# pyannote/pyannote-video

Measured on AMD Instinct MI355X. Metric: frames/sec end-to-end detect->embed->cluster, 1080p@25fps, higher is better.
Workload: dtype f32 (detector scores, embedder) / f64 (tracker, clustering) / u8 frames; an f16 screening pass with a proven error bound decides which windows the detector's exact f32 chain is evaluated for -- results identical to dense f32 scoring (`dense_scoring`)

## Files before the change

### include/pvface.h

```cpp
#ifndef PVFACE_H
#define PVFACE_H
#include <stdint.h>
#include <stddef.h>

#ifdef __cplusplus
extern "C" {
#endif

typedef uint64_t pvf_handle;
typedef struct { int32_t left, top, right, bottom; } pvf_rect_i32;

const char* pvf_last_error(void);
int32_t pvf_version(void);
int32_t pvf_device_count(int32_t* n);
int32_t pvf_ctx_create(int32_t device, pvf_handle* ctx);
int32_t pvf_ctx_create_prio(int32_t device, int32_t priority_class, pvf_handle* ctx);
int32_t pvf_ctx_destroy(pvf_handle ctx);
int32_t pvf_sync(pvf_handle ctx);

int32_t pvf_load_detector(pvf_handle ctx, const char* path);
int32_t pvf_load_shape_predictor(pvf_handle ctx, const char* path);
int32_t pvf_load_embedder(pvf_handle ctx, const char* path);
int32_t pvf_model_tensor(const char* path, int32_t kind, const char* name, void* out, int64_t cap_bytes, int64_t* nbytes);
int32_t pvf_set_tracker_tables(pvf_handle ctx, const double* mask64, const double* mask_scale, const double* tw64,
                               const double* tw32, double alpha_pow_m16, double ln_alpha);

int32_t pvf_frame_upload(pvf_handle ctx, const uint8_t* rgb, int32_t h, int32_t w, int64_t row_stride_bytes, pvf_handle* frame);
int32_t pvf_frame_wrap_device(pvf_handle ctx, const void* dev_rgb, int32_t h, int32_t w, pvf_handle* frame);
int32_t pvf_frame_release(pvf_handle ctx, pvf_handle frame);
int32_t pvf_frame_release_many(pvf_handle ctx, const pvf_handle* frames, int32_t n);
int32_t pvf_frame_pool_trim(pvf_handle ctx, int64_t keep_bytes, int64_t* pooled_bytes);
int32_t pvf_mem_info(pvf_handle ctx, int64_t* free_bytes, int64_t* total_bytes);
int32_t pvf_frame_device_ptr(pvf_handle ctx, pvf_handle frame, const void** dev_rgb);

int32_t pvf_ingest_create(pvf_handle ctx, int32_t h, int32_t w, int32_t depth, pvf_handle* ring);
int32_t pvf_ingest_destroy(pvf_handle ctx, pvf_handle ring);
int32_t pvf_ingest_acquire(pvf_handle ctx, pvf_handle ring, int32_t* slot, uint8_t** host_rgb);
int32_t pvf_ingest_submit(pvf_handle ctx, pvf_handle ring, int32_t slot, pvf_handle* frame);
int32_t pvf_ingest_wait(pvf_handle ctx, pvf_handle ring);
#define PVF_YUV_BT709 1
#define PVF_YUV_FULL_RANGE 2
int32_t pvf_ingest_create_yuv(pvf_handle ctx, int32_t h, int32_t w, int32_t depth, int32_t layout, int32_t flags, pvf_handle* ring);
int32_t pvf_frame_from_yuv(pvf_handle ctx, const uint8_t* y, int64_t y_pitch, const uint8_t* u, const uint8_t* v, int64_t c_pitch,
                           int32_t c_step, int32_t h, int32_t w, int32_t layout, int32_t flags, pvf_handle* frame);
int32_t pvf_frame_resize(pvf_handle ctx, pvf_handle frame, int32_t out_w, int32_t out_h, pvf_handle* out);

#define PVF_PRIM_RECT 0
#define PVF_PRIM_LINE 1
#define PVF_PRIM_TEXT 2
#define PVF_RENDER_MAX_PRIMS 4096
#define PVF_RENDER_MAX_RUN 64
#define PVF_RENDER_MAX_TEXT (1 << 20)
#define PVF_RENDER_MAX_SCALE 64
#define PVF_RENDER_MAX_BATCH 1024
typedef struct { int32_t type, a, b, c, d; uint32_t colour; int32_t scale, reserved; } pvf_prim;
int32_t pvf_render_batch(pvf_handle ctx, const pvf_handle* frames, int32_t n, int32_t out_w, int32_t out_h, int32_t flags,
                         const int32_t* start, const pvf_prim* prims, const uint8_t* text, int64_t text_bytes,
                         uint8_t* out, int32_t out_on_device);
int32_t pvf_egress_create(pvf_handle ctx, int32_t out_w, int32_t out_h, int32_t depth, int32_t flags, pvf_handle* ring);
int32_t pvf_egress_destroy(pvf_handle ctx, pvf_handle ring);
int32_t pvf_egress_submit(pvf_handle ctx, pvf_handle ring, pvf_handle frame, const pvf_prim* prims, int32_t n_prims,
                          const uint8_t* text, int64_t text_bytes, int32_t* slot);
int32_t pvf_egress_wait(pvf_handle ctx, pvf_handle ring, int32_t slot, const uint8_t** host_planes);
int32_t pvf_egress_release(pvf_handle ctx, pvf_handle ring, int32_t slot);
int32_t pvf_debug_render_rgb(pvf_handle ctx, pvf_handle frame, int32_t out_w, int32_t out_h, const pvf_prim* prims, int32_t n_prims,
                             const uint8_t* text, int64_t text_bytes, uint8_t* rgb);

int32_t pvf_detect(pvf_handle ctx, pvf_handle frame, int32_t upsample, double adjust_threshold,
                   pvf_rect_i32* out, float* scores, int32_t cap, int32_t* n);
int32_t pvf_detect_batch(pvf_handle ctx, const pvf_handle* frames, int32_t n_frames, int32_t upsample,
                         double adjust_threshold, pvf_rect_i32* out, float* scores, int32_t* counts,
                         int32_t cap_per_frame);
int32_t pvf_detect_many(pvf_handle ctx, const pvf_handle* frames, int32_t n_frames, int32_t batch, int32_t upsample,
                        double adjust_threshold, pvf_rect_i32* out, float* scores, int32_t* counts, int32_t cap);

int32_t pvf_detector_screening(pvf_handle ctx, int32_t on, int32_t list_cap);
int32_t pvf_detector_screening_stats(pvf_handle ctx, int64_t* batches, int64_t* listed, int64_t* retries, double* bounds, double* pipe_err);

int32_t pvf_embedder_split(pvf_handle ctx, int32_t on);
int32_t pvf_embedder_split_stats(pvf_handle ctx, int64_t* faces, int64_t* reruns, double* pipe_err);

int32_t pvf_tracker_create(pvf_handle ctx, pvf_handle* trk);
int32_t pvf_tracker_create_many(pvf_handle ctx, int32_t n, pvf_handle* trks);
int32_t pvf_tracker_destroy_many(pvf_handle ctx, const pvf_handle* trks, int32_t n);
int32_t pvf_tracker_clone_many(pvf_handle ctx, const pvf_handle* src, int32_t n, pvf_handle* dst);
int32_t pvf_tracker_destroy(pvf_handle ctx, pvf_handle trk);
int32_t pvf_tracker_start(pvf_handle ctx, pvf_handle trk, pvf_handle frame, const double box[4]);
int32_t pvf_tracker_update(pvf_handle ctx, pvf_handle trk, pvf_handle frame, double* psr);
int32_t pvf_tracker_position(pvf_handle ctx, pvf_handle trk, double box[4]);
int32_t pvf_tracker_start_many(pvf_handle ctx, const pvf_handle* trks, const pvf_handle* frames,
                               const double* boxes , int32_t n);
int32_t pvf_tracker_update_many(pvf_handle ctx, const pvf_handle* trks, const pvf_handle* frames, int32_t n,
                                double* psr , double* boxes_out );
int32_t pvf_tracker_update_many_deferred(pvf_handle ctx, const pvf_handle* trks, const pvf_handle* frames, int32_t n,
                                         double* psr, double* boxes_out);
int32_t pvf_tracker_commit_many(pvf_handle ctx, const pvf_handle* trks, const pvf_handle* frames, int32_t n);

int32_t pvf_overlap_matrix(const double* a, int32_t na, const double* b, int32_t nb, double ratio, double* out);
int32_t pvf_associate(const double* trackers, int32_t n_trackers, const double* detections, int32_t n_detections,
                      double min_overlap_ratio, int32_t* det_of_tracker);
int32_t pvf_munkres(const double* cost, int32_t n, int32_t* row_to_col);

int32_t pvf_landmarks(pvf_handle ctx, const pvf_handle* frames, const pvf_rect_i32* boxes, int32_t n,
                      int32_t* pts );
int32_t pvf_embed(pvf_handle ctx, const pvf_handle* frames, const int32_t* pts , int32_t n,
                  float* out );
int32_t pvf_landmarks_embed(pvf_handle ctx, const pvf_handle* frames, const pvf_rect_i32* boxes, int32_t n,
                            int32_t* pts , float* out );
int32_t pvf_embed_chips(pvf_handle ctx, const uint8_t* chips, int32_t n, float* out );
int32_t pvf_face_chips(pvf_handle ctx, const pvf_handle* frames, const int32_t* pts, int32_t n, uint8_t* chips );

int32_t pvf_pair_mean_dist(pvf_handle ctx, const double* X, int32_t N, int32_t dim, const int32_t* row_start,
                           int32_t T, double* D);
int32_t pvf_pair_mean_dist_metric(pvf_handle ctx, const double* X, int32_t N, int32_t dim, const int32_t* row_start,
                                  int32_t T, int32_t metric, double* D);
int32_t pvf_lane_create(int32_t n_frames, const int32_t* det_counts , const double* det_boxes ,
                        int32_t direction, double min_confidence, double min_overlap_ratio, int32_t deferring, pvf_handle* lane);
int32_t pvf_lane_destroy(pvf_handle lane);
int32_t pvf_lane_feed_plan(pvf_handle lane, int32_t p0, int32_t n_p, const uint8_t* has_update, const uint64_t* handles, const double* psr,
                           const double* pos);
int32_t pvf_lane_advance(pvf_handle lane, const double* reply_psr, const double* reply_pos, int32_t n_reply, int32_t* request,
                         uint64_t* req_handles, int32_t* req_frames, int32_t cap, int32_t* n_req, int32_t* plan_from);
int32_t pvf_lane_take_dead(pvf_handle lane, uint64_t* out, int32_t cap, int32_t* n);
int32_t pvf_lane_edges(pvf_handle lane, int32_t* n_edges, int32_t* u_frame_kind, double* u_box, int32_t* v_frame_kind, double* v_box,
                       double* conf, int32_t cap);
int32_t pvf_shot_tracks(pvf_handle lane_forward, pvf_handle lane_backward, const double* times, int32_t n_frames, double max_gap,
                        int32_t* rows, int32_t cap, int32_t* n_rows, int32_t* track_start, int32_t track_cap, int32_t* n_tracks);
int32_t pvf_track_rows(const int32_t* boxes, int64_t n, int32_t det_width, int32_t det_height, int32_t width, int32_t height,
                       double* file_box, int32_t* pixel_box);
int32_t pvf_round_decimals(const double* in, int64_t n, int32_t decimals, double* out);

int32_t pvf_pair_mean_dist_rows(pvf_handle ctx, const double* X, int32_t N, int32_t dim, const int32_t* row_start, int32_t T,
                                int32_t track0, int32_t track1, double* D);
int32_t pvf_pair_upper_rows(pvf_handle ctx, const double* X, int32_t N, int32_t dim, const int32_t* row_start, int32_t T,
                            int32_t track0, int32_t track1, double* D);
int32_t pvf_cluster_dist(pvf_handle ctx, const double* D, const int32_t* row_start, int32_t T, double threshold,
                         int32_t* labels, double* merge_log, int32_t* n_merges);
int32_t pvf_cluster_upper(pvf_handle ctx, const double* U, int32_t on_device, const int32_t* row_start, int32_t T, double threshold,
                          int32_t* labels, double* merge_log, int32_t* n_merges);
int32_t pvf_cluster_tracks(pvf_handle ctx, const double* X, int32_t N, int32_t dim, const int32_t* row_start,
                           int32_t T, double threshold, int32_t* labels, double* merge_log, int32_t* n_merges);
int32_t pvf_cluster_tracks_f32(pvf_handle ctx, const float* emb, int64_t row_stride_bytes, int32_t n_src, int32_t emb_on_device,
                               const int32_t* order, int32_t N, int32_t decimals, const int32_t* row_start, int32_t T, int32_t metric,
                               double threshold, int32_t* labels, double* merge_log, int32_t* n_merges);
int32_t pvf_pair_upper_rows_f32(pvf_handle ctx, const float* emb, int64_t row_stride_bytes, int32_t n_src, int32_t emb_on_device,
                                const int32_t* order, int32_t N, int32_t decimals, const int32_t* row_start, int32_t T,
                                int32_t track0, int32_t track1, double* rows_out, int32_t out_on_device);

int32_t pvf_format_rows(const double* t, const int64_t* identifier, const double* values, int64_t n_rows, int32_t n_cols,
                        int32_t decimals, char* out, int64_t cap, int64_t* written);

int32_t pvf_round_rows(const float* x, int64_t n, int32_t decimals, double* out);

int32_t pvf_parse_rows(const char* text, int64_t len, double* out, int64_t cap, int64_t* n_rows, int32_t* n_cols);

int32_t pvf_prof_enable(pvf_handle ctx, int32_t on);
int32_t pvf_prof_reset(pvf_handle ctx);
int32_t pvf_prof_get(pvf_handle ctx, const char* family, double* total_ms, int64_t* launches);

int32_t pvf_debug_pyramid_level(pvf_handle ctx, pvf_handle frame, int32_t upsample, int32_t level,
                                uint8_t* out, int32_t* h, int32_t* w);
int32_t pvf_debug_pyramid_batch(pvf_handle ctx, const pvf_handle* frames, int32_t n, int32_t upsample);
int32_t pvf_debug_level_features(pvf_handle ctx, pvf_handle frame, int32_t upsample, int32_t level,
                                 float* out, int32_t* fh, int32_t* fw);
int32_t pvf_debug_level_plan(pvf_handle ctx, pvf_handle frame, int32_t upsample, int32_t level, int32_t* out8);
int32_t pvf_debug_fhog(pvf_handle ctx, const uint8_t* img, int32_t h, int32_t w, int32_t cell, int32_t pad_r,
                       int32_t pad_c, float* out, int32_t* fh, int32_t* fw);
int32_t pvf_debug_detect_raw(pvf_handle ctx, pvf_handle frame, int32_t upsample, double adjust, float* scores,
                             int32_t* meta , int32_t cap, int32_t* n);
int32_t pvf_debug_detect_raw_many(pvf_handle ctx, const pvf_handle* frames, int32_t n_frames, int32_t batch, int32_t upsample,
                                  double adjust, int32_t* counts, int32_t* rows, int64_t cap, int64_t* total);
int32_t pvf_debug_extract_chip(pvf_handle ctx, pvf_handle frame, const double rect[4], double cs, double sn,
                               int32_t rows, int32_t cols, uint8_t* out);
int32_t pvf_debug_tracker_state(pvf_handle ctx, pvf_handle trk, double* F, double* A, double* B);
int32_t pvf_debug_tracker_scale_state(pvf_handle ctx, pvf_handle trk, double* As, double* Bs);
int32_t pvf_debug_embed_stage(pvf_handle ctx, const uint8_t* chips, int32_t n, int32_t split, int32_t stage, float* out, int32_t dims[3],
                              int32_t* flags);
int32_t pvf_debug_conv(pvf_handle ctx, const int32_t geom[18], const float* in, const float* w, const float* bias, const float* gamma,
                       const float* beta, const float* skip, int32_t split, int32_t force_generic, float* out, int32_t* flags);
int32_t pvf_debug_embed_head(pvf_handle ctx, const float* x, int32_t n, int32_t hw, float* out);

int32_t pvf_shot_dfd(pvf_handle ctx, const pvf_handle* frames, int32_t n, int32_t width, int32_t height, const float* tables,
                     double* dfd, uint8_t* gray_out, float* flow_out);

int32_t pvf_orb_extract(pvf_handle ctx, const pvf_handle* frames, int32_t n, int32_t width, int32_t height, int32_t cap,
                        int32_t* counts, float* keypoints, uint8_t* descriptors);
int32_t pvf_orb_match_counts(pvf_handle ctx, const uint8_t* descriptors, const int32_t* rows, int32_t n_sets, int32_t cap,
                             const int32_t* pairs, int64_t n_pairs, int32_t* counts);

#ifdef __cplusplus
}
#endif
#endif
```

### pyannote-video_amd/csrc/api.hip

```cpp
#include "pvf_internal.h"
#include <algorithm>
#include <cmath>
#include <cstdlib>
#include <string>
#include <thread>

#define API_BEGIN try {
#define API_END                                                        \
    return 0;                                                          \
    }                                                                  \
    catch (const std::exception& e) { pvf_set_error(e.what()); return -1; } \
    catch (...) { pvf_set_error("unknown error"); return -2; }

#define ENTER(c, h)                                                \
    Ctx* c = pvf_ctx(h);                                           \
    std::lock_guard<std::recursive_mutex> _api_lock(c->api_mu);    \
    HIP_CHECK(hipSetDevice(c->device))
#define ENTER_DET(c, h)                                            \
    Ctx* c = pvf_ctx(h);                                           \
    std::lock_guard<std::recursive_mutex> _det_lock(c->det_mu);    \
    HIP_CHECK(hipSetDevice(c->device))
#define ENTER_BOTH(c, h)                                           \
    Ctx* c = pvf_ctx(h);                                           \
    std::lock_guard<std::recursive_mutex> _det_lock(c->det_mu);    \
// ... 47 lines not shown
extern "C" int32_t pvf_embedder_split(pvf_handle h, int32_t on)
{
    API_BEGIN
    ENTER(c, h);
    c->emb_split = on != 0;
    API_END
}

extern "C" int32_t pvf_embedder_split_stats(pvf_handle h, int64_t* faces, int64_t* reruns, double* pipe_err)
{
    API_BEGIN
    ENTER(c, h);
    if (faces) *faces = c->emb_split_faces;
    if (reruns) *reruns = c->emb_reruns;
    if (pipe_err) *pipe_err = c->emb_pipe_err;
    API_END
}

extern "C" int32_t pvf_detect_batch(pvf_handle h, const pvf_handle* frames, int32_t n_frames, int32_t upsample, double adjust,
                                    pvf_rect_i32* out, float* scores, int32_t* counts, int32_t cap)
{
    API_BEGIN
    ENTER_DET(c, h);
    PVF_REQUIRE(n_frames > 0 && frames && out && counts && cap > 0, "pvf_detect_batch: bad arguments");
    PVF_REQUIRE(upsample >= 0 && upsample <= 2, "pvf_detect_batch: upsample must be 0..2");
    std::vector<Frame> fr(n_frames);
    for (int i = 0; i < n_frames; ++i) fr[i] = c->frame(frames[i]);
    std::vector<std::vector<RawDet>> raw;
    with_candidate_room(c, [&]() { det_run_batch(c, fr, upsample, adjust, raw); });
    std::vector<RawDet> kept;
    for (int i = 0; i < n_frames; ++i) {
        det_nms(c->det, raw[i], kept);
        const int n = std::min<int>((int)kept.size(), cap);
        counts[i] = n;
        for (int k = 0; k < n; ++k) {
            out[(size_t)i * cap + k] = pvf_rect_i32{kept[k].l, kept[k].t, kept[k].rr, kept[k].b};
            if (scores) scores[(size_t)i * cap + k] = kept[k].score;
        }
    }
    API_END
}

extern "C" int32_t pvf_detect_many(pvf_handle h, const pvf_handle* frames, int32_t n_frames, int32_t batch, int32_t upsample, double adjust,
                                   pvf_rect_i32* out, float* scores, int32_t* counts, int32_t cap)
{
    API_BEGIN
    ENTER_DET(c, h);
    PVF_REQUIRE(n_frames > 0 && batch > 0 && frames && out && counts && cap > 0, "pvf_detect_many: bad arguments");
    PVF_REQUIRE(upsample >= 0 && upsample <= 2, "pvf_detect_many: upsample must be 0..2");
    std::vector<Frame> fr(n_frames);
    for (int i = 0; i < n_frames; ++i) fr[i] = c->frame(frames[i]);
    std::vector<std::vector<RawDet>> kept_all;
    with_candidate_room(c, [&]() { det_run_many(c, fr, batch, upsample, adjust, kept_all, true); });
    for (int i = 0; i < n_frames; ++i) {
        const std::vector<RawDet>& kept = kept_all[i];
        const int n = std::min<int>((int)kept.size(), cap);
        counts[i] = n;
        for (int k = 0; k < n; ++k) {
            out[(size_t)i * cap + k] = pvf_rect_i32{kept[k].l, kept[k].t, kept[k].rr, kept[k].b};
            if (scores) scores[(size_t)i * cap + k] = kept[k].score;
        }
    }
    API_END
}

extern "C" int32_t pvf_detect(pvf_handle h, pvf_handle frame, int32_t upsample, double adjust, pvf_rect_i32* out, float* scores,
                              int32_t cap, int32_t* n)
{
    int32_t cnt = 0;
    const int32_t rc = pvf_detect_batch(h, &frame, 1, upsample, adjust, out, scores, &cnt, cap);
    if (rc == 0 && n) *n = cnt;
    return rc;
}

extern "C" int32_t pvf_debug_detect_raw(pvf_handle h, pvf_handle frame, int32_t upsample, double adjust, float* scores, int32_t* meta,
                                        int32_t cap, int32_t* n)
{
    API_BEGIN
    ENTER_DET(c, h);
    std::vector<Frame> fr{c->frame(frame)};
    std::vector<std::vector<RawDet>> raw;
    with_candidate_room(c, [&]() { det_run_batch(c, fr, upsample, adjust, raw); });
    const int k = std::min<int>((int)raw[0].size(), cap);
    *n = (int)raw[0].size();
    for (int i = 0; i < k; ++i) {
        const RawDet& d = raw[0][i];
        scores[i] = d.score;
        int32_t* m = meta + (size_t)i * 8;
        m[0] = d.filter; m[1] = d.level; m[2] = d.r; m[3] = d.c; m[4] = d.l; m[5] = d.t; m[6] = d.rr; m[7] = d.b;
    }
    API_END
}

extern "C" int32_t pvf_debug_detect_raw_many(pvf_handle h, const pvf_handle* frames, int32_t n_frames, int32_t batch, int32_t upsample, double adjust,
                                             int32_t* counts, int32_t* rows, int64_t cap, int64_t* total)
{
    API_BEGIN
    ENTER_DET(c, h);
    PVF_REQUIRE(n_frames > 0 && batch > 0 && frames && counts && total && (rows || cap == 0), "pvf_debug_detect_raw_many: bad arguments");
    PVF_REQUIRE(upsample >= 0 && upsample <= 2, "pvf_debug_detect_raw_many: upsample must be 0..2");
    std::vector<Frame> fr(n_frames);
    for (int i = 0; i < n_frames; ++i) fr[i] = c->frame(frames[i]);
    std::vector<std::vector<RawDet>> raw;
    with_candidate_room(c, [&]() { det_run_many(c, fr, batch, upsample, adjust, raw, false); });
    int64_t k = 0;
    for (int i = 0; i < n_frames; ++i) {
        counts[i] = (int32_t)raw[i].size();
        for (const RawDet& d : raw[i]) {
            if (k < cap) {
                int32_t* m = rows + (size_t)k * 5;
                m[0] = d.level; m[1] = d.filter; m[2] = d.r; m[3] = d.c;
                memcpy(&m[4], &d.score, 4);
            }
            ++k;
        }
    }
    *total = k;
    API_END
}

extern "C" int32_t pvf_debug_pyramid_level(pvf_handle h, pvf_handle frame, int32_t upsample, int32_t level, uint8_t* out, int32_t* oh,
                                           int32_t* ow)
{
    API_BEGIN
    ENTER_DET(c, h);
    std::vector<uint8_t> buf;
    int hh = 0, ww = 0;
    det_pyramid_level(c, c->frame(frame), upsample, level, out ? &buf : nullptr, &hh, &ww);
    *oh = hh; *ow = ww;
    if (out) memcpy(out, buf.data(), buf.size());
    API_END
}

extern "C" int32_t pvf_debug_pyramid_batch(pvf_handle h, const pvf_handle* frames, int32_t n, int32_t upsample)
{
    API_BEGIN
    ENTER_DET(c, h);
    PVF_REQUIRE(frames && n > 0, "pvf_debug_pyramid_batch: bad arguments");
    std::vector<Frame> fr;
    for (int i = 0; i < n; ++i) fr.push_back(c->frame(frames[i]));
    det_pyramid_batch(c, fr, upsample);
    API_END
}

extern "C" int32_t pvf_debug_level_features(pvf_handle h, pvf_handle frame, int32_t upsample, int32_t level, float* out, int32_t* fh, int32_t* fw)
{
    API_BEGIN
    ENTER_DET(c, h);
    std::vector<float> buf;
    int a = 0, b = 0;
    det_level_features(c, c->frame(frame), upsample, level, out ? &buf : nullptr, &a, &b);
    *fh = a; *fw = b;
    if (out) memcpy(out, buf.data(), buf.size() * sizeof(float));
    API_END
}

extern "C" int32_t pvf_debug_level_plan(pvf_handle h, pvf_handle frame, int32_t upsample, int32_t level, int32_t* out8)
{
    API_BEGIN
    ENTER_DET(c, h);
    PVF_REQUIRE(out8 != nullptr, "pvf_debug_level_plan: out8 is NULL");
    det_level_plan(c, c->frame(frame), upsample, level, out8);
    API_END
}

extern "C" int32_t pvf_debug_fhog(pvf_handle h, const uint8_t* img, int32_t ih, int32_t iw, int32_t cell, int32_t pad_r, int32_t pad_c,
                                  float* out, int32_t* fh, int32_t* fw)
{
    API_BEGIN
    ENTER_BOTH(c, h);
    int a = 0, b = 0;
    if (!out) { fhog_dims(ih, iw, cell, pad_r, pad_c, &a, &b); *fh = a; *fw = b; return 0; }
    std::vector<float> buf;
    fhog_debug(c, img, ih, iw, cell, pad_r, pad_c, buf, &a, &b);
    *fh = a; *fw = b;
    memcpy(out, buf.data(), buf.size() * sizeof(float));
    API_END
}

static pvf_handle tracker_new(Ctx* c)
{
    std::unique_ptr<Tracker> t(new Tracker());
    const uint64_t id = c->next_id++;
    c->trackers[id] = std::move(t);
    return id;
}

extern "C" int32_t pvf_tracker_create(pvf_handle h, pvf_handle* trk)
{
    API_BEGIN
    ENTER(c, h);
    *trk = tracker_new(c);
    API_END
}

extern "C" int32_t pvf_tracker_create_many(pvf_handle h, int32_t n, pvf_handle* trks)
{
    API_BEGIN
    ENTER(c, h);
    PVF_REQUIRE(n >= 0, "negative count");
    for (int i = 0; i < n; ++i) trks[i] = tracker_new(c);
    API_END
}

extern "C" int32_t pvf_tracker_clone_many(pvf_handle h, const pvf_handle* src, int32_t n, pvf_handle* dst)
{
    API_BEGIN
    ENTER(c, h);
    PVF_REQUIRE(n >= 0, "negative count");
    std::vector<Tracker*> s(n), d(n);
    for (int i = 0; i < n; ++i) s[i] = &c->tracker(src[i]);
    for (int i = 0; i < n; ++i) { dst[i] = tracker_new(c); d[i] = &c->tracker(dst[i]); }
    dsst_clone_many(c, s, d);
    API_END
}

static const size_t TRACKER_POOL_KEEP = 4096;
static void pool_tracker_state(Ctx* c, Tracker& t)
{
    double* d_state = t.d_state;
    t.d_state = nullptr;
    if (t.share) {
        int* sh = t.share;
        t.share = nullptr;
        if (--*sh > 0) return;
        delete sh;
    }
    if (!d_state) return;
    if (c->tracker_pool.size() < TRACKER_POOL_KEEP) { c->tracker_pool.push_back(d_state); return; }
    HIP_CHECK(hipStreamSynchronize(c->stream));
    HIP_CHECK(hipFree(d_state));
}

extern "C" int32_t pvf_tracker_destroy_many(pvf_handle h, const pvf_handle* trks, int32_t n)
{
    API_BEGIN
    ENTER(c, h);
    for (int i = 0; i < n; ++i) {
        auto it = c->trackers.find(trks[i]);
        PVF_REQUIRE(it != c->trackers.end(), "unknown tracker handle");
        pool_tracker_state(c, *it->second);
        c->trackers.erase(it);
    }
    API_END
}

extern "C" int32_t pvf_tracker_destroy(pvf_handle h, pvf_handle trk)
{
    API_BEGIN
    ENTER(c, h);
    auto it = c->trackers.find(trk);
    PVF_REQUIRE(it != c->trackers.end(), "unknown tracker handle");
    pool_tracker_state(c, *it->second);
    c->trackers.erase(it);
    API_END
}
extern "C" int32_t pvf_tracker_start_many(pvf_handle h, const pvf_handle* trks, const pvf_handle* frames, const double* boxes, int32_t n)
{
    API_BEGIN
    ENTER(c, h);
    std::vector<Tracker*> t(n);
    std::vector<Frame> f(n);
    PVF_REQUIRE(n >= 0 && (n == 0 || (trks && frames && boxes)), "tracker.start_track: bad arguments");
    for (int i = 0; i < n; ++i) {
        const double* b = boxes + 4 * (size_t)i;
        PVF_REQUIRE(std::isfinite(b[0]) && std::isfinite(b[1]) && std::isfinite(b[2]) && std::isfinite(b[3]),
                    "tracker.start_track: box with a non-finite coordinate");
        PVF_REQUIRE(b[2] - b[0] != 0.0 && b[3] - b[1] != 0.0, "tracker.start_track: box of zero width or height");
    }
    for (int i = 0; i < n; ++i) { t[i] = &c->tracker(trks[i]); f[i] = c->frame(frames[i]); }
    dsst_start_many(c, t, f, boxes);
    API_END
}
extern "C" int32_t pvf_tracker_update_many(pvf_handle h, const pvf_handle* trks, const pvf_handle* frames, int32_t n, double* psr,
                                           double* boxes_out)
{
    API_BEGIN
    ENTER(c, h);
    std::vector<Tracker*> t(n);
    std::vector<Frame> f(n);
    for (int i = 0; i < n; ++i) { t[i] = &c->tracker(trks[i]); f[i] = c->frame(frames[i]); }
    dsst_update_many(c, t, f, psr, boxes_out);
    API_END
}
extern "C" int32_t pvf_tracker_start(pvf_handle h, pvf_handle trk, pvf_handle frame, const double box[4])
{
    return pvf_tracker_start_many(h, &trk, &frame, box, 1);
}
extern "C" int32_t pvf_tracker_update_many_deferred(pvf_handle h, const pvf_handle* trks, const pvf_handle* frames, int32_t n, double* psr,
                                                    double* boxes_out)
{
    API_BEGIN
    ENTER(c, h);
    std::vector<Tracker*> t(n);
    std::vector<Frame> f(n);
    for (int i = 0; i < n; ++i) { t[i] = &c->tracker(trks[i]); f[i] = c->frame(frames[i]); }
    dsst_update_many(c, t, f, psr, boxes_out, 1);
    API_END
}

extern "C" int32_t pvf_tracker_commit_many(pvf_handle h, const pvf_handle* trks, const pvf_handle* frames, int32_t n)
{
    API_BEGIN
    ENTER(c, h);
    std::vector<Tracker*> t(n);
    std::vector<Frame> f(n);
// ... 689 lines not shown
```

### pyannote-video_amd/csrc/detect.hip

```cpp
#include "detect_ml.h"
#include <algorithm>
#include <thread>
#include <cmath>
#include <cstdlib>

#define RESIZE_MAXS 22
struct RowTab { int32_t top, bottom; double tb, tb1, pad; };
struct ColTab { int32_t left, pad; double lr, lr1, pad2; };

template <int RS, int NSTRIP>
__global__ void __launch_bounds__(256) resize_rows_k(const uint8_t* const* __restrict__ in_ptrs, const uint8_t* __restrict__ in_base,
                                                     size_t in_stride, int in_rb, int ih, int iw, uint8_t* __restrict__ out,
                                                     size_t out_stride, int out_rb, int oh, int ow,
                                                     const RowTab* __restrict__ rows, const ColTab* __restrict__ cols)
{
    constexpr int MAXS = (RS == 16) ? RESIZE_MAXS : (RS * 5) / 4 + 3;
    __shared__ uint32_t s_rows[4][MAXS][64];
    __shared__ uint32_t s_out[4][64];
    const int lane = threadIdx.x & 63;
    const int wave = __builtin_amdgcn_readfirstlane(threadIdx.x >> 6);
    const int c0 = blockIdx.x * 256 + wave * 64;
    const int b = blockIdx.z;
    if (c0 >= ow) return;
    const int c = min(c0 + lane, ow - 1);
// ... 164 lines not shown
}

static void pyramid_up_dims(int ih, int iw, int* oh, int* ow)
{
    const double right = ((iw - 1) + 1.25) * 2.0;
    const double bottom = ((ih - 1) + 0.75) * 2.0;
    *ow = (int)std::floor(right + 0.5) + 1;
    *oh = (int)std::floor(bottom + 0.5) + 1;
}


static inline long iround(double v) { return (long)std::floor(v + 0.5); }
static void rect_down6(long r[4]) { const double ratio = (6 - 1.0) / 6; for (int i = 0; i < 4; ++i) r[i] = iround((r[i] - 0.3) * ratio + 0.3); }
static void rect_up6(long r[4]) { const double ratio = 6 / (6 - 1.0); for (int i = 0; i < 4; ++i) r[i] = iround((r[i] - 0.3) * ratio + 0.3); }
static void rect_down2i(long r[4])
{
    r[0] = iround(r[0] / 2.0 - 1.25); r[1] = iround(r[1] / 2.0 - 0.75);
    r[2] = iround(r[2] / 2.0 - 1.25); r[3] = iround(r[3] / 2.0 - 0.75);
}
static int detector_levels(int h, int w, const DetectorModel& m)
{
    long r[4] = {0, 0, w - 1, h - 1};
    int levels = 0;
    do { rect_down6(r); ++levels; } while ((r[2] - r[0] + 1) >= m.min_w && (r[3] - r[1] + 1) >= m.min_h && levels < m.max_levels);
    return levels;
}
static void fhog_to_image(long px, long py, int cell, int pad_r, int pad_c, long* ox, long* oy)
{
    long x = (px + 1 - (pad_c - 1) / 2) * cell + 1;
    long y = (py + 1 - (pad_r - 1) / 2) * cell + 1;
    x += (x >= 0) ? cell / 2 : -(cell / 2);
    y += (y >= 0) ? cell / 2 : -(cell / 2);
    *ox = x; *oy = y;
}

struct LevelDims { int h, w; };
static std::vector<LevelDims> level_schedule(int h, int w, int upsample, const DetectorModel& m, std::vector<LevelDims>* ups)
{
    int ch = h, cw = w;
    for (int u = 0; u < upsample; ++u) {
        int nh, nw;
        pyramid_up_dims(ch, cw, &nh, &nw);
        ch = nh; cw = nw;
        if (ups) ups->push_back({ch, cw});
    }
    const int levels = detector_levels(ch, cw, m);
    std::vector<LevelDims> out;
    out.push_back({ch, cw});
    for (int l = 1; l < levels; ++l) { ch = (5 * ch) / 6; cw = (5 * cw) / 6; out.push_back({ch, cw}); }
    return out;
}

static void upload_frame_ptrs(Ctx* c, const std::vector<Frame>& frames, const uint8_t*** d_ptrs)
{
    DevBuf& d = c->s_fptr[c->det_slot & 1];
    HostBuf& h = c->h_fptr[c->det_slot & 1];
    d.ensure(frames.size() * sizeof(void*));
    h.ensure(frames.size() * sizeof(void*));
    const uint8_t** hp = h.as<const uint8_t*>();
    for (size_t i = 0; i < frames.size(); ++i) hp[i] = frames[i].d;
    HIP_CHECK(hipMemcpyAsync(d.p, hp, frames.size() * sizeof(void*), hipMemcpyHostToDevice, c->det_stream));
    *d_ptrs = d.as<const uint8_t*>();
}


__device__ __forceinline__ int ml_block(const MlStarts& st) { return (int)blockIdx.x; }
static inline int ml_grid(int total) { return total; }

__device__ __forceinline__ int ml_level(const MlStarts& st, int g)
{
    int l = 0;
    while (l + 1 < st.nl && g >= st.b0[l + 1]) ++l;
    return l;
}

#define FUSED_OUT 61
__device__ __forceinline__ uint32_t from_next_lane(uint32_t v) { return (uint32_t)__builtin_amdgcn_update_dpp(0, (int)v, 0x130, 0xf, 0xf, true); }
__device__ __forceinline__ uint32_t from_prev_lane(uint32_t v) { return (uint32_t)__builtin_amdgcn_update_dpp(0, (int)v, 0x138, 0xf, 0xf, true); }

#define FS_PAIRS 4
#define FS_COLS 65
#define FS_SLOT_DW (8 * FS_COLS * 2)
#define FS_BINS_DW (2 * 18 * 64)
#define FS_FLAG_DW (4 * 64)
#define FS_LDS_BYTES (FS_PAIRS * (FS_BINS_DW + 2 * FS_SLOT_DW + FS_FLAG_DW) * 4)
static_assert(FS_COLS * 8 == 520, "the ring's column pitch is written into the instruction strings below");
typedef __attribute__((address_space(3))) uint32_t* lds_u32;
__device__ __forceinline__ uint32_t lds_addr(const void* p) { return (uint32_t)(uintptr_t)(lds_u32)p; }

__device__ __forceinline__ void ring_write(uint32_t data_at, uint32_t flag_at, const u32x2* v, uint32_t row1)
{
    asm volatile("ds_write_b64 %0, %2\n\tds_write_b64 %0, %3 offset:520\n\tds_write_b64 %0, %4 offset:1040\n\tds_write_b64 %0, %5 offset:1560\n\t"
                 "ds_write_b64 %0, %6 offset:2080\n\tds_write_b64 %0, %7 offset:2600\n\tds_write_b64 %0, %8 offset:3120\n\t"
                 "ds_write_b64 %0, %9 offset:3640\n\tds_write_b32 %1, %10"
                 :: "v"(data_at), "v"(flag_at), "v"(v[0]), "v"(v[1]), "v"(v[2]), "v"(v[3]), "v"(v[4]), "v"(v[5]), "v"(v[6]), "v"(v[7]), "v"(row1) : "memory");
}
__device__ __forceinline__ uint32_t ring_read(uint32_t data_at, uint32_t flag_at, u32x2* own, u32x2* nb)
{
    uint32_t ready;
    asm volatile("ds_read_b32 %0, %18\n\t"
                 "ds_read_b64 %1, %17\n\tds_read_b64 %9, %17 offset:8\n\tds_read_b64 %2, %17 offset:520\n\tds_read_b64 %10, %17 offset:528\n\t"
                 "ds_read_b64 %3, %17 offset:1040\n\tds_read_b64 %11, %17 offset:1048\n\tds_read_b64 %4, %17 offset:1560\n\tds_read_b64 %12, %17 offset:1568\n\t"
                 "ds_read_b64 %5, %17 offset:2080\n\tds_read_b64 %13, %17 offset:2088\n\tds_read_b64 %6, %17 offset:2600\n\tds_read_b64 %14, %17 offset:2608\n\t"
                 "ds_read_b64 %7, %17 offset:3120\n\tds_read_b64 %15, %17 offset:3128\n\tds_read_b64 %8, %17 offset:3640\n\tds_read_b64 %16, %17 offset:3648\n\t"
                 "s_waitcnt lgkmcnt(0)"
                 : "=&v"(ready), "=&v"(own[0]), "=&v"(own[1]), "=&v"(own[2]), "=&v"(own[3]), "=&v"(own[4]), "=&v"(own[5]), "=&v"(own[6]), "=&v"(own[7]),
                   "=&v"(nb[0]), "=&v"(nb[1]), "=&v"(nb[2]), "=&v"(nb[3]), "=&v"(nb[4]), "=&v"(nb[5]), "=&v"(nb[6]), "=&v"(nb[7])
                 : "v"(data_at), "v"(flag_at) : "memory");
    return ready;
}
__device__ __forceinline__ void flag_write(uint32_t flag_at, uint32_t v)
{
    asm volatile("ds_write_b32 %0, %1" :: "v"(flag_at), "v"(v) : "memory");
}

template <int A, int B> __device__ __forceinline__ uint32_t sub_into_upper(uint32_t acc, uint32_t x, uint32_t y);
#define PVF_SUBW1(A, B)                                                                                                                  \
    template <> __device__ __forceinline__ uint32_t sub_into_upper<A, B>(uint32_t acc, uint32_t x, uint32_t y)                           \
    {                                                                                                                                    \
        asm("v_sub_u32_sdwa %0, %1, %2 dst_sel:WORD_1 dst_unused:UNUSED_PRESERVE src0_sel:BYTE_" #A " src1_sel:BYTE_" #B "\n\ts_nop 0"   \
            : "+v"(acc) : "v"(x), "v"(y));                                                                                               \
        return acc;                                                                                                                      \
    }
PVF_SUBW1(0, 0) PVF_SUBW1(1, 1) PVF_SUBW1(2, 2) PVF_SUBW1(3, 3)
#undef PVF_SUBW1
typedef short s16x2 __attribute__((ext_vector_type(2)));

template <int P>
__device__ __forceinline__ u32x2 split_grad_px(const uint32_t* up, const uint32_t* ce, const uint32_t* dn, const __amdgpu_buffer_rsrc_t& lut_rs,
                                               bool valid)
{
    uint32_t pk[3];
    int cv[3];
#define PVF_CH(K)                                                                                                                         \
    {                                                                                                                                     \
        constexpr int IU = 4 + 3 * P + K, IL = 1 + 3 * P + K, IR = 7 + 3 * P + K;                                                         \
        const uint32_t cx = ((ce[IR >> 2] >> (8 * (IR & 3))) & 0xffu) - ((ce[IL >> 2] >> (8 * (IL & 3))) & 0xffu);                          \
        pk[K] = sub_into_upper<(IU & 3), (IU & 3)>(cx, dn[IU >> 2], up[IU >> 2]);                                                          \
        const s16x2 v = __builtin_bit_cast(s16x2, pk[K]);                                                                                 \
        cv[K] = __builtin_amdgcn_sdot2(v, v, 0, false);                                                                                   \
    }
    PVF_CH(0) PVF_CH(1) PVF_CH(2)
#undef PVF_CH
    const int bv = max(cv[0], max(cv[1], cv[2]));
    const uint32_t pb = (cv[0] == bv) ? pk[0] : ((cv[1] == bv) ? pk[1] : pk[2]);
    const uint32_t off = (pb & 7u) | ((pb >> 13) & 0xff8u) | ((pb << 9) & 0x3f000u);
    u32x2 r;
    r.y = (uint32_t)__builtin_amdgcn_raw_buffer_load_b8(lut_rs, off, 0, 0);
    const float m = sqrt_exact_small((float)bv);
    r.x = valid ? __float_as_uint(m) : 0u;
    return r;
}

__global__ void __launch_bounds__(512) __attribute__((amdgpu_waves_per_eu(4, 4)))
fhog_split_ml_k(MlStarts st, const LvDesc* __restrict__ lv, int B, const uint8_t* __restrict__ img_base, float* __restrict__ feat_base,
                const uint8_t* __restrict__ lutw, int oy, int ox)
{
    constexpr int RSRC_FLAGS = 0x00020000;
    extern __shared__ __attribute__((aligned(16))) uint32_t fs_lds[];
    const int lane = threadIdx.x & 63;
    const int wave = __builtin_amdgcn_readfirstlane(threadIdx.x >> 6);
    const int pair = wave & 3, role = wave >> 2;
    for (int i = threadIdx.x; i < FS_PAIRS * (2 * FS_SLOT_DW + FS_FLAG_DW); i += 512) fs_lds[FS_PAIRS * FS_BINS_DW + i] = 0u;
    __syncthreads();
    const int g = ml_block(st);
    if (g >= st.b0[st.nl]) return;
    const int l = ml_level(st, g);
    const LvDesc d = lv[l];
    const int task = (g - st.b0[l]) * FS_PAIRS + pair;
    if (task >= d.fused_tasks) return;
    const int sx = task % d.strips;
    const int t2 = task / d.strips;
    const int cy = t2 % d.chunks;
    const int b = t2 / d.chunks;
    const int y0 = cy * d.chunk_rows;
    const int R = min(d.chunk_rows, d.hog_nr - y0);
    const int g_first = y0 + 1, g_last = y0 + R + 3;
    const int y_begin = 8 * g_first - 12;
    const uint32_t ring_at = lds_addr(fs_lds + FS_PAIRS * FS_BINS_DW + pair * 2 * FS_SLOT_DW) + 8u * lane;
    uint32_t* const flags = fs_lds + FS_PAIRS * (FS_BINS_DW + 2 * FS_SLOT_DW) + pair * FS_FLAG_DW + lane;
    const uint32_t flag_at = lds_addr(flags);

    if (role == 0) {
        const int hx = FUSED_OUT * sx + 1 + lane;
        const int x_first = 8 * hx - 12;
        const uint8_t* im = img_base + d.img_off + (size_t)b * d.img_stride;
        const int rb = d.rb;
        unsigned xmask = 0;
#pragma unroll
        for (int p = 0; p < 8; ++p) if (x_first + p >= 1 && x_first + p < d.visible_nc) xmask |= 1u << p;
        const bool strip_inside = __builtin_amdgcn_ballot_w64(xmask != 0xffu) == 0;
        const int voff = 3 * x_first - 4, voff2 = voff + 16;
        const __amdgpu_buffer_rsrc_t lut_rs = __builtin_amdgcn_make_buffer_rsrc((void*)lutw, 0, 1 << 18, RSRC_FLAGS);
        uint32_t rw[4][8];
        auto load_row = [&](int yi, uint32_t* dst) {
            const int bytes = (yi >= 0 && yi < d.h) ? rb : 0;
            const int yc = min(max(yi, 0), d.h - 1);
            const __amdgpu_buffer_rsrc_t rs = __builtin_amdgcn_make_buffer_rsrc((void*)(im + (size_t)yc * rb), 0, bytes, RSRC_FLAGS);
            const u32x4 a = __builtin_amdgcn_raw_buffer_load_b128(rs, voff, 0, 0);
            const u32x4 c = __builtin_amdgcn_raw_buffer_load_b128(rs, voff2, 0, 0);
            dst[0] = a.x; dst[1] = a.y; dst[2] = a.z; dst[3] = a.w; dst[4] = c.x; dst[5] = c.y; dst[6] = c.z; dst[7] = c.w;
        };
#pragma unroll
        for (int q = 0; q < 4; ++q) load_row(y_begin - 1 + q, rw[q]);
        const int nrows = 8 * (g_last - g_first + 1);
        for (int k0 = 0; k0 < nrows; k0 += 4) {
#pragma unroll
            for (int i = 0; i < 4; ++i) {
                const int k = k0 + i, y = y_begin + k;
                const uint32_t* up = rw[i & 3];
                const uint32_t* ce = rw[(i + 1) & 3];
                const uint32_t* dn = rw[(i + 2) & 3];
                const int freed = (int)__hip_atomic_load(flags + 128 + 64 * (i & 1), __ATOMIC_RELAXED, __HIP_MEMORY_SCOPE_WORKGROUP);
                const bool ok = (y >= 1 && y < d.visible_nr);
                u32x2 mb[8];
                if (strip_inside && ok) {
                    mb[0] = split_grad_px<0>(up, ce, dn, lut_rs, true); mb[1] = split_grad_px<1>(up, ce, dn, lut_rs, true);
                    mb[2] = split_grad_px<2>(up, ce, dn, lut_rs, true); mb[3] = split_grad_px<3>(up, ce, dn, lut_rs, true);
                    mb[4] = split_grad_px<4>(up, ce, dn, lut_rs, true); mb[5] = split_grad_px<5>(up, ce, dn, lut_rs, true);
                    mb[6] = split_grad_px<6>(up, ce, dn, lut_rs, true); mb[7] = split_grad_px<7>(up, ce, dn, lut_rs, true);
                } else {
                    mb[0] = split_grad_px<0>(up, ce, dn, lut_rs, ok && (xmask & 1u));
                    mb[1] = split_grad_px<1>(up, ce, dn, lut_rs, ok && (xmask & 2u));
                    mb[2] = split_grad_px<2>(up, ce, dn, lut_rs, ok && (xmask & 4u));
                    mb[3] = split_grad_px<3>(up, ce, dn, lut_rs, ok && (xmask & 8u));
                    mb[4] = split_grad_px<4>(up, ce, dn, lut_rs, ok && (xmask & 16u));
                    mb[5] = split_grad_px<5>(up, ce, dn, lut_rs, ok && (xmask & 32u));
                    mb[6] = split_grad_px<6>(up, ce, dn, lut_rs, ok && (xmask & 64u));
                    mb[7] = split_grad_px<7>(up, ce, dn, lut_rs, ok && (xmask & 128u));
                }
                load_row(y + 3, rw[i & 3]);
                int fr = freed;
                while (fr < k - 1) {
                    __builtin_amdgcn_s_sleep(1);
                    fr = (int)__hip_atomic_load(flags + 128 + 64 * (i & 1), __ATOMIC_RELAXED, __HIP_MEMORY_SCOPE_WORKGROUP);
                }
                ring_write(ring_at + (i & 1) * 4 * FS_SLOT_DW, flag_at + 256 * (i & 1), mb, (uint32_t)(k + 1));
            }
        }
        return;
    }

    float* accE = reinterpret_cast<float*>(fs_lds) + pair * FS_BINS_DW + lane;
    float* accO = accE + 18 * 64;
#pragma unroll
    for (int k = 0; k < 18; ++k) { accE[64 * k] = 0.0f; accO[64 * k] = 0.0f; }
    float hprev[18];
    float e0 = 0.f, e1 = 0.f, e2 = 0.f;
#pragma unroll
    for (int k = 0; k < 18; ++k) hprev[k] = 0.f;
    int krow = 0;
    auto band = [&](int gb, float* accU, float* accL) {
#pragma unroll
        for (int i = 0; i < 8; ++i) {
            u32x2 own[8], nb[8];
            for (;;) {
                const int ready = (int)ring_read(ring_at + (i & 1) * 4 * FS_SLOT_DW, flag_at + 256 * (i & 1), own, nb);
                if (__builtin_amdgcn_readfirstlane(ready) > krow) break;
                __builtin_amdgcn_s_sleep(1);
            }
            ++krow;
            flag_write(flag_at + 512 + 256 * (i & 1), (uint32_t)krow);
            const float fy = ((float)i + 0.5f) / 8.0f;
#pragma unroll
            for (int j = 0; j < 16; ++j) {
                const int p = j & 7;
                const u32x2 v = (j < 8) ? own[p] : nb[p];
                const float mv = __uint_as_float(v.x);
                const int bv = (int)(v.y << 8);
                const float fx = ((float)p + 0.5f) / 8.0f;
                const float wx = (j < 8) ? fx : 1.0f - fx;
                float* const pl = reinterpret_cast<float*>(reinterpret_cast<char*>(accL) + bv);
                float* const pu = reinterpret_cast<float*>(reinterpret_cast<char*>(accU) + bv);
                const float vl = *pl, vu = *pu;
                *pl = vl + ((1.0f - fy) * wx) * mv;
                *pu = vu + (fy * wx) * mv;
            }
        }
        const int c = gb - 1;
        float e = 0.0f;
#pragma unroll
        for (int o = 0; o < 9; ++o) { const float s2 = accL[64 * o] + accL[64 * (o + 9)]; e = e + s2 * s2; }
        e2 = e1; e1 = e0; e0 = e;
        if (c >= y0 + 3) {
            float n[9];
            n[1] = e2; n[4] = e1; n[7] = e0;
            n[0] = __uint_as_float(from_prev_lane(__float_as_uint(e2))); n[2] = __uint_as_float(from_next_lane(__float_as_uint(e2)));
            n[3] = __uint_as_float(from_prev_lane(__float_as_uint(e1))); n[5] = __uint_as_float(from_next_lane(__float_as_uint(e1)));
            n[6] = __uint_as_float(from_prev_lane(__float_as_uint(e0))); n[8] = __uint_as_float(from_next_lane(__float_as_uint(e0)));
            const int x = FUSED_OUT * sx + lane - 1, yh = c - 3;
            if (lane >= 1 && lane <= FUSED_OUT && x < d.hog_nc) {
                float4* dst = reinterpret_cast<float4*>(feat_base + d.feat_off + (size_t)b * d.feat_stride + feat_at(yh + oy, 0, x + ox, d.fwp));
                const size_t step = (size_t)d.fwp;
                const float eps = 0.0001f;
                const float z1[4] = {n[4], n[1], n[3], n[0]}, z2[4] = {n[5], n[2], n[4], n[1]}, z3[4] = {n[7], n[4], n[6], n[3]}, z4[4] = {n[8], n[5], n[7], n[4]};
                float nn[4], nv[4], t[4] = {0.f, 0.f, 0.f, 0.f};
#pragma unroll
                for (int k = 0; k < 4; ++k) {
                    nn[k] = 0.2f * sqrtf((((z1[k] + z2[k]) + z3[k]) + z4[k]) + eps);
                    nv[k] = 0.1f / nn[k];
                }
                float o[20];
#pragma unroll
                for (int g = 0; g < 18; g += 3) {
                    float hh[3][4];
#pragma unroll
                    for (int j = 0; j < 3; ++j) {
#pragma unroll
                        for (int k = 0; k < 4; ++k) hh[j][k] = fminf(hprev[g + j], nn[k]) * nv[k];
                        o[g + j] = (hh[j][0] + hh[j][1]) + (hh[j][2] + hh[j][3]);
                    }
#pragma unroll
                    for (int k = 0; k < 4; ++k) t[k] = t[k] + ((hh[0][k] + hh[1][k]) + hh[2][k]);
                    if (g == 3) { *dst = make_float4(o[0], o[1], o[2], o[3]); dst += step; __builtin_amdgcn_sched_barrier(0); }
                    if (g == 6) { *dst = make_float4(o[4], o[5], o[6], o[7]); dst += step; __builtin_amdgcn_sched_barrier(0); }
                    if (g == 9) { *dst = make_float4(o[8], o[9], o[10], o[11]); dst += step; __builtin_amdgcn_sched_barrier(0); }
                    if (g == 15) { *dst = make_float4(o[12], o[13], o[14], o[15]); dst += step; __builtin_amdgcn_sched_barrier(0); }
                }
                float ci[9];
#pragma unroll
                for (int g = 0; g < 9; ++g) {
                    const float s2 = hprev[g] + hprev[g + 9];
                    float hh[4];
#pragma unroll
                    for (int k = 0; k < 4; ++k) hh[k] = fminf(s2, nn[k]) * nv[k];
                    ci[g] = (hh[0] + hh[1]) + (hh[2] + hh[3]);
                    if (g == 1) { *dst = make_float4(o[16], o[17], ci[0], ci[1]); dst += step; __builtin_amdgcn_sched_barrier(0); }
                    if (g == 5) { *dst = make_float4(ci[2], ci[3], ci[4], ci[5]); dst += step; __builtin_amdgcn_sched_barrier(0); }
                }
                const float tscale = (float)(2 * 0.2357);
#pragma unroll
                for (int k = 0; k < 4; ++k) t[k] = t[k] * tscale;
                *dst = make_float4(ci[6], ci[7], ci[8], t[0]); dst += step;
                *dst = make_float4(t[1], t[2], t[3], 0.0f);
            }
        }
#pragma unroll
        for (int k = 0; k < 18; ++k) { hprev[k] = accL[64 * k]; accL[64 * k] = 0.0f; }
    };
    for (int gb = g_first; gb <= g_last; ++gb) {
        if (gb & 1) band(gb, accO, accE);
        else band(gb, accE, accO);
    }
}

__global__ void __launch_bounds__(256) feat_ring_zero_k(MlStarts st, const LvDesc* __restrict__ lv, int B, float* __restrict__ feat_base, int oy, int ox)
{
    const int g = ml_block(st);
    if (g >= st.b0[st.nl]) return;
    const int l = ml_level(st, g);
    const LvDesc d = lv[l];
    const int local = g - st.b0[l];
    const int xb = local % d.feat_bx;
    const int py = (local / d.feat_bx) % d.fh;
    const int b = local / (d.feat_bx * d.fh);
    const int px = xb * 256 + threadIdx.x;
    if (px >= d.fwp) return;
    const int x = px - ox, y = py - oy;
    if (x >= 0 && y >= 0 && x < d.hog_nc && y < d.hog_nr) return;
    float4* dst = reinterpret_cast<float4*>(feat_base + d.feat_off + (size_t)b * d.feat_stride + feat_at(py, 0, px, d.fwp));
#pragma unroll
    for (int k = 0; k < 8; ++k) dst[(size_t)k * d.fwp] = make_float4(0.f, 0.f, 0.f, 0.f);
}

__global__ void __launch_bounds__(128) __attribute__((amdgpu_waves_per_eu(2, 2)))
score_roll_k(MlStarts st, const LvDesc* __restrict__ lv, int B, const float* __restrict__ feat_base,
             const float4* __restrict__ Bg4, ScoreParams sp, int* __restrict__ counts, CandRec* __restrict__ cands)
{
    constexpr int FR = 10, FC = 10, NK = 12, PITCH = 31, MT = 2, WCOLS = MT * 48, SEG = WCOLS + 11, R = 5;
    constexpr int LAST_STEPS = 93 - 8 * (NK - 1);
    constexpr int NSTW = (SEG * 8 + 127) / 128;
    constexpr int SLAB = (SEG * PITCH + 3) / 4 * 4;
    constexpr int RSRC_FLAGS = 0x00020000;
    extern __shared__ __attribute__((aligned(16))) float s_seg[];
    const int lane = threadIdx.x & 63;
    const int wave = __builtin_amdgcn_readfirstlane(threadIdx.x >> 6);
    const int g = (int)blockIdx.x;
    if (g >= st.b0[st.nl]) return;
    const int l = ml_level(st, g);
    const LvDesc d = lv[l];
    const int local = g - st.b0[l];
    const int bx = local % d.score_bx;
    const int sg = (local / d.score_bx) % d.roll_nseg;
    const int b = __builtin_amdgcn_readfirstlane(local / (d.score_bx * d.roll_nseg));
    const int fw = d.fw;
    const int c_base = bx * WCOLS;
    const int c1 = fw - (FC - FC / 2 - 1);
    const int r_base = sg * d.roll_rows;
    const int out_rows = min(d.roll_rows, d.fh - (FR - 1) - r_base);
    const int fh = out_rows + FR - 1;
    const int fwp = d.fwp;
    const float* fb = feat_base + d.feat_off + (size_t)b * d.feat_stride + feat_at(r_base, 0, c_base, fwp);
    const int seg_cells = (fw - c_base < SEG) ? fw - c_base : SEG;
    const int i = lane & 15, kq = lane >> 4;
    const int lane16 = lane * 16;
    const bool two_tiles = (c_base + 48 + FC / 2 < c1);
    const __amdgpu_buffer_rsrc_t brs = __builtin_amdgcn_make_buffer_rsrc((void*)Bg4, 0, FR * NK * 2 * 64 * 16, RSRC_FLAGS);
    f32x4 acc[R][MT];
#pragma unroll
    for (int q = 0; q < R; ++q)
#pragma unroll
        for (int tt = 0; tt < MT; ++tt) acc[q][tt] = (f32x4){0.f, 0.f, 0.f, 0.f};
    constexpr int NH = 4;
    static_assert(NSTW <= 8 && SEG <= 128, "one cell per thread");
    u32x4 sv[NH];
    const int tid16 = (int)threadIdx.x * 16;
    auto load_part = [&](int fr, int half) {
        const int bytes = (fr < fh) ? seg_cells * 16 : 0;
#pragma unroll
        for (int u = 0; u < NH; ++u) {
            const __amdgpu_buffer_rsrc_t rs = __builtin_amdgcn_make_buffer_rsrc((void*)(fb + ((size_t)fr * 8 + half * NH + u) * fwp * 4), 0, bytes, RSRC_FLAGS);
            sv[u] = __builtin_amdgcn_raw_buffer_load_b128(rs, tid16, 0, 0);
        }
    };
    auto fill_part = [&](float* seg, int half) {
        if ((int)threadIdx.x < SEG) {
#pragma unroll
            for (int u = 0; u < NH; ++u) {
                const int q = half * NH + u;
                uint32_t* dd = reinterpret_cast<uint32_t*>(seg + (int)threadIdx.x * PITCH + 4 * q);
                dd[0] = sv[u].x; dd[1] = sv[u].y; dd[2] = sv[u].z;
                if (q != 7) dd[3] = sv[u].w;
            }
        }
    };
    auto emit = [&](int r_out, const f32x4 (&a)[MT]) {
        const int jc = lane & 15;
        if (jc < 15) {
            const int sft = jc / 5, f = jc % 5;
            const float th = sp.thresh[f];
            const int r = r_base + r_out + FR / 2;
#pragma unroll
            for (int tt = 0; tt < MT; ++tt)
#pragma unroll
                for (int reg = 0; reg < 4; ++reg) {
                    const int pos = 4 * (lane >> 4) + reg;
                    const int cc = c_base + tt * 48 + 3 * pos + sft + FC / 2;
                    const float v = a[tt][reg];
                    if (cc < c1 && v >= th && (tt == 0 || two_tiles)) {
                        const int idx = atomicAdd(&counts[b], 1);
                        if (idx < sp.cap) {
                            CandRec rec;
                            rec.score = v - th; rec.filter = f; rec.level = l; rec.r = r; rec.c = cc;
                            cands[(size_t)b * sp.cap + idx] = rec;
                        }
                    }
                }
        }
    };
    load_part(0, 0); fill_part(s_seg, 0);
    load_part(0, 1); fill_part(s_seg, 1);
    __syncthreads();
    for (int s = 0; s < fh; ++s) {
        const float* seg = s_seg + (s & 1) * SLAB;
        float* nxt = s_seg + ((s + 1) & 1) * SLAB;
        load_part(s + 1, 0);
        const int p = (s - wave) & 1;
        const int r0 = s - p;
        bool on[R];
        bool all_on = two_tiles, any_on = false;
#pragma unroll
        for (int q = 0; q < R; ++q) {
            const int r = r0 - 2 * q;
            on[q] = (r >= 0 && r < out_rows);
            all_on = all_on && on[q];
            any_on = any_on || on[q];
        }
        if (any_on) {
            const int bop = p * NK * 2048;
            const float* a0 = seg + (3 * i) * PITCH + kq;
            u32x4 bn[R][2];
            float an[8 * MT];
#pragma unroll
            for (int q = 0; q < R; ++q) {
                bn[q][0] = __builtin_amdgcn_raw_buffer_load_b128(brs, lane16, bop + 2 * q * NK * 2048, 0);
                bn[q][1] = __builtin_amdgcn_raw_buffer_load_b128(brs, lane16, bop + 2 * q * NK * 2048 + 1024, 0);
            }
#pragma unroll
            for (int pq = 0; pq < 8; ++pq)
#pragma unroll
                for (int tt = 0; tt < MT; ++tt) an[pq * MT + tt] = a0[(tt * 48) * PITCH + 4 * pq];
#pragma unroll
            for (int n = 0; n < NK; ++n) {
                float ac[8 * MT];
                float bc[R][8];
#pragma unroll
                for (int x = 0; x < 8 * MT; ++x) ac[x] = an[x];
#pragma unroll
                for (int q = 0; q < R; ++q)
#pragma unroll
                    for (int h = 0; h < 2; ++h) {
                        const uint32_t b0 = bn[q][h].x, b1 = bn[q][h].y, b2 = bn[q][h].z, b3 = bn[q][h].w;
                        bc[q][4 * h] = __uint_as_float(b0); bc[q][4 * h + 1] = __uint_as_float(b1);
                        bc[q][4 * h + 2] = __uint_as_float(b2); bc[q][4 * h + 3] = __uint_as_float(b3);
                    }
                if (n + 1 < NK) {
#pragma unroll
                    for (int q = 0; q < R; ++q) {
                        bn[q][0] = __builtin_amdgcn_raw_buffer_load_b128(brs, lane16, bop + (2 * q * NK + n + 1) * 2048, 0);
                        bn[q][1] = __builtin_amdgcn_raw_buffer_load_b128(brs, lane16, bop + (2 * q * NK + n + 1) * 2048 + 1024, 0);
                    }
#pragma unroll
                    for (int pq = 0; pq < 8; ++pq)
#pragma unroll
                        for (int tt = 0; tt < MT; ++tt) an[pq * MT + tt] = a0[(tt * 48) * PITCH + 32 * (n + 1) + 4 * pq];
                }
                if (n == NK / 2) { fill_part(nxt, 0); load_part(s + 1, 1); }
                __builtin_amdgcn_sched_barrier(0);
                const int steps = (n == NK - 1) ? LAST_STEPS : 8;
                if (all_on) {
#pragma unroll
                    for (int pq = 0; pq < steps; ++pq)
#pragma unroll
                        for (int q = 0; q < R; ++q)
#pragma unroll
// ... 88 lines not shown
            const int hog_nr = (int)((double)ld.h / 8.0 + 0.5) - 2, hog_nc = (int)((double)ld.w / 8.0 + 0.5) - 2;
            if (hog_nr > 0 && hog_nc > 0) tasks += (long long)((hog_nc + FUSED_OUT - 1) / FUSED_OUT) * std::max(2, (hog_nr + cand - 1) / cand) * B;
        }
        if (tasks >= 2LL * c->n_cu * 2 * 4) { chunk_big = cand; break; }
    }
    if (getenv("PVF_FHOG_CHUNK") && atoi(getenv("PVF_FHOG_CHUNK")) > 0) chunk_big = atoi(getenv("PVF_FHOG_CHUNK"));
    for (size_t l = 0; l < dims.size(); ++l) {
        LvDesc d;
        memset(&d, 0, sizeof d);
        d.h = dims[l].h; d.w = dims[l].w;
        d.cells_nr = (int)((double)d.h / 8.0 + 0.5); d.cells_nc = (int)((double)d.w / 8.0 + 0.5);
        d.visible_nr = std::min(d.cells_nr * 8, d.h) - 1; d.visible_nc = std::min(d.cells_nc * 8, d.w) - 1;
        d.hog_nr = d.cells_nr - 2; d.hog_nc = d.cells_nc - 2;
        const bool feat_ok = d.hog_nr > 0 && d.hog_nc > 0;
        d.fh = feat_ok ? d.hog_nr + m.frows - 1 : 0; d.fw = feat_ok ? d.hog_nc + m.fcols - 1 : 0;
        d.valid_score = (d.fh >= m.frows && d.fw >= m.fcols) ? 1 : 0;
        d.rb = (int)al((size_t)d.w * 3, 64);
        d.img_off = (long long)p.img_bytes; d.img_stride = (long long)d.h * d.rb;
        p.img_bytes += (size_t)d.img_stride * B;
        d.fwp = feat_ok ? d.fw + FEAT_PAD_COLS : 0;
        d.feat_off = (long long)p.feat_floats; d.feat_stride = (long long)d.fh * d.fwp * PVF_FHOG_STRIDE;
        p.feat_floats += (size_t)d.feat_stride * B;
        d.feat_bx = feat_ok ? (d.fwp + 255) / 256 : 0;
        const int out_c = d.fw - 9;
        d.score_bx = d.valid_score ? (out_c + 95) / 96 : 0;
        d.strips = feat_ok ? (d.hog_nc + FUSED_OUT - 1) / FUSED_OUT : 0;
        {
            const int nch = std::max(2, (d.hog_nr + chunk_big - 1) / chunk_big);
            d.chunk_rows = std::max((d.hog_nr + nch - 1) / nch, 1);
        }
        d.chunks = feat_ok ? (d.hog_nr + d.chunk_rows - 1) / d.chunk_rows : 0;
        d.fused_tasks = d.strips * d.chunks * B;
        p.feat.b0[l] = p.feat_blocks; p.feat_blocks += d.feat_bx * d.fh * B;
        p.fused.b0[l] = p.fused_blocks; p.fused_blocks += (d.fused_tasks + 3) / 4;
        p.lv.push_back(d);
    }
    const int nl = (int)dims.size();
    {
        long long total = 0;
        for (const LvDesc& d : p.lv) if (d.valid_score) total += (long long)d.score_bx * (d.fh - 9 + 9) * B;
        const int slots = 4 * 256;
        int roll_max = (int)std::max<long long>(64, total / slots / 2);
        if (getenv("PVF_SCORE_SEG")) roll_max = std::max(2, atoi(getenv("PVF_SCORE_SEG")));
        for (int l = 0; l < nl; ++l) {
            LvDesc& d = p.lv[l];
            const int out_r = d.fh - 9;
            d.roll_nseg = d.valid_score ? (out_r + roll_max - 1) / roll_max : 0;
            d.roll_rows = d.valid_score ? ((out_r + d.roll_nseg - 1) / d.roll_nseg + 1) / 2 * 2 : 0;
            if (d.valid_score) d.roll_nseg = (out_r + d.roll_rows - 1) / d.roll_rows;
            p.walk.b0[l] = p.walk_blocks; p.walk_blocks += d.score_bx * d.roll_nseg * B;
        }
    }
    p.feat.b0[nl] = p.feat_blocks; p.walk.b0[nl] = p.walk_blocks;
    p.fused.b0[nl] = p.fused_blocks;
    HIP_CHECK(hipMalloc((void**)&p.d_lv, sizeof(LvDesc) * nl));
    HIP_CHECK(hipMemcpy(p.d_lv, p.lv.data(), sizeof(LvDesc) * nl, hipMemcpyHostToDevice));
    {
        std::vector<RowTab> tab;
        int ch = h;
        for (size_t u = 0; u < p.ups.size(); ++u) { p.up_tab.push_back(tab.size()); fill_row_table(tab, ch, p.ups[u].h); ch = p.ups[u].h; }
        p.lv_tab.push_back(0);
        for (int l = 1; l < nl; ++l) { p.lv_tab.push_back(tab.size()); fill_row_table(tab, p.lv[l - 1].h, p.lv[l].h); }
        HIP_CHECK(hipMalloc((void**)&p.d_rowtab, sizeof(RowTab) * std::max<size_t>(tab.size(), 1)));
        if (!tab.empty()) HIP_CHECK(hipMemcpy(p.d_rowtab, tab.data(), sizeof(RowTab) * tab.size(), hipMemcpyHostToDevice));
        std::vector<ColTab> ctab;
        int cw2 = w;
        for (size_t u = 0; u < p.ups.size(); ++u) { p.up_ctab.push_back(ctab.size()); fill_col_table(ctab, cw2, p.ups[u].w); cw2 = p.ups[u].w; }
        p.lv_ctab.push_back(0);
        for (int l = 1; l < nl; ++l) { p.lv_ctab.push_back(ctab.size()); fill_col_table(ctab, p.lv[l - 1].w, p.lv[l].w); }
        HIP_CHECK(hipMalloc((void**)&p.d_coltab, sizeof(ColTab) * std::max<size_t>(ctab.size(), 1)));
        if (!ctab.empty()) HIP_CHECK(hipMemcpy(p.d_coltab, ctab.data(), sizeof(ColTab) * ctab.size(), hipMemcpyHostToDevice));
    }
    MlPlan* raw = pp.get();
    c->ml_plans->plans[key] = std::move(pp);
    return raw;
}

static MlPlan* ml_build_pyramid(Ctx* c, const std::vector<Frame>& frames, int upsample)
{
    const int B = (int)frames.size();
    const int h = frames[0].h, w = frames[0].w;
    for (auto& f : frames) PVF_REQUIRE(f.h == h && f.w == w, "batched frames must share one size");
    MlPlan* p = ml_plan(c, h, w, upsample, B);
    c->s_pyr.ensure(p->img_bytes + p->up_bytes + 256);
    uint8_t* base = c->s_pyr.as<uint8_t>();
    uint8_t* up_tmp = base + ((p->img_bytes + 63) / 64) * 64;
    const uint8_t** d_ptrs = nullptr;
    upload_frame_ptrs(c, frames, &d_ptrs);
    ProfScope ps(c, "pyramid", c->det_stream);
    auto al = [](size_t v, size_t a) { return (v + a - 1) / a * a; };
    const uint8_t* cur = nullptr;
    int ch = h, cw = w, crb = w * 3;
    size_t cstride = 0;
    for (size_t u = 0; u < p->ups.size(); ++u) {
        const bool last = (u + 1 == p->ups.size());
        uint8_t* dst = last ? base + p->lv[0].img_off : up_tmp;
        const int drb = (int)al((size_t)p->ups[u].w * 3, 64);
        const size_t dstride = (size_t)p->ups[u].h * drb;
        launch_resize_rows(c, cur ? nullptr : d_ptrs, cur, cstride, crb, ch, cw, dst, dstride, drb, p->ups[u].h, p->ups[u].w, B, p->d_rowtab + p->up_tab[u], p->d_coltab + p->up_ctab[u]);
        cur = dst; cstride = dstride; crb = drb; ch = p->ups[u].h; cw = p->ups[u].w;
    }
    if (!cur) {
        for (int b = 0; b < B; ++b)
            HIP_CHECK(hipMemcpy2DAsync(base + p->lv[0].img_off + (size_t)b * p->lv[0].img_stride, (size_t)p->lv[0].rb, frames[b].d, (size_t)w * 3,
                                       (size_t)w * 3, (size_t)h, hipMemcpyDeviceToDevice, c->det_stream));
    }
    for (size_t l = 1; l < p->lv.size(); ++l)
        launch_resize_rows(c, nullptr, base + p->lv[l - 1].img_off, (size_t)p->lv[l - 1].img_stride, p->lv[l - 1].rb, p->lv[l - 1].h, p->lv[l - 1].w,
                           base + p->lv[l].img_off, (size_t)p->lv[l].img_stride, p->lv[l].rb, p->lv[l].h, p->lv[l].w, B, p->d_rowtab + p->lv_tab[l], p->d_coltab + p->lv_ctab[l]);
    return p;
}

__global__ void dpp_probe_k(int* out)
{
    const int lane = threadIdx.x;
    out[lane] = (int)from_next_lane((uint32_t)(lane + 100));
    out[64 + lane] = (int)from_prev_lane((uint32_t)(lane + 100));
}
#define SQRT_PROBE_N (2 * 255 * 255 + 1)
__global__ void sqrt_probe_k(float* out)
{
    const int i = blockIdx.x * blockDim.x + threadIdx.x;
    if (i < SQRT_PROBE_N) out[i] = sqrt_exact_small((float)i);
}
static void check_dpp_direction(Ctx* c)
{
    MlPlanCache* pc = c->ml_plans;
    if (pc->dpp_probe < 0) {
        int* d = nullptr;
        HIP_CHECK(hipMalloc((void**)&d, 128 * sizeof(int) + SQRT_PROBE_N * sizeof(float)));
        float* ds = reinterpret_cast<float*>(d + 128);
        hipLaunchKernelGGL(dpp_probe_k, dim3(1), dim3(64), 0, c->det_stream, d);
        hipLaunchKernelGGL(sqrt_probe_k, dim3((SQRT_PROBE_N + 255) / 256), dim3(256), 0, c->det_stream, ds);
        int h[128];
        std::vector<float> hs(SQRT_PROBE_N);
        HIP_CHECK(hipMemcpyAsync(h, d, sizeof h, hipMemcpyDeviceToHost, c->det_stream));
        HIP_CHECK(hipMemcpyAsync(hs.data(), ds, SQRT_PROBE_N * sizeof(float), hipMemcpyDeviceToHost, c->det_stream));
        HIP_CHECK(hipStreamSynchronize(c->det_stream));
        (void)hipFree(d);
        bool ok = true;
        for (int i = 0; i < 64; ++i) {
            ok = ok && h[i] == (i < 63 ? i + 101 : 0);
            ok = ok && h[64 + i] == (i > 0 ? i + 99 : 0);
        }
        pc->dpp_probe = ok ? 1 : 0;
        bool sq = true;
        for (int i = 0; i < SQRT_PROBE_N; ++i) sq = sq && hs[i] == (float)std::sqrt((double)i);
        pc->sqrt_probe = sq ? 1 : 0;
    }
    PVF_REQUIRE(pc->dpp_probe == 1, "v_mov_b32_dpp wave_shl / wave_shr do not move data as the FHOG kernel expects on this device");
    PVF_REQUIRE(pc->sqrt_probe == 1, "v_sqrt_f32 is not within one step below the correctly rounded root on this device: the FHOG kernel's one-sided correction does not hold");
}

static MlPlan* ml_features(Ctx* c, const std::vector<Frame>& frames, int upsample)
{
    const DetectorModel& m = c->det;
    const int B = (int)frames.size();
    MlPlan* p = ml_build_pyramid(c, frames, upsample);
    const int oy = (m.frows - 1) / 2, ox = (m.fcols - 1) / 2;
    const void* feat_before = c->s_feat.p;
    c->s_feat.ensure(p->feat_floats * sizeof(float) + 64);
    if (p->fused_blocks == 0) return p;
    check_dpp_direction(c);
    ProfScope ps(c, "fhog", c->det_stream);
    if (c->s_feat.p != feat_before || c->feat_ring_owner != (const void*)p) {
        hipLaunchKernelGGL(feat_ring_zero_k, dim3(ml_grid(p->feat_blocks)), dim3(256), 0, c->det_stream, p->feat, p->d_lv, B, c->s_feat.as<float>(), oy, ox);
        c->feat_ring_owner = (const void*)p;
    }
    static std::atomic<uint64_t> attr_set{0};
    const uint64_t bit = 1ull << (c->device & 63);
    if (!(attr_set.load() & bit)) {
        HIP_CHECK(hipFuncSetAttribute(reinterpret_cast<const void*>(fhog_split_ml_k), hipFuncAttributeMaxDynamicSharedMemorySize, FS_LDS_BYTES));
        attr_set.fetch_or(bit);
    }
    hipLaunchKernelGGL(fhog_split_ml_k, dim3(ml_grid(p->fused_blocks)), dim3(512), FS_LDS_BYTES, c->det_stream, p->fused, p->d_lv, B,
                       c->s_pyr.as<uint8_t>(), c->s_feat.as<float>(), orientation_lut_wrapped(c), oy, ox);
    return p;
}

static void det_run_batch_ml(Ctx* c, const std::vector<Frame>& frames, int upsample, const ScoreParams& sp0, int* d_counts, CandRec* d_cands)
{
    const DetectorModel& m = c->det;
    const int B = (int)frames.size();
    MlPlan* p = ml_features(c, frames, upsample);
    if (p->walk_blocks == 0) return;
    if (c->det_screen && !c->det_screen_suspended) {
        if (!p->screen_built) { screen_plan_build(p->screen, p->lv, B); p->screen_built = true; }
        if (p->screen.usable) {
            ProfScope ps(c, "score_screened", c->det_stream);
            screen_launch(c, p->screen, p->d_lv, B, c->s_feat.as<float>(), sp0, d_counts, d_cands, d_counts + B);
            ++c->screen_batches;
            return;
        }
    }
    ProfScope ps(c, "score", c->det_stream);
    const size_t lds = (size_t)2 * (((2 * 48 + 11) * 31 + 3) / 4 * 4) * sizeof(float);
    const float4* b4 = reinterpret_cast<const float4*>(m.d_bmfma4);
    hipLaunchKernelGGL(score_roll_k, dim3(p->walk_blocks), dim3(128), lds, c->det_stream, p->walk, p->d_lv, B, c->s_feat.as<float>(), b4, sp0, d_counts, d_cands);
}

void det_pyramid_level(Ctx* c, const Frame& f, int upsample, int level, std::vector<uint8_t>* out, int* oh, int* ow)
{
    PVF_REQUIRE(c->det.loaded, "detector not loaded");
    std::vector<Frame> fr{f};
    MlPlan* p = ml_build_pyramid(c, fr, upsample);
    PVF_REQUIRE(level >= 0 && level < (int)p->lv.size(), "pyramid level out of range");
    *oh = p->lv[level].h; *ow = p->lv[level].w;
    if (out) {
        out->resize((size_t)(*oh) * (*ow) * 3);
        HIP_CHECK(hipMemcpy2DAsync(out->data(), (size_t)(*ow) * 3, c->s_pyr.as<uint8_t>() + p->lv[level].img_off, (size_t)p->lv[level].rb,
                                   (size_t)(*ow) * 3, (size_t)(*oh), hipMemcpyDeviceToHost, c->det_stream));
    }
    HIP_CHECK(hipStreamSynchronize(c->det_stream));
}

void det_pyramid_batch(Ctx* c, const std::vector<Frame>& frames, int upsample)
{
    PVF_REQUIRE(c->det.loaded, "detector not loaded");
    PVF_REQUIRE(!frames.empty(), "pyramid batch: no frames");
    (void)ml_build_pyramid(c, frames, upsample);
    HIP_CHECK(hipStreamSynchronize(c->det_stream));
}

void det_level_features(Ctx* c, const Frame& f, int upsample, int level, std::vector<float>* out, int* fh, int* fw)
{
    PVF_REQUIRE(c->det.loaded, "detector not loaded");
    std::vector<Frame> fr{f};
    MlPlan* p = ml_features(c, fr, upsample);
    PVF_REQUIRE(level >= 0 && level < (int)p->lv.size(), "pyramid level out of range");
    const LvDesc& d = p->lv[level];
    *fh = d.fh; *fw = d.fw;
    if (out) {
        out->resize((size_t)d.fh * d.fw * PVF_FHOG_STRIDE);
        std::vector<float> dev((size_t)d.feat_stride);
        if (!dev.empty())
            HIP_CHECK(hipMemcpyAsync(dev.data(), c->s_feat.as<float>() + d.feat_off, dev.size() * sizeof(float), hipMemcpyDeviceToHost, c->det_stream));
        HIP_CHECK(hipStreamSynchronize(c->det_stream));
        for (int y = 0; y < d.fh; ++y)
            for (int j = 0; j < 8; ++j)
                for (int x = 0; x < d.fw; ++x)
                    memcpy(out->data() + ((size_t)y * d.fw + x) * PVF_FHOG_STRIDE + 4 * j, dev.data() + feat_at(y, j, x, d.fwp), 4 * sizeof(float));
    }
    HIP_CHECK(hipStreamSynchronize(c->det_stream));
}

void det_level_plan(Ctx* c, const Frame& f, int upsample, int level, int32_t out[8])
{
    PVF_REQUIRE(c->det.loaded, "detector not loaded");
    MlPlan* p = ml_plan(c, f.h, f.w, upsample, 1);
    PVF_REQUIRE(level >= 0 && level < (int)p->lv.size(), "pyramid level out of range");
    const LvDesc& d = p->lv[level];
    const int32_t v[8] = {d.h, d.w, d.hog_nr, d.hog_nc, d.chunk_rows, d.chunks, d.roll_rows, d.roll_nseg};
    memcpy(out, v, sizeof v);
}

static bool raw_less(const RawDet& x, const RawDet& y)
{
    if (x.score != y.score) return x.score > y.score;
    if (x.filter != y.filter) return x.filter < y.filter;
    if (x.level != y.level) return x.level < y.level;
    if (x.r != y.r) return x.r < y.r;
    return x.c < y.c;
}

static void decode_candidates(const DetectorModel& m, int upsample, const CandRec* q, int n, std::vector<RawDet>& v);

static void screen_verdict(Ctx* c, const int* ctl)
{
    if (!c->det_screen || c->det_screen_suspended) return;
    c->screen_listed += std::min(ctl[SCR_FLAGGED], c->screen_list_cap);
    if (ctl[SCR_FLAGGED] > c->screen_list_cap || ctl[SCR_VIOLATION] != 0) {
        HIP_CHECK(hipStreamSynchronize(c->det_stream));
        throw ScreenRetry();
    }
}

void det_run_batch(Ctx* c, const std::vector<Frame>& frames, int upsample, double adjust, std::vector<std::vector<RawDet>>& raw_sorted)
{
    const DetectorModel& m = c->det;
    PVF_REQUIRE(m.loaded, "detector not loaded");
    PVF_REQUIRE(!frames.empty(), "no frames");
    const int B = (int)frames.size();
    const int cap = c->det_cand_cap;
    const size_t cnt_bytes = (((size_t)(B + SCR_CTL_INTS) * sizeof(int) + 63) / 64) * 64;
    c->s_cand.ensure((size_t)B * cap * sizeof(CandRec) + cnt_bytes + 64);
    int* d_counts = c->s_cand.as<int>();
    CandRec* d_cands = reinterpret_cast<CandRec*>(c->s_cand.as<uint8_t>() + cnt_bytes);
    HIP_CHECK(hipMemsetAsync(d_counts, 0, (size_t)(B + SCR_CTL_INTS) * sizeof(int), c->det_stream));
    ScoreParams sp;
    for (int f = 0; f < 8; ++f) sp.thresh[f] = f < m.n_filters ? (float)((double)m.thresh[f] + adjust) : 3.0e38f;
    sp.n_filters = m.n_filters; sp.cap = cap;
    det_run_batch_ml(c, frames, upsample, sp, d_counts, d_cands);
    HIP_CHECK(hipGetLastError());
    c->h_cand.ensure((size_t)B * cap * sizeof(CandRec) + cnt_bytes + 64);
    int* h_counts = c->h_cand.as<int>();
    CandRec* h_cands = reinterpret_cast<CandRec*>(c->h_cand.as<uint8_t>() + cnt_bytes);
    HIP_CHECK(hipMemcpyAsync(h_counts, d_counts, (size_t)(B + SCR_CTL_INTS) * sizeof(int), hipMemcpyDeviceToHost, c->det_stream));
    HIP_CHECK(hipStreamSynchronize(c->det_stream));
    screen_verdict(c, h_counts + B);
    raw_sorted.assign(B, {});
    for (int b = 0; b < B; ++b) {
        const int n = h_counts[b];
        if (n > cap) throw CandOverflow(n);
        if (n == 0) continue;
        HIP_CHECK(hipMemcpyAsync(h_cands + (size_t)b * cap, d_cands + (size_t)b * cap, (size_t)n * sizeof(CandRec), hipMemcpyDeviceToHost,
                                 c->det_stream));
    }
    HIP_CHECK(hipStreamSynchronize(c->det_stream));
    for (int b = 0; b < B; ++b) decode_candidates(m, upsample, h_cands + (size_t)b * cap, h_counts[b], raw_sorted[b]);
}

static const int DET_PREFETCH = 512;

static void decode_candidates(const DetectorModel& m, int upsample, const CandRec* q, int n, std::vector<RawDet>& v)
{
    const int bw = m.fcols - 2 * m.padding, bh = m.frows - 2 * m.padding;
    v.resize(n);
    for (int i = 0; i < n; ++i) {
        long rect[4];
        const long cl = q[i].c - bw / 2, ct = q[i].r - bh / 2;
        fhog_to_image(cl, ct, m.cell, m.frows, m.fcols, &rect[0], &rect[1]);
        fhog_to_image(cl + bw - 1, ct + bh - 1, m.cell, m.frows, m.fcols, &rect[2], &rect[3]);
        for (int k = 0; k < q[i].level; ++k) rect_up6(rect);
        for (int u = 0; u < upsample; ++u) rect_down2i(rect);
        v[i] = RawDet{q[i].score, q[i].filter, q[i].level, q[i].r, q[i].c, (int32_t)rect[0], (int32_t)rect[1], (int32_t)rect[2], (int32_t)rect[3]};
    }
    std::sort(v.begin(), v.end(), raw_less);
}

void det_run_many(Ctx* c, const std::vector<Frame>& frames, int batch, int upsample, double adjust,
                  std::vector<std::vector<RawDet>>& raw_sorted, bool nms)
{
    const DetectorModel& m = c->det;
    PVF_REQUIRE(m.loaded, "detector not loaded");
    PVF_REQUIRE(!frames.empty() && batch > 0, "no frames");
    const int N = (int)frames.size();
    raw_sorted.assign(N, {});
    {
        const int nb = (N + batch - 1) / batch;
        batch = (N + nb - 1) / nb;
    }
    const int cap = c->det_cand_cap, PF = DET_PREFETCH;
    ScoreParams sp;
    for (int f = 0; f < 8; ++f) sp.thresh[f] = f < m.n_filters ? (float)((double)m.thresh[f] + adjust) : 3.0e38f;
    sp.n_filters = m.n_filters; sp.cap = cap;
    const size_t cnt_bytes = (((size_t)(batch + SCR_CTL_INTS) * sizeof(int) + 63) / 64) * 64;
    for (int k = 0; k < 2; ++k) {
        c->s_cand2[k].ensure(cnt_bytes + (size_t)batch * cap * sizeof(CandRec));
        c->h_cand2[k].ensure(cnt_bytes + (size_t)batch * PF * sizeof(CandRec));
        if (!c->det_ev[k]) HIP_CHECK(hipEventCreateWithFlags(&c->det_ev[k], hipEventDisableTiming));
    }
    auto submit = [&](int o, int slot) {
        std::vector<Frame> fr(frames.begin() + o, frames.begin() + std::min(N, o + batch));
        const int B = (int)fr.size();
        int* d_counts = c->s_cand2[slot].as<int>();
        CandRec* d_cands = reinterpret_cast<CandRec*>(c->s_cand2[slot].as<uint8_t>() + cnt_bytes);
        HIP_CHECK(hipMemsetAsync(d_counts, 0, (size_t)(B + SCR_CTL_INTS) * sizeof(int), c->det_stream));
        c->det_slot = slot;
        det_run_batch_ml(c, fr, upsample, sp, d_counts, d_cands);
        HIP_CHECK(hipGetLastError());
        uint8_t* hb = c->h_cand2[slot].as<uint8_t>();
        HIP_CHECK(hipMemcpyAsync(hb, d_counts, (size_t)(B + SCR_CTL_INTS) * sizeof(int), hipMemcpyDeviceToHost, c->det_stream));
        HIP_CHECK(hipMemcpy2DAsync(hb + cnt_bytes, (size_t)PF * sizeof(CandRec), d_cands, (size_t)cap * sizeof(CandRec),
                                   (size_t)PF * sizeof(CandRec), (size_t)B, hipMemcpyDeviceToHost, c->det_stream));
        HIP_CHECK(hipEventRecord(c->det_ev[slot], c->det_stream));
    };
    auto collect = [&](int o, int slot) {
        const int B = std::min(N, o + batch) - o;
        HIP_CHECK(hipEventSynchronize(c->det_ev[slot]));
        const uint8_t* hb = c->h_cand2[slot].as<uint8_t>();
        const int* h_counts = reinterpret_cast<const int*>(hb);
        const CandRec* h_cands = reinterpret_cast<const CandRec*>(hb + cnt_bytes);
        const CandRec* d_cands = reinterpret_cast<const CandRec*>(c->s_cand2[slot].as<uint8_t>() + cnt_bytes);
        screen_verdict(c, h_counts + B);
        for (int b = 0; b < B; ++b)
            if (h_counts[b] > cap) {
                HIP_CHECK(hipStreamSynchronize(c->det_stream));
                throw CandOverflow(h_counts[b]);
            }
        std::vector<std::vector<CandRec>> big(B);
        bool any_big = false;
        for (int b = 0; b < B; ++b)
            if (h_counts[b] > PF) {
                big[b].resize(h_counts[b]);
                HIP_CHECK(hipMemcpyAsync(big[b].data(), d_cands + (size_t)b * cap, (size_t)h_counts[b] * sizeof(CandRec), hipMemcpyDeviceToHost, c->det_stream));
                any_big = true;
            }
        if (any_big) HIP_CHECK(hipStreamSynchronize(c->det_stream));
        auto frames_of = [&](int b0, int b1) {
            std::vector<RawDet> sorted_raw;
            for (int b = b0; b < b1; ++b) {
                const int n = h_counts[b];
                std::vector<RawDet>& dst = nms ? sorted_raw : raw_sorted[o + b];
                decode_candidates(m, upsample, n <= PF ? h_cands + (size_t)b * PF : big[b].data(), n, dst);
// ... 43 lines not shown
```

### pyannote-video_amd/csrc/detect_ml.h

```cpp
#pragma once
#include "pvf_internal.h"
#include "fhog_dev.h"

#define ML_MAX 32
struct LvDesc {
    int h, w, rb;
    int cells_nr, cells_nc, visible_nr, visible_nc;
    int fh, fw, hog_nr, hog_nc;
    int fwp;
    int feat_bx, score_bx;
    int valid_score;
    int roll_nseg, roll_rows;
    int strips, chunks, chunk_rows, fused_tasks;
    long long img_off, img_stride;
    long long feat_off, feat_stride;
};
struct MlStarts { int nl; int b0[ML_MAX + 1]; };

#define FEAT_PAD_COLS 52
__host__ __device__ __forceinline__ size_t feat_at(int row, int j, int col, int fwp) { return (((size_t)row * 8 + j) * fwp + col) * 4; }

struct ScoreParams { float thresh[8]; int n_filters; int level; int cap; };
struct CandRec { float score; int32_t filter, level, r, c; };

#define SCR_SG 4
#define SCR_GROUP_COLS 48
#define SCR_TAIL_CELLS 9
#define SCR_FILTER_COLS 10
static_assert((SCR_GROUP_COLS - 1) + SCR_TAIL_CELLS - (SCR_FILTER_COLS - 1) <= FEAT_PAD_COLS,
              "FEAT_PAD_COLS: the screening pass's tail read leaves a feature row's zero columns");
struct ScreenItem { int32_t lv, b, c_base, r_base, out_rows, ng; };
enum { SCR_CURSOR = 0, SCR_FLAGGED = 1, SCR_VIOLATION = 2, SCR_CTL_INTS = 4 };

struct ScreenPlan {
    ScreenItem* d_items = nullptr;
    int n_items = 0;
    bool usable = false;
    ~ScreenPlan() { if (d_items) (void)hipFree(d_items); }
    ScreenPlan() = default;
    ScreenPlan(const ScreenPlan&) = delete;
    ScreenPlan& operator=(const ScreenPlan&) = delete;
};
void screen_plan_build(ScreenPlan& sp, const std::vector<LvDesc>& lv, int B);
void screen_launch(Ctx* c, const ScreenPlan& sp, const LvDesc* d_lv, int B, const float* feat, const ScoreParams& thr, int* d_counts,
                   CandRec* d_cands, int* ctl);
void screen_prepare_model(DetectorModel& d, const float* w);
```

### pyannote-video_amd/csrc/pvf_internal.h

```cpp
#pragma once
#include <hip/hip_runtime.h>
#include <cstdint>
#include <cstdio>
#include <cstring>
#include <deque>
#include <map>
#include <atomic>
#include <memory>
#include <mutex>
#include <stdexcept>
#include <string>
#include <unordered_map>
#include <vector>
#include "../../include/pvface.h"

#define PVF_FHOG_STRIDE 32

struct PvfError : std::runtime_error { using std::runtime_error::runtime_error; };
struct CandOverflow : PvfError { int needed; explicit CandOverflow(int n) : PvfError("detector: candidate buffer overflow"), needed(n) {} };
struct ScreenRetry : PvfError { ScreenRetry() : PvfError("detector: screening pass gave up") {} };

#define HIP_CHECK(expr)                                                                              \
    do {                                                                                             \
        hipError_t _e = (expr);                                                                      \
// ... 56 lines not shown
        if (busy[cur]) { HIP_CHECK(hipEventSynchronize(ev[cur])); busy[cur] = false; }
        buf[cur].ensure(bytes);
        return buf[cur].p;
    }
    void sent(hipStream_t st)
    {
        if (!ev[cur]) HIP_CHECK(hipEventCreateWithFlags(&ev[cur], hipEventDisableTiming));
        HIP_CHECK(hipEventRecord(ev[cur], st));
        busy[cur] = true;
    }
    ~StageRing() { for (auto e : ev) if (e) (void)hipEventDestroy(e); }
};

struct Tensor {
    std::string name;
    int dtype = 0;
    std::vector<int64_t> dims;
    std::vector<uint8_t> data;
    size_t numel() const { size_t n = 1; for (auto d : dims) n *= (size_t)d; return n; }
    const float* f32() const { return reinterpret_cast<const float*>(data.data()); }
    const int32_t* i32() const { return reinterpret_cast<const int32_t*>(data.data()); }
    const double* f64() const { return reinterpret_cast<const double*>(data.data()); }
};
std::map<std::string, Tensor> pvf_read_container(const char* path);
std::map<std::string, Tensor> pvf_read_model(const char* path, int kind);

struct Frame {
    const uint8_t* d = nullptr;
    int h = 0, w = 0;
    bool owned = false;
    bool pooled = false;
    hipEvent_t ready = nullptr;
};

struct ProfFamily {
    std::vector<std::pair<hipEvent_t, hipEvent_t>> pending;
    double total_ms = 0;
    int64_t launches = 0;
};

struct DetectorModel {
    bool loaded = false;
    int n_filters = 0, frows = 0, fcols = 0, cell = 0, padding = 0, win_w = 0, win_h = 0, min_w = 0, min_h = 0, max_levels = 0;
    double nms_iou = 0, nms_covered = 0;
    std::vector<float> thresh;
    float* d_w = nullptr;
    float* d_bmfma4 = nullptr;
    uint16_t* d_bscreen = nullptr;
    double screen_scale = 1.0;
    double screen_bound[8] = {0, 0, 0, 0, 0, 0, 0, 0};
};

struct ShapeModel {
    bool loaded = false;
    int n_cascades = 0, n_trees = 0, n_parts = 0, n_pix = 0, depth = 0;
    float* d_initial = nullptr;
    int32_t* d_anchor = nullptr;
    float* d_deltas = nullptr;
    int32_t* d_idx1 = nullptr;
    int32_t* d_idx2 = nullptr;
    float* d_thresh = nullptr;
    float* d_leaves = nullptr;
};

struct ConvLayer {
    int cin, cout, k, stride, pad;
    float* d_w;
    float* d_bias;
    float* d_gamma;
    float* d_beta;
    float* d_frag = nullptr;
    int w_exp = 0;
    uint32_t* d_wsplit = nullptr;
};

struct EmbedModel {
    bool loaded = false;
    int chip_size = 150;
    double chip_padding = 0.25;
    std::vector<float> mean_shape;
    std::vector<ConvLayer> convs;
    float* d_fc = nullptr;
    float* d_blob = nullptr;
    float* d_stem = nullptr;
};

struct TrackerTables {
    bool set = false;
    double* d_mask64 = nullptr;
    double* d_mask_scale = nullptr;
    double* d_tw64 = nullptr;
    double* d_tw32 = nullptr;
    double alpha_pow_m16 = 0, ln_alpha = 0;
};

struct Tracker {
    double* d_state = nullptr;
    int* share = nullptr;
    double pos[4] = {0, 0, 0, 0};
    double prev_pos[4] = {0, 0, 0, 0};
    bool started = false;
    bool pending = false;
};
constexpr size_t TRK_A = 0;
constexpr size_t TRK_B = TRK_A + (size_t)32 * 64 * 64 * 2;
constexpr size_t TRK_AS = TRK_B + (size_t)64 * 64;
constexpr size_t TRK_BS = TRK_AS + (size_t)512 * 32 * 2;
constexpr size_t TRK_POS = TRK_BS + 32;
constexpr size_t TRK_DOUBLES = TRK_POS + 4;
constexpr size_t TRKF_PLANE = (size_t)64 * 64;
constexpr size_t TRKF_A = 5 * TRKF_PLANE * sizeof(float);
constexpr size_t TRKF_BYTES = TRKF_A + TRKF_PLANE;
#define TRKF_SLOT(q) ((((q) & 511) << 3) | ((q) >> 9))

struct ChipJob {
    const uint8_t* img; int h, w;
    int bx0, by0, sw, sh, levels;
    double m[4], b[2];
    int rows, cols;
    bool empty;
};
struct ChipDetails { double l, t, r, b, cs, sn; int rows, cols; };

struct Ctx {
    int device = 0;
    hipStream_t stream = nullptr;
    hipStream_t det_stream = nullptr;
    DetectorModel det;
    ShapeModel shape;
    EmbedModel emb;
    TrackerTables ttab;
    std::unordered_map<uint64_t, Frame> frames;
    std::unordered_map<uint64_t, std::unique_ptr<Tracker>> trackers;
    std::vector<double*> tracker_pool;
    std::atomic<uint64_t> next_id{1};
    std::recursive_mutex api_mu;
    std::recursive_mutex det_mu;
    std::mutex frames_mu;
    std::mutex prof_mu;
    bool prof_on = false;
    std::map<std::string, ProfFamily> prof;
    std::vector<hipEvent_t> event_pool;
    DevBuf s_grad, s_pyr, s_hist, s_norm, s_feat, s_cand, s_misc, s_chip, s_chip_pyr, s_act0, s_act1, s_act2, s_trk0, s_trk1, s_trk2, s_trkfeat, s_clu0, s_clu1;
    HostBuf h_cand, h_misc;
    StageRing stage;
    DevBuf s_cand2[2], s_fptr[2];
    HostBuf h_cand2[2], h_fptr[2];
    hipEvent_t det_ev[2] = {nullptr, nullptr};
    int det_slot = 0;
    int det_cand_cap = 8192;
    bool det_screen = true, det_screen_suspended = false, screen_attr_set = false;
    int screen_list_cap = 1 << 20;
    DevBuf s_screen;
    int64_t screen_batches = 0, screen_listed = 0, screen_retries = 0;
    double screen_pipe_err = -1;
    bool screen_pipe_flushes_subnormals = false;
    bool emb_split = true, emb_probe_done = false;
    DevBuf s_emb_flags, s_emb_redo;
    int64_t emb_split_faces = 0, emb_reruns = 0;
    double emb_pipe_err = -1;
    int n_cu = 256;
    struct PoolBuf { uint8_t* p; hipEvent_t free_after; hipEvent_t free_after_det; };
    std::map<size_t, std::deque<PoolBuf>> frame_pool;
    size_t frame_pool_bytes = 0;
    void* ingest_rings = nullptr;
    void* render_state = nullptr;
    struct MlPlanCache* ml_plans = nullptr;
    std::map<std::vector<int>, std::unique_ptr<DevBuf>> resize_tabs;
    const void* feat_ring_owner = nullptr;
    uint8_t* d_orient_lut = nullptr;
    uint8_t* d_wrap_lut = nullptr;
    DevBuf s_orb_set, s_orb_work;
    int orb_n = 0, orb_cap = 0;

    Frame frame(uint64_t id)
    {
        std::lock_guard<std::mutex> lk(frames_mu);
        auto it = frames.find(id);
        if (it == frames.end()) throw PvfError("unknown frame handle");
        Frame& f = it->second;
        if (f.ready) {
            HIP_CHECK(hipStreamWaitEvent(stream, f.ready, 0));
            HIP_CHECK(hipStreamWaitEvent(det_stream, f.ready, 0));
            (void)hipEventDestroy(f.ready);
            f.ready = nullptr;
        }
        return f;
    }
    uint8_t* take_frame_buffer(size_t bytes, hipStream_t writer)
    {
        PoolBuf b{nullptr, nullptr, nullptr};
        {
            std::lock_guard<std::mutex> lk(frames_mu);
            auto& v = frame_pool[bytes];
            if (!v.empty()) { b = v.front(); v.pop_front(); frame_pool_bytes -= bytes; }
        }
        if (!b.p) {
            HIP_CHECK(hipMalloc((void**)&b.p, bytes));
            return b.p;
        }
        for (hipEvent_t e : {b.free_after, b.free_after_det}) {
            if (!e) continue;
            if (writer) HIP_CHECK(hipStreamWaitEvent(writer, e, 0));
            else HIP_CHECK(hipEventSynchronize(e));
            (void)hipEventDestroy(e);
        }
        return b.p;
    }
    void pool_give(uint8_t* p, size_t bytes)
    {
        hipEvent_t e = nullptr, e2 = nullptr;
        HIP_CHECK(hipEventCreateWithFlags(&e, hipEventDisableTiming));
        HIP_CHECK(hipEventRecord(e, stream));
        HIP_CHECK(hipEventCreateWithFlags(&e2, hipEventDisableTiming));
        HIP_CHECK(hipEventRecord(e2, det_stream));
        frame_pool[bytes].push_back(PoolBuf{p, e, e2});
        frame_pool_bytes += bytes;
    }
    uint64_t add_frame(const Frame& f)
    {
        const uint64_t id = next_id++;
        std::lock_guard<std::mutex> lk(frames_mu);
        frames[id] = f;
        return id;
    }
    Tracker& tracker(uint64_t id)
    {
        auto it = trackers.find(id);
        if (it == trackers.end()) throw PvfError("unknown tracker handle");
        return *it->second;
    }
};

struct ProfScope {
    Ctx* c; ProfFamily* f = nullptr; hipEvent_t a = nullptr, b = nullptr; hipStream_t s = nullptr; bool ranged = false;
    ProfScope(Ctx* ctx, const char* family, hipStream_t on = nullptr);
    ~ProfScope();
};

Ctx* pvf_ctx(pvf_handle h);
void pvf_set_error(const char* msg);

struct RawDet { float score; int32_t filter, level, r, c, l, t, rr, b; };
void det_run_batch(Ctx* c, const std::vector<Frame>& frames, int upsample, double adjust,
                   std::vector<std::vector<RawDet>>& raw_sorted);
void det_run_many(Ctx* c, const std::vector<Frame>& frames, int batch, int upsample, double adjust,
                  std::vector<std::vector<RawDet>>& raw_sorted, bool nms = false);
void ml_plans_free(Ctx* c);
void ingest_free_all(Ctx* c);
struct ResizeTab { std::vector<int32_t> idx; std::vector<int16_t> coef; };
ResizeTab linear_table(int in, int out);
void render_free_all(Ctx* c);
void det_nms(const DetectorModel& m, const std::vector<RawDet>& sorted, std::vector<RawDet>& out);
void det_pyramid_level(Ctx* c, const Frame& f, int upsample, int level, std::vector<uint8_t>* out, int* h, int* w);
void det_level_features(Ctx* c, const Frame& f, int upsample, int level, std::vector<float>* out, int* fh, int* fw);
void det_level_plan(Ctx* c, const Frame& f, int upsample, int level, int32_t out[8]);
void det_pyramid_batch(Ctx* c, const std::vector<Frame>& frames, int upsample);
void fhog_debug(Ctx* c, const uint8_t* himg, int h, int w, int cell, int pad_r, int pad_c, std::vector<float>& out, int* fh, int* fw);
void fhog_device(Ctx* c, const uint8_t* d_img, int n, int h, int w, int cell, int pad_r, int pad_c, float* d_feat,
                 DevBuf& hist, DevBuf& norm, size_t img_stride_in = 0);
void fhog1_compact(Ctx* c, const uint8_t* d_chips, int n, uint8_t* d_rec);
void fhog_scale_chips(Ctx* c, const uint8_t* d_chips, int n, float* d_feat);
void fhog_dims(int ih, int iw, int cell, int pad_r, int pad_c, int* fh, int* fw);
ChipJob chip_plan(const Frame& f, const ChipDetails& d);
void chip_extract_batch(Ctx* c, const std::vector<ChipJob>& jobs, uint8_t* d_out );
void transform_batch(Ctx* c, const std::vector<ChipJob>& jobs, uint8_t* d_out);
void ert_run(Ctx* c, const std::vector<Frame>& frames, const pvf_rect_i32* boxes, int n, int32_t* pts);
void face_chip_details(const EmbedModel& m, const int32_t* pts68, ChipDetails* out);
void resnet_forward(Ctx* c, const uint8_t* d_chips, int n, float* h_out);
void conv_layer_upload(ConvLayer& L, const float* w, const float* bias, const float* gamma, const float* beta);
void conv_layer_free(ConvLayer& L);
#define EMB_STAGES 30
struct EmbedTap { int stage; float* h_out; int dims[3]; };
void resnet_debug_stage(Ctx* c, const uint8_t* d_chips, int n, bool split, EmbedTap* tap, int* h_flags);
void resnet_debug_conv(Ctx* c, const int32_t* geom, const float* in, const float* w, const float* bias, const float* gamma, const float* beta,
                       const float* skip, bool split, bool force_generic, float* out, int32_t* flags);
void resnet_debug_head(Ctx* c, const float* x, int n, int hw, float* out);
void dsst_start_many(Ctx* c, const std::vector<Tracker*>& t, const std::vector<Frame>& f, const double* boxes);
void dsst_clone_many(Ctx* c, const std::vector<Tracker*>& src, const std::vector<Tracker*>& dst);
double* tracker_state_alloc(Ctx* c);
void shot_dfd(Ctx* c, const std::vector<Frame>& frames, int ow, int oh, const float* tables22, double* dfd, uint8_t* gray_out, float* flow_out);
std::vector<int> orb_level_quota();
void orb_extract(Ctx* c, const std::vector<Frame>& frames, int ow, int oh, int cap, int32_t* counts, float* kp_out, uint8_t* desc_out);
void orb_match_counts(Ctx* c, const uint8_t* desc, const int32_t* nrows, int n_sets, int cap, const int32_t* pairs, int64_t n_pairs, int32_t* out);
void dsst_update_many(Ctx* c, const std::vector<Tracker*>& t, const std::vector<Frame>& f, double* psr, double* boxes_out, int mode = 0);
void overlap_matrix_host(const double* a, int na, const double* b, int nb, double ratio, double* out);
void munkres_host(const double* cost, int n, int32_t* row_to_col);
struct PairInput {
    const double* X = nullptr;
    const float* emb = nullptr; int64_t emb_stride = 0; int n_src = 0; const int32_t* order = nullptr; int decimals = -1; bool emb_on_device = false;
};
struct PairOutput { double* out = nullptr; bool on_device = false; bool compact = false; };
void pair_mean_dist_dev(Ctx* c, const PairInput& in, int N, int dim, const int32_t* row_start, int T, const PairOutput& out, double** d_D_keep,
                        int t0, int t1, int metric, bool mirror);
void mirror_upper_dev(Ctx* c, double* dD, int T);
int hac_dev(Ctx* c, double* d_D, const int32_t* row_start, int T, double threshold, int32_t* labels, double* merge_log);
```

### pyannote-video_amd/csrc/screen.hip

```cpp
#include "detect_ml.h"
#include <algorithm>
#include <cmath>
#include <cstring>

typedef _Float16 f16x8 __attribute__((ext_vector_type(8)));
typedef _Float16 f16x2 __attribute__((ext_vector_type(2)));

struct ScreenParams { float flag_at[8]; float lim_lo, lim_hi; int n_items, list_cap; };

#define SCR_B_BYTES (10 * 12 * 64 * 16)
#define SCR_M_STRIDE (12 * 64 * 16)

__device__ __forceinline__ uint32_t pk_f16(float a, float b)
{
    return __builtin_bit_cast(uint32_t, __builtin_amdgcn_cvt_pkrtz(a, b));
}

template <int NG>
__device__ __forceinline__ void screen_walk(const ScreenItem t, const LvDesc* __restrict__ lv, const float* __restrict__ feat_base,
                                            const uint8_t* s_b, const float th_lane, int* __restrict__ ctl, uint2* __restrict__ list,
                                            const int list_cap, u32x4& mx)
{
    constexpr int RSRC_FLAGS = 0x00020000;
    constexpr int FR = 10, FC = 10;
    static_assert(FC == SCR_FILTER_COLS, "detect_ml.h: SCR_FILTER_COLS is this kernel's filter width");
    const int lane = threadIdx.x & 63, i = lane & 15, kq = lane >> 4;
    const int fw = lv[t.lv].fw;
    const long long feat_off = lv[t.lv].feat_off, feat_stride = lv[t.lv].feat_stride;
    const int fwp = lv[t.lv].fwp;
    const float* fb = feat_base + feat_off + (size_t)t.b * feat_stride + feat_at(t.r_base, 0, t.c_base, fwp);
    const int row_bytes = (8 * fwp - t.c_base) * 16;
    const int fh_in = t.out_rows + FR - 1;
    const int c1 = fw - (FC - FC / 2 - 1);
    const int voff = i * 48 + kq * 2 * fwp * 16;
    const int voff2 = voff + fwp * 16;
    const int voff_t = i < 3 ? voff : 0x40000000, voff2_t = i < 3 ? voff2 : 0x40000000;
    f32x4 acc[10][NG];
#pragma unroll
    for (int q = 0; q < 10; ++q)
#pragma unroll
        for (int g = 0; g < NG; ++g) acc[q][g] = (f32x4){0.f, 0.f, 0.f, 0.f};
    const uint8_t* b_lo = s_b + lane * 16;
    const uint8_t* b_hi = s_b + lane * 16 + 5 * SCR_M_STRIDE;
    auto load_cls = [&](int row, int cls, u32x4 (&raw)[NG + 1][2]) {
        const __amdgpu_buffer_rsrc_t rs = __builtin_amdgcn_make_buffer_rsrc((void*)(fb + (size_t)row * 8 * fwp * 4), 0,
                                                                            row < fh_in ? row_bytes : 0, RSRC_FLAGS);
#pragma unroll
        for (int g = 0; g <= NG; ++g) {
            raw[g][0] = __builtin_amdgcn_raw_buffer_load_b128(rs, (g < NG ? voff : voff_t) + cls * 16 + g * 768, 0, 0);
            raw[g][1] = __builtin_amdgcn_raw_buffer_load_b128(rs, (g < NG ? voff2 : voff2_t) + cls * 16 + g * 768, 0, 0);
        }
    };
    auto cvt_frag = [&](const u32x4 (&r)[2]) -> u32x4 {
        u32x4 o;
        o.x = pk_f16(__uint_as_float(r[0].x), __uint_as_float(r[0].y)); o.y = pk_f16(__uint_as_float(r[0].z), __uint_as_float(r[0].w));
        o.z = pk_f16(__uint_as_float(r[1].x), __uint_as_float(r[1].y)); o.w = pk_f16(__uint_as_float(r[1].z), __uint_as_float(r[1].w));
#pragma unroll
        for (int k = 0; k < 4; ++k) mx[k] = __builtin_bit_cast(uint32_t, __builtin_elementwise_max(__builtin_bit_cast(f16x2, mx[k]), __builtin_bit_cast(f16x2, o[k])));
        return o;
    };
    auto shift_bases = [&](u32x4 (&a)[NG + 1]) {
#pragma unroll
        for (int g = 0; g <= NG; ++g) {
#pragma unroll
            for (int e = 0; e < 4; ++e) {
                int fill = 0;
                if (g < NG) fill = __builtin_amdgcn_update_dpp(0, (int)a[g + 1][e], 0x11F , 0xf, 0xf, true);
                a[g][e] = (uint32_t)__builtin_amdgcn_update_dpp(fill, (int)a[g][e], 0x101 , 0xf, 0xf, false);
            }
        }
    };
    auto emit = [&](const f32x4 (&a)[NG], int r_out) {
        float vm = a[0][0];
#pragma unroll
        for (int g = 0; g < NG; ++g)
#pragma unroll
            for (int e = 0; e < 4; ++e) vm = fmaxf(vm, a[g][e]);
        const bool hit = vm >= th_lane;
        if (r_out >= 0 && __builtin_amdgcn_ballot_w64(hit) != 0) {
            const int jc = lane & 15;
            const int sft = jc / 5, f = jc % 5;
            const int r = t.r_base + r_out + FR / 2;
#pragma unroll
            for (int g = 0; g < NG; ++g)
#pragma unroll
                for (int e = 0; e < 4; ++e) {
                    const int cc = t.c_base + 48 * g + 3 * (4 * kq + e) + sft + FC / 2;
                    if (a[g][e] >= th_lane && cc < c1) {
                        const int idx = atomicAdd(&ctl[SCR_FLAGGED], 1);
                        if (idx < list_cap) list[idx] = make_uint2((uint32_t)t.b, ((uint32_t)t.lv << 27) | ((uint32_t)f << 24) | ((uint32_t)r << 12) | (uint32_t)cc);
                    }
                }
        }
    };

    u32x4 A[3][NG + 1];
    {
        u32x4 raw[NG + 1][2];
#pragma unroll
        for (int cls = 0; cls < 3; ++cls) {
            load_cls(0, cls, raw);
#pragma unroll
            for (int g = 0; g <= NG; ++g) A[cls][g] = cvt_frag(raw[g]);
        }
    }
    auto b_frag = [&](int q, int j) -> u32x4 {
        return *reinterpret_cast<const u32x4*>((q < 5 ? b_lo + q * SCR_M_STRIDE : b_hi + (q - 5) * SCR_M_STRIDE) + j * 1024);
    };
    u32x4 bn[10];
#pragma unroll
    for (int q = 0; q < 10; ++q) bn[q] = b_frag(q, 0);
    for (int s = 0; s < fh_in; ++s) {
        u32x4 An[3][NG + 1];
        u32x4 raw[NG + 1][2];
        f32x4 done[NG];
#pragma unroll
        for (int j = 0; j < 12; ++j) {
            const int cls = j % 3;
            if (j > 0 && cls == 0) {
#pragma unroll
                for (int k = 0; k < 3; ++k) shift_bases(A[k]);
            }
            if (j % 4 == 0) load_cls(s + 1, j / 4, raw);
            u32x4 bc[10];
#pragma unroll
            for (int q = 0; q < 10; ++q) bc[q] = bn[q];
#pragma unroll
            for (int q = 0; q < 10; ++q) bn[q] = b_frag(q, (j + 1) % 12);
#pragma unroll
            for (int q = 9; q >= 0; --q) {
#pragma unroll
                for (int g = 0; g < NG; ++g) {
                    const f32x4 v = __builtin_amdgcn_mfma_f32_16x16x32_f16(__builtin_bit_cast(f16x8, A[cls][g]), __builtin_bit_cast(f16x8, bc[q]), acc[q][g], 0, 0, 0);
                    if (j < 11) acc[q][g] = v;
                    else if (q == 9) done[g] = v;
                    else acc[q + 1][g] = v;
                }
            }
            if (j % 4 == 3) {
#pragma unroll
                for (int g = 0; g <= NG; ++g) An[j / 4][g] = cvt_frag(raw[g]);
            }
            __builtin_amdgcn_sched_barrier(0);
        }
#pragma unroll
        for (int g = 0; g < NG; ++g) acc[0][g] = (f32x4){0.f, 0.f, 0.f, 0.f};
        emit(done, s - (FR - 1));
#pragma unroll
        for (int cls = 0; cls < 3; ++cls)
#pragma unroll
            for (int g = 0; g <= NG; ++g) A[cls][g] = An[cls][g];
    }
}

__global__ void __launch_bounds__(256) __attribute__((amdgpu_waves_per_eu(1, 1)))
score_screen_k(const ScreenItem* __restrict__ items, const LvDesc* __restrict__ lv, const float* __restrict__ feat_base,
               const u32x4* __restrict__ Bh, ScreenParams sp, int* __restrict__ ctl, uint2* __restrict__ list)
{
    extern __shared__ __attribute__((aligned(16))) uint8_t s_b[];
    for (int k = threadIdx.x; k < SCR_B_BYTES / 16; k += 256) reinterpret_cast<u32x4*>(s_b)[k] = Bh[k];
    __syncthreads();
    const int lane = threadIdx.x & 63;
    const int jc = lane & 15, f = jc % 5;
    float th_lane = sp.flag_at[0];
    th_lane = f == 1 ? sp.flag_at[1] : th_lane;
    th_lane = f == 2 ? sp.flag_at[2] : th_lane;
    th_lane = f == 3 ? sp.flag_at[3] : th_lane;
    th_lane = f == 4 ? sp.flag_at[4] : th_lane;
    th_lane = jc < 15 ? th_lane : 3.0e38f;
    u32x4 mx = {0u, 0u, 0u, 0u};
    for (;;) {
        int it = 0;
        if (lane == 0) it = atomicAdd(&ctl[SCR_CURSOR], 1);
        it = __builtin_amdgcn_readfirstlane(it);
        if (it >= sp.n_items) break;
        ScreenItem t;
        t.lv = __builtin_amdgcn_readfirstlane(items[it].lv); t.b = __builtin_amdgcn_readfirstlane(items[it].b);
        t.c_base = __builtin_amdgcn_readfirstlane(items[it].c_base); t.r_base = __builtin_amdgcn_readfirstlane(items[it].r_base);
        t.out_rows = __builtin_amdgcn_readfirstlane(items[it].out_rows); t.ng = __builtin_amdgcn_readfirstlane(items[it].ng);
        switch (t.ng) {
        case 1: screen_walk<1>(t, lv, feat_base, s_b, th_lane, ctl, list, sp.list_cap, mx); break;
        case 2: screen_walk<2>(t, lv, feat_base, s_b, th_lane, ctl, list, sp.list_cap, mx); break;
        case 3: screen_walk<3>(t, lv, feat_base, s_b, th_lane, ctl, list, sp.list_cap, mx); break;
        default: screen_walk<4>(t, lv, feat_base, s_b, th_lane, ctl, list, sp.list_cap, mx); break;
        }
    }
    auto lo16 = [](uint32_t v) { return (float)__builtin_bit_cast(f16x2, v)[0]; };
    auto hi16 = [](uint32_t v) { return (float)__builtin_bit_cast(f16x2, v)[1]; };
    const float m_lo = fmaxf(fmaxf(lo16(mx.x), hi16(mx.x)), lo16(mx.y));
    const float m_hi = fmaxf(fmaxf(hi16(mx.y), fmaxf(lo16(mx.z), hi16(mx.z))), fmaxf(lo16(mx.w), hi16(mx.w)));
    const float lim_hi = (lane >> 4) == 3 ? sp.lim_hi : sp.lim_lo;
    if (m_lo > sp.lim_lo || m_hi > lim_hi) atomicOr(&ctl[SCR_VIOLATION], 1);
}

__global__ void __launch_bounds__(256) score_list_k(const uint2* __restrict__ list, const int* __restrict__ ctl, int list_cap,
                                                    const LvDesc* __restrict__ lv, const float* __restrict__ feat_base,
                                                    const float* __restrict__ W, ScoreParams sp, int* __restrict__ counts, CandRec* __restrict__ cands)
{
    constexpr int FR = 10, FC = 10;
    const int n = min(ctl[SCR_FLAGGED], list_cap);
    for (int e = blockIdx.x * 256 + threadIdx.x; e < n; e += gridDim.x * 256) {
        const uint2 q = list[e];
        const int b = (int)q.x;
        const int l = (int)(q.y >> 27), f = (int)((q.y >> 24) & 7), r = (int)((q.y >> 12) & 4095), cc = (int)(q.y & 4095);
        const int fwp = lv[l].fwp;
        const float* fp = feat_base + lv[l].feat_off + (size_t)b * lv[l].feat_stride + feat_at(r - FR / 2, 0, cc - FC / 2, fwp);
        const float* wp = W + (size_t)f * FR * FC * PVF_FHOG_STRIDE;
        float acc = 0.0f;
        for (int m = 0; m < FR; ++m)
            for (int nn = 0; nn < FC; ++nn) {
                const f32x4* fv = reinterpret_cast<const f32x4*>(fp + feat_at(m, 0, nn, fwp));
                const f32x4* wv = reinterpret_cast<const f32x4*>(wp + ((size_t)m * FC + nn) * PVF_FHOG_STRIDE);
#pragma unroll
                for (int k = 0; k < 8; ++k) {
                    const f32x4 a = fv[(size_t)k * fwp], w = wv[k];
                    acc = fmaf(a[0], w[0], acc); acc = fmaf(a[1], w[1], acc); acc = fmaf(a[2], w[2], acc);
                    if (k < 7) acc = fmaf(a[3], w[3], acc);
                }
            }
        const float th = sp.thresh[f];
        if (acc >= th) {
            const int idx = atomicAdd(&counts[b], 1);
            if (idx < sp.cap) {
                CandRec rec;
                rec.score = acc - th; rec.filter = f; rec.level = l; rec.r = r; rec.c = cc;
                cands[(size_t)b * sp.cap + idx] = rec;
            }
        }
    }
}

__global__ void screen_probe_k(const u32x4* __restrict__ a, const u32x4* __restrict__ b, int steps, float* __restrict__ d, int* __restrict__ moved)
{
    const int lane = threadIdx.x;
    f32x4 acc = {0.f, 0.f, 0.f, 0.f};
    for (int s = 0; s < steps; ++s)
        acc = __builtin_amdgcn_mfma_f32_16x16x32_f16(__builtin_bit_cast(f16x8, a[s * 64 + lane]), __builtin_bit_cast(f16x8, b[s * 64 + lane]), acc, 0, 0, 0);
    for (int e = 0; e < 4; ++e) d[lane * 4 + e] = acc[e];
    const int fill = __builtin_amdgcn_update_dpp(0, lane + 1000, 0x11F, 0xf, 0xf, false);
    moved[lane] = __builtin_amdgcn_update_dpp(fill, lane + 100, 0x101, 0xf, 0xf, false);
}

static uint16_t f32_to_f16_rne(float v)
{
    uint32_t x;
    memcpy(&x, &v, 4);
    const uint32_t sign = (x >> 16) & 0x8000u;
    const int32_t e = (int32_t)((x >> 23) & 0xff) - 127 + 15;
    uint32_t man = x & 0x7fffffu;
    if (((x >> 23) & 0xff) == 0xff) return (uint16_t)(sign | 0x7c00u | (man ? 0x200u : 0));
    if (e >= 31) return (uint16_t)(sign | 0x7c00u);
    if (e <= 0) {
        if (e < -10) return (uint16_t)sign;
        man |= 0x800000u;
        const int shift = 14 - e;
        const uint32_t half = man >> shift, rem = man & ((1u << shift) - 1), mid = 1u << (shift - 1);
        uint32_t h = half;
        if (rem > mid || (rem == mid && (half & 1))) ++h;
        return (uint16_t)(sign | h);
    }
    uint32_t h = ((uint32_t)e << 10) | (man >> 13);
    const uint32_t rem = man & 0x1fffu;
    if (rem > 0x1000u || (rem == 0x1000u && (h & 1))) ++h;
    return (uint16_t)(sign | h);
}
static double f16_to_f64(uint16_t h)
{
    const int s = (h >> 15) & 1, e = (h >> 10) & 31, m = h & 1023;
    double v;
    if (e == 0) v = std::ldexp((double)m, -24);
    else if (e == 31) v = INFINITY;
    else v = std::ldexp((double)(m | 1024), e - 25);
    return s ? -v : v;
}

static const double SCR_FM_LO = 0.4004, SCR_FM_HI = 0.8492;
static const float SCR_LIM_LO = 0.400146484375f , SCR_LIM_HI = 0.8486328125f ;

void screen_prepare_model(DetectorModel& d, const float* w)
{
    PVF_REQUIRE(d.n_filters == 5 && d.frows == 10 && d.fcols == 10, "screening: 5 filters of 10 x 10 cells");
    double wmax = 0;
    for (size_t k = 0; k < (size_t)d.n_filters * 10 * 10 * 32; ++k) wmax = std::max(wmax, std::fabs((double)w[k]));
    PVF_REQUIRE(std::isfinite(wmax), "detector weights are not finite");
    int sh = 0;
    if (wmax > 0) { int ex; (void)std::frexp(wmax, &ex); sh = 7 - ex; }
    sh = std::max(-100, std::min(100, sh));
    const double SCR_SCALE = std::ldexp(1.0, sh);
    d.screen_scale = SCR_SCALE;
    std::vector<uint16_t> bh((size_t)10 * 12 * 64 * 8, 0);
    for (int m = 0; m < 10; ++m)
        for (int j = 0; j < 12; ++j)
            for (int l = 0; l < 64; ++l) {
                const int jc = l & 15, kq = l >> 4;
                if (jc >= 15) continue;
                const int sft = jc / 5, f = jc % 5, n = j - sft;
                if (n < 0 || n >= 10) continue;
                for (int e = 0; e < 8; ++e) {
                    const int p = 8 * kq + e;
                    if (p >= 31) continue;
                    bh[(((size_t)m * 12 + j) * 64 + l) * 8 + e] = f32_to_f16_rne((float)((double)w[(((size_t)f * 10 + m) * 10 + n) * 32 + p] * SCR_SCALE));
                }
            }
    if (d.d_bscreen) (void)hipFree(d.d_bscreen);
    HIP_CHECK(hipMalloc((void**)&d.d_bscreen, bh.size() * sizeof(uint16_t)));
    HIP_CHECK(hipMemcpy(d.d_bscreen, bh.data(), bh.size() * sizeof(uint16_t), hipMemcpyHostToDevice));
    const double u = std::ldexp(1.0, -24);
    for (int f = 0; f < d.n_filters; ++f) {
        double e_w = 0, e_f = 0, e_sub = 0, a_h = 0, a_w = 0;
// ... 7 lines not shown
                    e_f += std::fabs(wh) * std::max(fm * std::ldexp(1.0, -10), std::ldexp(1.0, -14));
                    a_h += fm * std::fabs(wh);
                    a_w += fm * std::fabs(wv);
                    if (wh != 0.0 && std::fabs(wh) * SCR_SCALE < std::ldexp(1.0, -14)) e_sub += fm * std::fabs(wh);
                }
        const double e_pipe = 3200.0 * std::ldexp(1.0, -22) * a_h * (1.0 + std::ldexp(1.0, -10));
        const double e_chain = 3100.0 * u / (1.0 - 3100.0 * u) * a_w;
        d.screen_bound[f] = 1.02 * (e_w + e_f + e_sub + e_pipe + e_chain) + 1e-6;
    }
}

void screen_plan_build(ScreenPlan& sp, const std::vector<LvDesc>& lv, int B)
{
    int seg = 16;
    for (int cand : {512, 160, 96, 64, 48, 32, 24}) {
        long long n = 0;
        for (const LvDesc& d : lv)
            if (d.valid_score) n += (long long)((d.fw - 9 + 48 * SCR_SG - 1) / (48 * SCR_SG)) * ((d.fh - 9 + cand - 1) / cand) * B;
        if (n >= 3 * 1024) { seg = cand; break; }
    }
    if (getenv("PVF_SCREEN_SEG") && atoi(getenv("PVF_SCREEN_SEG")) > 0) seg = std::max(2, atoi(getenv("PVF_SCREEN_SEG")));
    std::vector<ScreenItem> items;
    sp.usable = lv.size() <= 32;
    for (const LvDesc& d : lv) sp.usable = sp.usable && d.fh < 4096 && d.fw < 4096;
    if (!sp.usable) return;
    for (int l = 0; l < (int)lv.size(); ++l) {
        const LvDesc& d = lv[l];
        if (!d.valid_score) continue;
        const int out_c = d.fw - 9, out_r = d.fh - 9;
        const int nseg = (out_r + seg - 1) / seg, rows = (out_r + nseg - 1) / nseg;
        for (int c0 = 0; c0 < out_c; c0 += 48 * SCR_SG)
            for (int r0 = 0; r0 < out_r; r0 += rows)
                for (int b = 0; b < B; ++b)
                    items.push_back(ScreenItem{l, b, c0, r0, std::min(rows, out_r - r0), std::min(SCR_SG, (out_c - c0 + 47) / 48)});
    }
    for (const ScreenItem& it : items)
        PVF_REQUIRE(it.ng >= 1 && it.c_base + SCR_GROUP_COLS * it.ng + SCR_TAIL_CELLS - 1 < lv[it.lv].fwp,
                    "screening plan: a strip's tail read passes the FEAT_PAD_COLS zero columns of its feature row");
    std::stable_sort(items.begin(), items.end(), [](const ScreenItem& a, const ScreenItem& b) { return a.ng * (a.out_rows + 9) > b.ng * (b.out_rows + 9); });
    if (sp.d_items) (void)hipFree(sp.d_items);
    sp.d_items = nullptr;
    sp.n_items = (int)items.size();
    if (items.empty()) return;
    HIP_CHECK(hipMalloc((void**)&sp.d_items, items.size() * sizeof(ScreenItem)));
    HIP_CHECK(hipMemcpy(sp.d_items, items.data(), items.size() * sizeof(ScreenItem), hipMemcpyHostToDevice));
}

static void screen_probe(Ctx* c)
{
    const int steps = 100;
    const size_t nh = (size_t)steps * 64 * 8;
    std::vector<uint16_t> ha(nh), hb(nh);
    uint8_t* dev = nullptr;
    const size_t fb = nh * 2;
    HIP_CHECK(hipMalloc((void**)&dev, 2 * fb + 64 * 4 * sizeof(float) + 64 * sizeof(int)));
    float* d_d = reinterpret_cast<float*>(dev + 2 * fb);
    int* d_m = reinterpret_cast<int*>(dev + 2 * fb + 64 * 4 * sizeof(float));
    float hd[256];
    int hm[64];
    auto A = [&](int row, int K) -> uint16_t& { return ha[((size_t)(K >> 5) * 64 + ((K >> 3) & 3) * 16 + row) * 8 + (K & 7)]; };
    auto B = [&](int K, int col) -> uint16_t& { return hb[((size_t)(K >> 5) * 64 + ((K >> 3) & 3) * 16 + col) * 8 + (K & 7)]; };
    auto run = [&]() {
        HIP_CHECK(hipMemcpy(dev, ha.data(), fb, hipMemcpyHostToDevice));
        HIP_CHECK(hipMemcpy(dev + fb, hb.data(), fb, hipMemcpyHostToDevice));
        hipLaunchKernelGGL(screen_probe_k, dim3(1), dim3(64), 0, c->det_stream, reinterpret_cast<const u32x4*>(dev), reinterpret_cast<const u32x4*>(dev + fb),
                           steps, d_d, d_m);
        HIP_CHECK(hipMemcpyAsync(hd, d_d, sizeof hd, hipMemcpyDeviceToHost, c->det_stream));
        HIP_CHECK(hipMemcpyAsync(hm, d_m, sizeof hm, hipMemcpyDeviceToHost, c->det_stream));
        HIP_CHECK(hipStreamSynchronize(c->det_stream));
    };
    auto worst_rel = [&]() {
        double worst = 0;
        for (int l = 0; l < 64; ++l)
            for (int e = 0; e < 4; ++e) {
                const int col = l & 15, row = 4 * (l >> 4) + e;
                double sum = 0, mag = 0;
                for (int K = 0; K < 32 * steps; ++K) {
                    const double t = f16_to_f64(A(row, K)) * f16_to_f64(B(K, col));
                    sum += t; mag += std::fabs(t);
                }
                if (mag > 0) worst = std::max(worst, std::fabs((double)hd[l * 4 + e] - sum) / mag);
            }
        return worst;
    };
    uint32_t rs = 12345u;
    auto rnd = [&]() { rs = rs * 1664525u + 1013904223u; return (double)(rs >> 8) / 16777216.0; };
    double worst = 0;
    for (int s = 0; s < steps; ++s)
        for (int l = 0; l < 64; ++l)
            for (int e = 0; e < 8; ++e) {
                ha[((size_t)s * 64 + l) * 8 + e] = f32_to_f16_rne((float)(0.05 + 0.8 * rnd()));
                const double sgn = ((l & 15) < 8 || ((s + e) & 1)) ? 1.0 : -1.0;
                hb[((size_t)s * 64 + l) * 8 + e] = f32_to_f16_rne((float)(sgn * (1.0 + 25.0 * rnd())));
            }
    run();
    worst = std::max(worst, worst_rel());
    bool dpp_ok = true;
    for (int l = 0; l < 64; ++l) dpp_ok = dpp_ok && hm[l] == ((l & 15) < 15 ? l + 101 : l - 15 + 1000);
    for (int order = 0; order < 2; ++order) {
        std::vector<double> av(32 * steps), bv(32 * steps);
        for (int K = 0; K < 32 * steps; ++K) {
            av[K] = std::ldexp(1.0 + rnd(), -14 + (int)(rnd() * 21.999));
            bv[K] = std::ldexp(1.0 + rnd(), -14 + (int)(rnd() * 21.999));
        }
        std::vector<int> idx(32 * steps);
        for (int K = 0; K < 32 * steps; ++K) idx[K] = K;
        if (order == 1) std::sort(idx.begin(), idx.end(), [&](int x, int y) { return av[x] * bv[x] > av[y] * bv[y]; });
        for (int K = 0; K < 32 * steps; ++K)
            for (int r = 0; r < 16; ++r) {
                const int kk = idx[(K + 97 * r) % (32 * steps)], kr = idx[(32 * steps - 1 - K + 97 * r) % (32 * steps)];
                A(r, K) = f32_to_f16_rne((float)av[r < 8 ? kk : kr]);
                B(K, r) = f32_to_f16_rne((float)bv[r < 8 ? kk : kr]);
            }
        run();
        worst = std::max(worst, worst_rel());
    }
    {
        const DetectorModel& m = c->det;
        std::vector<float> w((size_t)5 * 10 * 10 * 32);
        HIP_CHECK(hipMemcpy(w.data(), m.d_w, w.size() * sizeof(float), hipMemcpyDeviceToHost));
        std::fill(ha.begin(), ha.end(), (uint16_t)0);
        std::fill(hb.begin(), hb.end(), (uint16_t)0);
        for (int K = 0; K < 3100; ++K) {
            const int cellp = K / 31, p = K % 31;
            const double fm = p < 27 ? (double)SCR_LIM_LO : (double)SCR_LIM_HI;
            for (int col = 0; col < 16; ++col)
                B(K, col) = f32_to_f16_rne((float)((double)w[((size_t)(col % 5) * 100 + cellp) * 32 + p] * m.screen_scale));
            for (int row = 0; row < 16; ++row) {
                double f;
                switch (row & 3) {
                case 0: f = fm; break;
                case 1: f = (K & 1) ? fm : 0.0; break;
                case 2: f = (K & 1) ? 0.0 : fm; break;
                default: f = fm * rnd(); break;
                }
                A(row, K) = f32_to_f16_rne((float)f);
            }
        }
        run();
        worst = std::max(worst, worst_rel());
    }
    {
        for (size_t i = 0; i < nh; ++i) { ha[i] = 0x3c00u ; hb[i] = 0x0010u ; }
        run();
        c->screen_pipe_flushes_subnormals = !(hd[0] > 0.0f);
        if (!c->screen_pipe_flushes_subnormals) worst = std::max(worst, worst_rel());
    }
    (void)hipFree(dev);
    c->screen_pipe_err = worst;
    PVF_REQUIRE(worst <= 3200.0 * std::ldexp(1.0, -22), "screening: v_mfma_f32_16x16x32_f16 does not accumulate as the error bound of the screening pass assumes on this device");
    PVF_REQUIRE(dpp_ok, "screening: v_mov_b32_dpp row_shl:1 / row_shr:15 do not move data as the screening kernel expects on this device");
}

void screen_launch(Ctx* c, const ScreenPlan& plan, const LvDesc* d_lv, int B, const float* feat, const ScoreParams& thr, int* d_counts,
                   CandRec* d_cands, int* ctl)
{
    const DetectorModel& m = c->det;
    if (plan.n_items == 0) return;
    if (!c->screen_attr_set) {
        screen_probe(c);
        HIP_CHECK(hipFuncSetAttribute(reinterpret_cast<const void*>(score_screen_k), hipFuncAttributeMaxDynamicSharedMemorySize, SCR_B_BYTES));
        c->screen_attr_set = true;
    }
    ScreenParams sp;
    for (int f = 0; f < 8; ++f) {
        if (f < m.n_filters) {
            const float at = (float)(((double)thr.thresh[f] - m.screen_bound[f]) * m.screen_scale);
            sp.flag_at[f] = std::nextafterf(at, -INFINITY);
        }
        else sp.flag_at[f] = 3.0e38f;
    }
    sp.lim_lo = SCR_LIM_LO; sp.lim_hi = SCR_LIM_HI;
    if (const char* e = getenv("PVF_SCREEN_LIMIT_SCALE")) {
        sp.lim_lo *= (float)atof(e); sp.lim_hi *= (float)atof(e);
    }
    sp.n_items = plan.n_items;
    sp.list_cap = c->screen_list_cap;
    c->s_screen.ensure((size_t)sp.list_cap * sizeof(uint2) + 64);
    uint2* list = c->s_screen.as<uint2>();
    const int grid = std::min(c->n_cu, (plan.n_items + 3) / 4);
    hipLaunchKernelGGL(score_screen_k, dim3(grid), dim3(256), SCR_B_BYTES, c->det_stream, plan.d_items, d_lv, feat,
                       reinterpret_cast<const u32x4*>(m.d_bscreen), sp, ctl, list);
    hipLaunchKernelGGL(score_list_k, dim3(256), dim3(256), 0, c->det_stream, list, ctl, sp.list_cap, d_lv, feat, m.d_w, thr, d_counts, d_cands);
}
```

### pyannote-video_amd/pyannote_video_amd/_lib.py

```python
import ctypes as C
import os
import numpy as np

_HERE = os.path.dirname(os.path.abspath(__file__))
LIB_PATH = os.environ.get("PVF_LIBRARY") or os.path.join(_HERE, "libpvface.so")

_lib = None


class PvfError(RuntimeError):
    pass


class OrbCapError(PvfError):

    def __init__(self, message, needed):
        PvfError.__init__(self, message)
        self.needed = int(needed)


class Rect(C.Structure):
    _fields_ = [("left", C.c_int32), ("top", C.c_int32), ("right", C.c_int32), ("bottom", C.c_int32)]


H = C.c_uint64
P = C.c_void_p
_SIGS = {
    "pvf_last_error": (C.c_char_p, []),
    "pvf_version": (C.c_int32, []),
    "pvf_device_count": (C.c_int32, [P]),
    "pvf_ctx_create": (C.c_int32, [C.c_int32, P]),
    "pvf_ctx_create_prio": (C.c_int32, [C.c_int32, C.c_int32, P]),
    "pvf_ctx_destroy": (C.c_int32, [H]),
    "pvf_sync": (C.c_int32, [H]),
    "pvf_load_detector": (C.c_int32, [H, C.c_char_p]),
    "pvf_load_shape_predictor": (C.c_int32, [H, C.c_char_p]),
    "pvf_load_embedder": (C.c_int32, [H, C.c_char_p]),
    "pvf_model_tensor": (C.c_int32, [C.c_char_p, C.c_int32, C.c_char_p, P, C.c_int64, P]),
    "pvf_set_tracker_tables": (C.c_int32, [H, P, P, P, P, C.c_double, C.c_double]),
    "pvf_frame_upload": (C.c_int32, [H, P, C.c_int32, C.c_int32, C.c_int64, P]),
    "pvf_frame_wrap_device": (C.c_int32, [H, P, C.c_int32, C.c_int32, P]),
    "pvf_frame_release": (C.c_int32, [H, H]),
    "pvf_frame_release_many": (C.c_int32, [H, P, C.c_int32]),
    "pvf_frame_pool_trim": (C.c_int32, [H, C.c_int64, P]),
    "pvf_mem_info": (C.c_int32, [H, P, P]),
    "pvf_frame_device_ptr": (C.c_int32, [H, H, P]),
    "pvf_ingest_create": (C.c_int32, [H, C.c_int32, C.c_int32, C.c_int32, P]),
    "pvf_ingest_destroy": (C.c_int32, [H, H]),
    "pvf_ingest_acquire": (C.c_int32, [H, H, P, P]),
    "pvf_ingest_submit": (C.c_int32, [H, H, C.c_int32, P]),
    "pvf_ingest_wait": (C.c_int32, [H, H]),
    "pvf_ingest_create_yuv": (C.c_int32, [H, C.c_int32, C.c_int32, C.c_int32, C.c_int32, C.c_int32, P]),
    "pvf_frame_from_yuv": (C.c_int32, [H, P, C.c_int64, P, P, C.c_int64, C.c_int32, C.c_int32, C.c_int32, C.c_int32, C.c_int32, P]),
    "pvf_frame_resize": (C.c_int32, [H, H, C.c_int32, C.c_int32, P]),
    "pvf_render_batch": (C.c_int32, [H, P, C.c_int32, C.c_int32, C.c_int32, C.c_int32, P, P, P, C.c_int64, P, C.c_int32]),
    "pvf_egress_create": (C.c_int32, [H, C.c_int32, C.c_int32, C.c_int32, C.c_int32, P]),
    "pvf_egress_destroy": (C.c_int32, [H, H]),
    "pvf_egress_submit": (C.c_int32, [H, H, H, P, C.c_int32, P, C.c_int64, P]),
    "pvf_egress_wait": (C.c_int32, [H, H, C.c_int32, P]),
    "pvf_egress_release": (C.c_int32, [H, H, C.c_int32]),
    "pvf_debug_render_rgb": (C.c_int32, [H, H, C.c_int32, C.c_int32, P, C.c_int32, P, C.c_int64, P]),
    "pvf_detect": (C.c_int32, [H, H, C.c_int32, C.c_double, P, P, C.c_int32, P]),
    "pvf_detect_batch": (C.c_int32, [H, P, C.c_int32, C.c_int32, C.c_double, P, P, P, C.c_int32]),
    "pvf_detect_many": (C.c_int32, [H, P, C.c_int32, C.c_int32, C.c_int32, C.c_double, P, P, P, C.c_int32]),
    "pvf_detector_screening": (C.c_int32, [H, C.c_int32, C.c_int32]),
    "pvf_detector_screening_stats": (C.c_int32, [H, P, P, P, P, P]),
    "pvf_embedder_split": (C.c_int32, [H, C.c_int32]),
    "pvf_embedder_split_stats": (C.c_int32, [H, P, P, P]),
    "pvf_tracker_create": (C.c_int32, [H, P]),
    "pvf_tracker_destroy": (C.c_int32, [H, H]),
    "pvf_tracker_create_many": (C.c_int32, [H, C.c_int32, P]),
    "pvf_tracker_destroy_many": (C.c_int32, [H, P, C.c_int32]),
    "pvf_tracker_clone_many": (C.c_int32, [H, P, C.c_int32, P]),
    "pvf_tracker_start": (C.c_int32, [H, H, H, P]),
    "pvf_tracker_update": (C.c_int32, [H, H, H, P]),
    "pvf_tracker_position": (C.c_int32, [H, H, P]),
    "pvf_tracker_start_many": (C.c_int32, [H, P, P, P, C.c_int32]),
    "pvf_tracker_update_many": (C.c_int32, [H, P, P, C.c_int32, P, P]),
    "pvf_tracker_update_many_deferred": (C.c_int32, [H, P, P, C.c_int32, P, P]),
    "pvf_tracker_commit_many": (C.c_int32, [H, P, P, C.c_int32]),
    "pvf_overlap_matrix": (C.c_int32, [P, C.c_int32, P, C.c_int32, C.c_double, P]),
    "pvf_munkres": (C.c_int32, [P, C.c_int32, P]),
    "pvf_associate": (C.c_int32, [P, C.c_int32, P, C.c_int32, C.c_double, P]),
    "pvf_landmarks": (C.c_int32, [H, P, P, C.c_int32, P]),
    "pvf_embed": (C.c_int32, [H, P, P, C.c_int32, P]),
    "pvf_landmarks_embed": (C.c_int32, [H, P, P, C.c_int32, P, P]),
    "pvf_embed_chips": (C.c_int32, [H, P, C.c_int32, P]),
    "pvf_face_chips": (C.c_int32, [H, P, P, C.c_int32, P]),
    "pvf_pair_mean_dist": (C.c_int32, [H, P, C.c_int32, C.c_int32, P, C.c_int32, P]),
    "pvf_pair_mean_dist_metric": (C.c_int32, [H, P, C.c_int32, C.c_int32, P, C.c_int32, C.c_int32, P]),
    "pvf_pair_mean_dist_rows": (C.c_int32, [H, P, C.c_int32, C.c_int32, P, C.c_int32, C.c_int32, C.c_int32, P]),
    "pvf_pair_upper_rows": (C.c_int32, [H, P, C.c_int32, C.c_int32, P, C.c_int32, C.c_int32, C.c_int32, P]),
    "pvf_lane_create": (C.c_int32, [C.c_int32, P, P, C.c_int32, C.c_double, C.c_double, C.c_int32, P]),
    "pvf_lane_destroy": (C.c_int32, [H]),
    "pvf_lane_feed_plan": (C.c_int32, [H, C.c_int32, C.c_int32, P, P, P, P]),
    "pvf_lane_advance": (C.c_int32, [H, P, P, C.c_int32, P, P, P, C.c_int32, P, P]),
    "pvf_lane_take_dead": (C.c_int32, [H, P, C.c_int32, P]),
    "pvf_lane_edges": (C.c_int32, [H, P, P, P, P, P, P, C.c_int32]),
    "pvf_shot_tracks": (C.c_int32, [H, H, P, C.c_int32, C.c_double, P, C.c_int32, P, P, C.c_int32, P]),
    "pvf_track_rows": (C.c_int32, [P, C.c_int64, C.c_int32, C.c_int32, C.c_int32, C.c_int32, P, P]),
    "pvf_round_decimals": (C.c_int32, [P, C.c_int64, C.c_int32, P]),
    "pvf_cluster_dist": (C.c_int32, [H, P, P, C.c_int32, C.c_double, P, P, P]),
    "pvf_cluster_tracks": (C.c_int32, [H, P, C.c_int32, C.c_int32, P, C.c_int32, C.c_double, P, P, P]),
    "pvf_cluster_upper": (C.c_int32, [H, P, C.c_int32, P, C.c_int32, C.c_double, P, P, P]),
    "pvf_cluster_tracks_f32": (C.c_int32, [H, P, C.c_int64, C.c_int32, C.c_int32, P, C.c_int32, C.c_int32, P, C.c_int32, C.c_int32, C.c_double, P, P, P]),
    "pvf_pair_upper_rows_f32": (C.c_int32, [H, P, C.c_int64, C.c_int32, C.c_int32, P, C.c_int32, C.c_int32, P, C.c_int32, C.c_int32, C.c_int32, P, C.c_int32]),
    "pvf_format_rows": (C.c_int32, [P, P, P, C.c_int64, C.c_int32, C.c_int32, P, C.c_int64, P]),
    "pvf_round_rows": (C.c_int32, [P, C.c_int64, C.c_int32, P]),
    "pvf_parse_rows": (C.c_int32, [C.c_char_p, C.c_int64, P, C.c_int64, P, P]),
    "pvf_prof_enable": (C.c_int32, [H, C.c_int32]),
    "pvf_prof_reset": (C.c_int32, [H]),
    "pvf_prof_get": (C.c_int32, [H, C.c_char_p, P, P]),
    "pvf_debug_pyramid_level": (C.c_int32, [H, H, C.c_int32, C.c_int32, P, P, P]),
    "pvf_debug_pyramid_batch": (C.c_int32, [H, P, C.c_int32, C.c_int32]),
    "pvf_debug_level_features": (C.c_int32, [H, H, C.c_int32, C.c_int32, P, P, P]),
    "pvf_debug_level_plan": (C.c_int32, [H, H, C.c_int32, C.c_int32, P]),
    "pvf_debug_fhog": (C.c_int32, [H, P, C.c_int32, C.c_int32, C.c_int32, C.c_int32, C.c_int32, P, P, P]),
    "pvf_debug_detect_raw": (C.c_int32, [H, H, C.c_int32, C.c_double, P, P, C.c_int32, P]),
    "pvf_debug_detect_raw_many": (C.c_int32, [H, P, C.c_int32, C.c_int32, C.c_int32, C.c_double, P, P, C.c_int64, P]),
    "pvf_debug_extract_chip": (C.c_int32, [H, H, P, C.c_double, C.c_double, C.c_int32, C.c_int32, P]),
    "pvf_debug_tracker_state": (C.c_int32, [H, H, P, P, P]),
    "pvf_debug_tracker_scale_state": (C.c_int32, [H, H, P, P]),
    "pvf_debug_embed_stage": (C.c_int32, [H, P, C.c_int32, C.c_int32, C.c_int32, P, P, P]),
    "pvf_debug_conv": (C.c_int32, [H, P, P, P, P, P, P, P, C.c_int32, C.c_int32, P, P]),
    "pvf_debug_embed_head": (C.c_int32, [H, P, C.c_int32, C.c_int32, P]),
    "pvf_shot_dfd": (C.c_int32, [H, P, C.c_int32, C.c_int32, C.c_int32, P, P, P, P]),
    "pvf_orb_extract": (C.c_int32, [H, P, C.c_int32, C.c_int32, C.c_int32, C.c_int32, P, P, P]),
    "pvf_orb_match_counts": (C.c_int32, [H, P, P, C.c_int32, C.c_int32, P, C.c_int64, P]),
}
EXPORTS = sorted(_SIGS)


def lib():
    global _lib
    if _lib is None:
        if not os.path.exists(LIB_PATH):
            raise PvfError("libpvface.so is not built (%s): run `python -c 'import __graft_entry__ as g; g.build()'`; "
                           "there is no CPU fallback" % LIB_PATH)
        l = C.CDLL(LIB_PATH)
        for name, (res, args) in _SIGS.items():
            fn = getattr(l, name)
            fn.restype = res
            fn.argtypes = args
        _lib = l
    return _lib


def check(rc):
    if rc != 0:
        raise PvfError(lib().pvf_last_error().decode("utf-8", "replace"))


def ptr(a):
    return a.ctypes.data_as(C.c_void_p) if a is not None else None


def handles(seq):
    return np.ascontiguousarray(np.asarray(seq, dtype=np.uint64))


def device_count():
    n = C.c_int32(0)
    check(lib().pvf_device_count(C.byref(n)))
    return n.value


def model_tensor(path, kind, name, dtype):
    n = C.c_int64(0)
    check(lib().pvf_model_tensor(str(path).encode(), int(kind), name.encode(), None, 0, C.byref(n)))
    out = np.zeros(n.value // np.dtype(dtype).itemsize, dtype)
    check(lib().pvf_model_tensor(str(path).encode(), int(kind), name.encode(), ptr(out), out.nbytes, C.byref(n)))
    return out


def overlap_matrix(a, b, ratio):
    a = np.ascontiguousarray(a, np.float64).reshape(-1, 4)
    b = np.ascontiguousarray(b, np.float64).reshape(-1, 4)
    out = np.zeros((len(a), len(b)), np.float64)
    check(lib().pvf_overlap_matrix(ptr(a), len(a), ptr(b), len(b), float(ratio), ptr(out)))
    return out


import threading as _threading
_assoc_tls = _threading.local()
_ASSOC_KEEP = 256


def associate(trackers, detections, ratio):
    na, nb = len(trackers), len(detections)
    key = (na, nb)
    cache = getattr(_assoc_tls, "buf", None)
    if cache is None:
        cache = _assoc_tls.buf = {}
    buf = cache.get(key)
    if buf is None:
        if len(cache) >= _ASSOC_KEEP:
            cache.clear()
        buf = cache[key] = ((C.c_double * (4 * na))(), (C.c_double * (4 * nb))(), (C.c_int32 * max(na, 1))())
    a, b, out = buf
    k = 0
    for box in trackers:
        a[k], a[k + 1], a[k + 2], a[k + 3] = box
        k += 4
    k = 0
    for box in detections:
        b[k], b[k + 1], b[k + 2], b[k + 3] = box
        k += 4
    check(lib().pvf_associate(a, na, b, nb, float(ratio), out))
    return [(t, d) for t, d in enumerate(out[:na]) if d >= 0]


def round_decimals(x, decimals):
    x = np.ascontiguousarray(x, np.float64)
    out = np.empty_like(x)
    if x.size:
        check(lib().pvf_round_decimals(ptr(x), x.size, int(decimals), ptr(out)))
    return out


def track_rows(boxes, det_width, det_height, width, height):
    b = np.ascontiguousarray(boxes, np.int32).reshape(-1, 4)
    fb = np.empty(b.shape, np.float64)
    pb = np.empty(b.shape, np.int32)
    if len(b):
        check(lib().pvf_track_rows(ptr(b), len(b), int(det_width), int(det_height), int(width), int(height), ptr(fb), ptr(pb)))
    return fb, pb


def format_rows(t, identifier, values, decimals=5):
    t = np.ascontiguousarray(t, np.float64)
    ident = np.ascontiguousarray(identifier, np.int64)
    v = np.ascontiguousarray(values, np.float64)
    v = v.reshape(len(t), -1) if len(t) else v.reshape(0, max(v.shape[-1], 1) if v.ndim else 1)
    cap = len(t) * (64 + 42 * v.shape[1])
    buf = np.empty(max(cap, 1), np.uint8)
    n = C.c_int64(0)
    check(lib().pvf_format_rows(ptr(t), ptr(ident), ptr(v), len(t), v.shape[1], int(decimals), ptr(buf), cap, C.byref(n)))
    return buf[:n.value].tobytes()


def round_rows(x, decimals=5):
    x = np.ascontiguousarray(x, np.float32)
    out = np.empty(x.shape, np.float64)
    check(lib().pvf_round_rows(ptr(x), x.size, int(decimals), ptr(out)))
    return out


def parse_rows(text):
    n = len(text)
    rows, cols = C.c_int64(0), C.c_int32(0)
    for cap in (n // 6 + 16, n // 2 + 1):
        out = np.empty(cap, np.float64)
        if lib().pvf_parse_rows(text, n, ptr(out), out.size, C.byref(rows), C.byref(cols)) == 0:
            return out[:rows.value * cols.value].reshape(rows.value, cols.value)
        if b"too small" not in lib().pvf_last_error():
            break
    raise PvfError(lib().pvf_last_error().decode("utf-8", "replace"))


def munkres(cost):
    cost = np.ascontiguousarray(cost, np.float64)
    n = cost.shape[0]
    assert cost.shape == (n, n)
    out = np.zeros(n, np.int32)
    check(lib().pvf_munkres(ptr(cost), n, ptr(out)))
    return [(i, int(out[i])) for i in range(n)]
```

### pyannote-video_amd/pyannote_video_amd/runtime.py

```python
import contextlib
import ctypes as C
import threading
import itertools
import operator
import numpy as np
from . import _lib
from ._lib import check, ptr, handles
from . import models as _models
from .y4m import YuvFrame, chroma_shape


class DeviceFrame(object):
    __slots__ = ("ctx", "handle", "height", "width", "keep", "transient", "__weakref__")

    def __init__(self, ctx, handle, height, width, keep=None, transient=False):
        self.ctx, self.handle, self.height, self.width, self.keep = ctx, handle, height, width, keep
        self.transient = transient

    @property
    def shape(self):
        return (self.height, self.width, 3)

    def release(self):
        if self.handle is not None and self.ctx._h is not None:
# ... 356 lines not shown
        _, p, text = _render.pack_primitives([prims])
        out = np.empty((int(height), int(width), 3), np.uint8)
        check(self._l.pvf_debug_render_rgb(self._h, self.stage(frame).handle, int(width), int(height), ptr(p), len(p), ptr(text), len(text),
                                           ptr(out)))
        return out

    def frame_from_yuv_device(self, y_ptr, y_pitch, u_ptr, v_ptr, c_pitch, height, width, layout="420", matrix="601", full_range=False,
                              c_step=1):
        h = C.c_uint64(0)
        check(self._l.pvf_frame_from_yuv(self._h, C.c_void_p(int(y_ptr)), int(y_pitch), C.c_void_p(int(u_ptr)), C.c_void_p(int(v_ptr)),
                                         int(c_pitch), int(c_step), int(height), int(width), _yuv_layout(layout),
                                         _yuv_flags(matrix, full_range), C.byref(h)))
        return DeviceFrame(self, h.value, int(height), int(width))

    def frame_from_yuv_torch(self, y, u, v=None, layout="420", matrix="601", full_range=False):
        for t in (y, u) + (() if v is None else (v,)):
            assert t.is_cuda and t.element_size() == 1 and t.stride(-1) == 1
        if v is None:
            assert u.dim() == 3 and u.shape[2] == 2 and (u.shape[1] == 1 or u.stride(1) == 2)
            return self.frame_from_yuv_device(y.data_ptr(), y.stride(0), u.data_ptr(), u.data_ptr() + 1, u.stride(0), y.shape[0], y.shape[1],
                                              layout, matrix, full_range, c_step=2)
        assert u.dim() == 2 and v.dim() == 2 and u.shape == v.shape and u.stride(0) == v.stride(0)
        return self.frame_from_yuv_device(y.data_ptr(), y.stride(0), u.data_ptr(), v.data_ptr(), u.stride(0), y.shape[0], y.shape[1],
                                          layout, matrix, full_range)

    def stage(self, rgb):
        if isinstance(rgb, DeviceFrame):
            return rgb
        key = (id(rgb), rgb.__array_interface__["data"][0] if hasattr(rgb, "__array_interface__") else 0)
        with self._stage_mu:
            f = self._staged.get(key)
            if f is None or f.keep is not rgb:
                f = self.upload(rgb)
                f.keep = rgb
                self._staged[key] = f
                self._staged_order.append(key)
                if not self._hold:
                    self._trim()
            return f

    def _trim(self):
        with self._stage_mu:
            while len(self._staged_order) > self.stage_capacity:
                old = self._staged_order.pop(0)
                g = self._staged.pop(old, None)
                if g is not None:
                    g.release()

    @contextlib.contextmanager
    def _staging(self):
        with self._stage_mu:
            self._hold += 1
        try:
            yield
        finally:
            with self._stage_mu:
                self._hold -= 1
                if not self._hold:
                    self._trim()

    def _handles(self, frames):
        if isinstance(frames, np.ndarray) and frames.dtype == np.uint64:
            return np.ascontiguousarray(frames)
        try:
            return np.fromiter(map(_handle_of, frames), dtype=np.uint64, count=len(frames))
        except AttributeError:
            return handles([self.stage(f).handle for f in frames])

    def frame_handles(self, frames):
        return self._handles(frames)

    def unstage_all(self):
        for f in self._staged.values():
            f.release()
        self._staged.clear()
        self._staged_order = []

    def detect_batch(self, frames, upsample=1, adjust_threshold=0.0, cap=256):
        n = len(frames)
        out = np.zeros((n, cap, 4), np.int32)
        scores = np.zeros((n, cap), np.float32)
        counts = np.zeros(n, np.int32)
        with self._staging():
            hs = self._handles(frames)
            check(self._l.pvf_detect_batch(self._h, ptr(hs), n, int(upsample), float(adjust_threshold), ptr(out), ptr(scores), ptr(counts), cap))
        if int(counts.max(initial=0)) >= cap:
            return self.detect_batch(frames, upsample, adjust_threshold, cap * 8)
        return _boxes_and_scores(out, scores, counts)

    def detect_many(self, frames, batch, upsample=1, adjust_threshold=0.0, cap=64, arrays=False):
        n = len(frames)
        out = np.zeros((n, cap, 4), np.int32)
        scores = np.zeros((n, cap), np.float32)
        counts = np.zeros(n, np.int32)
        with self._staging():
            hs = self._handles(frames)
            check(self._l.pvf_detect_many(self._h, ptr(hs), n, int(batch), int(upsample), float(adjust_threshold), ptr(out), ptr(scores), ptr(counts), cap))
        if int(counts.max(initial=0)) >= cap:
            return self.detect_many(frames, batch, upsample, adjust_threshold, cap * 8, arrays)
        if arrays:
            m = int(counts.max(initial=0))
            return out[:, :m], scores[:, :m], counts
        return _boxes_and_scores(out, scores, counts)

    def detect(self, frame, upsample=1, adjust_threshold=0.0):
        return self.detect_batch([frame], upsample, adjust_threshold)[0]

    def detect_raw(self, frame, upsample=1, adjust_threshold=0.0, cap=65536):
        f = self.stage(frame)
        scores = np.zeros(cap, np.float32)
        meta = np.zeros((cap, 8), np.int32)
        n = C.c_int32(0)
        check(self._l.pvf_debug_detect_raw(self._h, f.handle, int(upsample), float(adjust_threshold), ptr(scores), ptr(meta), cap, C.byref(n)))
        k = min(n.value, cap)
        return [(float(scores[i]), int(meta[i, 0]), int(meta[i, 1]), int(meta[i, 2]), int(meta[i, 3]),
                 tuple(int(v) for v in meta[i, 4:8])) for i in range(k)]

    def detect_raw_many(self, frames, batch, upsample=1, adjust_threshold=0.0, cap=1 << 16):
        n = len(frames)
        counts = np.zeros(n, np.int32)
        total = C.c_int64(0)
        with self._staging():
            hs = self._handles(frames)
            while True:
                rows = np.zeros((cap, 5), np.int32)
                check(self._l.pvf_debug_detect_raw_many(self._h, ptr(hs), n, int(batch), int(upsample), float(adjust_threshold), ptr(counts), ptr(rows), cap, C.byref(total)))
                if total.value <= cap:
                    break
                cap = int(total.value)
        off = np.concatenate([[0], np.cumsum(counts)])
        return [rows[off[i]:off[i + 1]] for i in range(n)]

    def pyramid_batch(self, frames, upsample=1):
        with self._staging():
            hs = self._handles(frames)
            check(self._l.pvf_debug_pyramid_batch(self._h, ptr(hs), len(frames), int(upsample)))

    def pyramid_level(self, frame, upsample, level):
        f = self.stage(frame)
        oh, ow = C.c_int32(0), C.c_int32(0)
        check(self._l.pvf_debug_pyramid_level(self._h, f.handle, upsample, level, None, C.byref(oh), C.byref(ow)))
        out = np.zeros((oh.value, ow.value, 3), np.uint8)
        check(self._l.pvf_debug_pyramid_level(self._h, f.handle, upsample, level, ptr(out), C.byref(oh), C.byref(ow)))
        return out

    def level_features(self, frame, upsample, level):
        f = self.stage(frame)
        fh, fw = C.c_int32(0), C.c_int32(0)
        check(self._l.pvf_debug_level_features(self._h, f.handle, upsample, level, None, C.byref(fh), C.byref(fw)))
        out = np.zeros((fh.value, fw.value, 32), np.float32)
        if out.size:
            check(self._l.pvf_debug_level_features(self._h, f.handle, upsample, level, ptr(out), C.byref(fh), C.byref(fw)))
        return out

    def level_plan(self, frame, upsample, level):
        f = self.stage(frame)
        out = np.zeros(8, np.int32)
        check(self._l.pvf_debug_level_plan(self._h, f.handle, int(upsample), int(level), ptr(out)))
        return dict(zip(("h", "w", "hog_nr", "hog_nc", "chunk_rows", "chunks", "roll_rows", "roll_nseg"), (int(v) for v in out)))

    def fhog(self, img, cell, pad_r, pad_c):
        img = np.ascontiguousarray(img, np.uint8)
        fh, fw = C.c_int32(0), C.c_int32(0)
        check(self._l.pvf_debug_fhog(self._h, ptr(img), img.shape[0], img.shape[1], cell, pad_r, pad_c, None, C.byref(fh), C.byref(fw)))
        out = np.zeros((fh.value, fw.value, 32), np.float32)
        check(self._l.pvf_debug_fhog(self._h, ptr(img), img.shape[0], img.shape[1], cell, pad_r, pad_c, ptr(out), C.byref(fh), C.byref(fw)))
        return out

    def tracker_create(self):
        self.ensure_tracker_tables()
        h = C.c_uint64(0)
        check(self._l.pvf_tracker_create(self._h, C.byref(h)))
        return h.value

    def tracker_create_many(self, n, as_array=False):
        self.ensure_tracker_tables()
        out = np.zeros(int(n), np.uint64)
        if n:
            check(self._l.pvf_tracker_create_many(self._h, int(n), ptr(out)))
        return out if as_array else out.tolist()

    def tracker_clone_many(self, trks, as_array=False):
        out = np.zeros(len(trks), np.uint64)
        if len(trks):
            check(self._l.pvf_tracker_clone_many(self._h, ptr(handles(trks)), len(trks), ptr(out)))
        return out if as_array else out.tolist()

    def tracker_destroy_many(self, trks):
        if self._h is not None and len(trks):
            check(self._l.pvf_tracker_destroy_many(self._h, ptr(handles(trks)), len(trks)))

    def tracker_destroy(self, trk):
        if self._h is not None:
            check(self._l.pvf_tracker_destroy(self._h, trk))

    def tracker_start_many(self, trks, frames, boxes):
        if not len(trks):
            return
        b = np.ascontiguousarray(boxes, np.float64).reshape(-1, 4)
        with self._staging():
            check(self._l.pvf_tracker_start_many(self._h, ptr(handles(trks)), ptr(self._handles(frames)), ptr(b), len(trks)))

    def tracker_update_many(self, trks, frames, defer=False):
        n = len(trks)
        if not n:
            return np.zeros(0), np.zeros((0, 4))
        psr = np.zeros(n, np.float64)
        boxes = np.zeros((n, 4), np.float64)
        fn = self._l.pvf_tracker_update_many_deferred if defer else self._l.pvf_tracker_update_many
        with self._staging():
            check(fn(self._h, ptr(handles(trks)), ptr(self._handles(frames)), n, ptr(psr), ptr(boxes)))
        return psr, boxes

    def tracker_commit_many(self, trks, frames):
        n = len(trks)
        if n:
            with self._staging():
                check(self._l.pvf_tracker_commit_many(self._h, ptr(handles(trks)), ptr(self._handles(frames)), n))

    def tracker_position(self, trk):
        b = np.zeros(4, np.float64)
        check(self._l.pvf_tracker_position(self._h, trk, ptr(b)))
        return tuple(b.tolist())

    def tracker_state(self, trk):
        F = np.zeros((32, 64, 64, 2), np.float64)
        A = np.zeros((32, 64, 64, 2), np.float64)
        B = np.zeros((64, 64), np.float64)
        check(self._l.pvf_debug_tracker_state(self._h, trk, ptr(F), ptr(A), ptr(B)))
        return F, A, B

    def tracker_scale_state(self, trk):
        As = np.zeros((512, 32, 2), np.float64)
        Bs = np.zeros(32, np.float64)
        check(self._l.pvf_debug_tracker_scale_state(self._h, trk, ptr(As), ptr(Bs)))
        return As, Bs

    def landmarks(self, frames, boxes):
        n = len(boxes)
        pts = np.zeros((n, 68, 2), np.int32)
        if n == 0:
            return pts
        r = _rects(boxes, n)
        with self._staging():
            check(self._l.pvf_landmarks(self._h, ptr(self._handles(frames)), ptr(r), n, ptr(pts)))
        return pts

    def embed(self, frames, pts):
        pts = np.ascontiguousarray(pts, np.int32).reshape(-1, 68, 2)
        n = len(pts)
        out = np.zeros((n, 128), np.float32)
        if n == 0:
            return out
        with self._staging():
            check(self._l.pvf_embed(self._h, ptr(self._handles(frames)), ptr(pts), n, ptr(out)))
        return out

    def landmarks_embed(self, frames, boxes):
        n = len(boxes)
        pts = np.zeros((n, 68, 2), np.int32)
        out = np.zeros((n, 128), np.float32)
        if n == 0:
            return pts, out
        r = _rects(boxes, n)
        with self._staging():
            check(self._l.pvf_landmarks_embed(self._h, ptr(self._handles(frames)), ptr(r), n, ptr(pts), ptr(out)))
        return pts, out

    def face_chips(self, frames, pts):
        pts = np.ascontiguousarray(pts, np.int32).reshape(-1, 68, 2)
        n = len(pts)
        out = np.zeros((n, 150, 150, 3), np.uint8)
        with self._staging():
            check(self._l.pvf_face_chips(self._h, ptr(self._handles(frames)), ptr(pts), n, ptr(out)))
        return out

    def embed_chips(self, chips):
        chips = np.ascontiguousarray(chips, np.uint8).reshape(-1, 150, 150, 3)
        out = np.zeros((len(chips), 128), np.float32)
        check(self._l.pvf_embed_chips(self._h, ptr(chips), len(chips), ptr(out)))
        return out

    def extract_chip(self, frame, rect, cs, sn, rows, cols):
        f = self.stage(frame)
        r = np.asarray(rect, np.float64)
        out = np.zeros((rows, cols, 3), np.uint8)
        check(self._l.pvf_debug_extract_chip(self._h, f.handle, ptr(r), float(cs), float(sn), rows, cols, ptr(out)))
        return out

    EMBED_STAGES = 30

    def embed_stage(self, chips, stage, split):
        chips = np.ascontiguousarray(chips, np.uint8).reshape(-1, 150, 150, 3)
        n = len(chips)
        dims = np.zeros(3, np.int32)
        check(self._l.pvf_debug_embed_stage(self._h, None, n, 1 if split else 0, int(stage), None, ptr(dims), None))
        out = np.zeros((n,) + tuple(int(d) for d in dims), np.float32)
        flags = np.zeros(n, np.int32)
        check(self._l.pvf_debug_embed_stage(self._h, ptr(chips), n, 1 if split else 0, int(stage), ptr(out), ptr(dims), ptr(flags)))
        return out, flags

    def debug_conv(self, x, w, bias, gamma, beta, stride=1, pad=1, skip=None, skip_mode=0, out_hw=None, split=False, force_generic=False):
        x = np.ascontiguousarray(x, np.float32)
        w = np.ascontiguousarray(w, np.float32)
        B, H, W, cin = x.shape
        cout, wc, k, k2 = w.shape
# ... 228 lines not shown
```

Measured before the change: 4661.

## Emit packed f16 FHOG features in the FHOG kernel for the screening pass

When screening is enabled, the FHOG kernel now writes a second feature buffer in packed f16, in a layout matching the screening kernel's fragments, alongside the f32 features. The screening kernel reads these f16 features directly, halving its feature loads and dropping the per-load f32-to-f16 conversion. The exact f32 rescoring still reads the f32 buffer. The cost is extra stores and a second ring buffer written by the FHOG kernel, plus a debug API for inspecting the f16 features.

New measurement: 4660. No clear change (-0.0%).

```diff
diff --git a/include/pvface.h b/include/pvface.h
--- a/include/pvface.h
+++ b/include/pvface.h
@@ -163,6 +163,8 @@
 int32_t pvf_debug_pyramid_batch(pvf_handle ctx, const pvf_handle* frames, int32_t n, int32_t upsample);
 int32_t pvf_debug_level_features(pvf_handle ctx, pvf_handle frame, int32_t upsample, int32_t level,
                                  float* out, int32_t* fh, int32_t* fw);
+int32_t pvf_debug_level_features_f16(pvf_handle ctx, pvf_handle frame, int32_t upsample, int32_t level,
+                                     uint16_t* out, int32_t* fh, int32_t* fw, int32_t pad_kq, uint16_t* pad_out, int32_t* fwp);
 int32_t pvf_debug_level_plan(pvf_handle ctx, pvf_handle frame, int32_t upsample, int32_t level, int32_t* out8);
 int32_t pvf_debug_fhog(pvf_handle ctx, const uint8_t* img, int32_t h, int32_t w, int32_t cell, int32_t pad_r,
                        int32_t pad_c, float* out, int32_t* fh, int32_t* fw);
diff --git a/pyannote-video_amd/csrc/api.hip b/pyannote-video_amd/csrc/api.hip
--- a/pyannote-video_amd/csrc/api.hip
+++ b/pyannote-video_amd/csrc/api.hip
@@ -223,6 +223,21 @@
     det_level_features(c, c->frame(frame), upsample, level, out ? &buf : nullptr, &a, &b);
     *fh = a; *fw = b;
     if (out) memcpy(out, buf.data(), buf.size() * sizeof(float));
+    API_END
+}
+
+extern "C" int32_t pvf_debug_level_features_f16(pvf_handle h, pvf_handle frame, int32_t upsample, int32_t level, uint16_t* out, int32_t* fh, int32_t* fw,
+                                                int32_t pad_kq, uint16_t* pad_out, int32_t* fwp)
+{
+    API_BEGIN
+    ENTER_DET(c, h);
+    PVF_REQUIRE(fh && fw && fwp, "pvf_debug_level_features_f16: fh, fw or fwp is NULL");
+    std::vector<uint16_t> buf, pad;
+    int a = 0, b = 0, p = 0;
+    det_level_features_f16(c, c->frame(frame), upsample, level, out ? &buf : nullptr, &a, &b, pad_kq, pad_out ? &pad : nullptr, &p);
+    *fh = a; *fw = b; *fwp = p;
+    if (out) memcpy(out, buf.data(), buf.size() * sizeof(uint16_t));
+    if (pad_out) memcpy(pad_out, pad.data(), pad.size() * sizeof(uint16_t));
     API_END
 }
 
diff --git a/pyannote-video_amd/csrc/detect.hip b/pyannote-video_amd/csrc/detect.hip
--- a/pyannote-video_amd/csrc/detect.hip
+++ b/pyannote-video_amd/csrc/detect.hip
@@ -340,9 +340,10 @@
     return r;
 }
 
+template <bool F16>
 __global__ void __launch_bounds__(512) __attribute__((amdgpu_waves_per_eu(4, 4)))
 fhog_split_ml_k(MlStarts st, const LvDesc* __restrict__ lv, int B, const uint8_t* __restrict__ img_base, float* __restrict__ feat_base,
-                const uint8_t* __restrict__ lutw, int oy, int ox)
+                uint16_t* __restrict__ feat16_base, const uint8_t* __restrict__ lutw, int oy, int ox)
 {
     constexpr int RSRC_FLAGS = 0x00020000;
     extern __shared__ __attribute__((aligned(16))) uint32_t fs_lds[];
@@ -480,6 +481,18 @@
             if (lane >= 1 && lane <= FUSED_OUT && x < d.hog_nc) {
                 float4* dst = reinterpret_cast<float4*>(feat_base + d.feat_off + (size_t)b * d.feat_stride + feat_at(yh + oy, 0, x + ox, d.fwp));
                 const size_t step = (size_t)d.fwp;
+                u32x4* dst16 = nullptr;
+                if (F16) dst16 = reinterpret_cast<u32x4*>(feat16_base + d.feat_off + (size_t)b * d.feat_stride + feat16_at(yh + oy, 0, x + ox, d.fwp));
+                uint32_t h0 = 0u, h1 = 0u;
+                auto put = [&](const int j, const float a, const float b4, const float c4, const float d4) {
+                    *dst = make_float4(a, b4, c4, d4); dst += step;
+                    if (F16) {
+                        const uint32_t p0 = __builtin_bit_cast(uint32_t, __builtin_amdgcn_cvt_pkrtz(a, b4));
+                        const uint32_t p1 = __builtin_bit_cast(uint32_t, __builtin_amdgcn_cvt_pkrtz(c4, d4));
+                        if (j & 1) { *dst16 = (u32x4){h0, h1, p0, p1}; dst16 += step; }
+                        else { h0 = p0; h1 = p1; }
+                    }
+                };
                 const float eps = 0.0001f;
                 const float z1[4] = {n[4], n[1], n[3], n[0]}, z2[4] = {n[5], n[2], n[4], n[1]}, z3[4] = {n[7], n[4], n[6], n[3]}, z4[4] = {n[8], n[5], n[7], n[4]};
                 float nn[4], nv[4], t[4] = {0.f, 0.f, 0.f, 0.f};
@@ -500,10 +513,10 @@
                     }
 #pragma unroll
                     for (int k = 0; k < 4; ++k) t[k] = t[k] + ((hh[0][k] + hh[1][k]) + hh[2][k]);
-                    if (g == 3) { *dst = make_float4(o[0], o[1], o[2], o[3]); dst += step; __builtin_amdgcn_sched_barrier(0); }
-                    if (g == 6) { *dst = make_float4(o[4], o[5], o[6], o[7]); dst += step; __builtin_amdgcn_sched_barrier(0); }
-                    if (g == 9) { *dst = make_float4(o[8], o[9], o[10], o[11]); dst += step; __builtin_amdgcn_sched_barrier(0); }
-                    if (g == 15) { *dst = make_float4(o[12], o[13], o[14], o[15]); dst += step; __builtin_amdgcn_sched_barrier(0); }
+                    if (g == 3) { put(0, o[0], o[1], o[2], o[3]); __builtin_amdgcn_sched_barrier(0); }
+                    if (g == 6) { put(1, o[4], o[5], o[6], o[7]); __builtin_amdgcn_sched_barrier(0); }
+                    if (g == 9) { put(2, o[8], o[9], o[10], o[11]); __builtin_amdgcn_sched_barrier(0); }
+                    if (g == 15) { put(3, o[12], o[13], o[14], o[15]); __builtin_amdgcn_sched_barrier(0); }
                 }
                 float ci[9];
 #pragma unroll
@@ -513,14 +526,14 @@
 #pragma unroll
                     for (int k = 0; k < 4; ++k) hh[k] = fminf(s2, nn[k]) * nv[k];
                     ci[g] = (hh[0] + hh[1]) + (hh[2] + hh[3]);
-                    if (g == 1) { *dst = make_float4(o[16], o[17], ci[0], ci[1]); dst += step; __builtin_amdgcn_sched_barrier(0); }
-                    if (g == 5) { *dst = make_float4(ci[2], ci[3], ci[4], ci[5]); dst += step; __builtin_amdgcn_sched_barrier(0); }
+                    if (g == 1) { put(4, o[16], o[17], ci[0], ci[1]); __builtin_amdgcn_sched_barrier(0); }
+                    if (g == 5) { put(5, ci[2], ci[3], ci[4], ci[5]); __builtin_amdgcn_sched_barrier(0); }
                 }
                 const float tscale = (float)(2 * 0.2357);
 #pragma unroll
                 for (int k = 0; k < 4; ++k) t[k] = t[k] * tscale;
-                *dst = make_float4(ci[6], ci[7], ci[8], t[0]); dst += step;
-                *dst = make_float4(t[1], t[2], t[3], 0.0f);
+                put(6, ci[6], ci[7], ci[8], t[0]);
+                put(7, t[1], t[2], t[3], 0.0f);
             }
         }
 #pragma unroll
@@ -532,7 +545,8 @@
     }
 }
 
-__global__ void __launch_bounds__(256) feat_ring_zero_k(MlStarts st, const LvDesc* __restrict__ lv, int B, float* __restrict__ feat_base, int oy, int ox)
+__global__ void __launch_bounds__(256) feat_ring_zero_k(MlStarts st, const LvDesc* __restrict__ lv, int B, float* __restrict__ feat_base,
+                                                        uint16_t* __restrict__ feat16_base, int oy, int ox)
 {
     const int g = ml_block(st);
     if (g >= st.b0[st.nl]) return;
@@ -546,9 +560,16 @@
     if (px >= d.fwp) return;
     const int x = px - ox, y = py - oy;
     if (x >= 0 && y >= 0 && x < d.hog_nc && y < d.hog_nr) return;
-    float4* dst = reinterpret_cast<float4*>(feat_base + d.feat_off + (size_t)b * d.feat_stride + feat_at(py, 0, px, d.fwp));
-#pragma unroll
-    for (int k = 0; k < 8; ++k) dst[(size_t)k * d.fwp] = make_float4(0.f, 0.f, 0.f, 0.f);
+    if (feat_base) {
+        float4* dst = reinterpret_cast<float4*>(feat_base + d.feat_off + (size_t)b * d.feat_stride + feat_at(py, 0, px, d.fwp));
+#pragma unroll
+        for (int k = 0; k < 8; ++k) dst[(size_t)k * d.fwp] = make_float4(0.f, 0.f, 0.f, 0.f);
+    }
+    if (feat16_base) {
+        u32x4* dst = reinterpret_cast<u32x4*>(feat16_base + d.feat_off + (size_t)b * d.feat_stride + feat16_at(py, 0, px, d.fwp));
+#pragma unroll
+        for (int k = 0; k < 4; ++k) dst[(size_t)k * d.fwp] = (u32x4){0u, 0u, 0u, 0u};
+    }
 }
 
 __global__ void __launch_bounds__(128) __attribute__((amdgpu_waves_per_eu(2, 2)))
@@ -943,7 +964,7 @@
     PVF_REQUIRE(pc->sqrt_probe == 1, "v_sqrt_f32 is not within one step below the correctly rounded root on this device: the FHOG kernel's one-sided correction does not hold");
 }
 
-static MlPlan* ml_features(Ctx* c, const std::vector<Frame>& frames, int upsample)
+static MlPlan* ml_features(Ctx* c, const std::vector<Frame>& frames, int upsample, bool with_f16 = false)
 {
     const DetectorModel& m = c->det;
     const int B = (int)frames.size();
@@ -954,18 +975,32 @@
     if (p->fused_blocks == 0) return p;
     check_dpp_direction(c);
     ProfScope ps(c, "fhog", c->det_stream);
-    if (c->s_feat.p != feat_before || c->feat_ring_owner != (const void*)p) {
-        hipLaunchKernelGGL(feat_ring_zero_k, dim3(ml_grid(p->feat_blocks)), dim3(256), 0, c->det_stream, p->feat, p->d_lv, B, c->s_feat.as<float>(), oy, ox);
-        c->feat_ring_owner = (const void*)p;
+    const bool ring32 = c->s_feat.p != feat_before || c->feat_ring_owner != (const void*)p;
+    bool ring16 = false;
+    if (with_f16) {
+        const void* feat16_before = c->s_feat16.p;
+        c->s_feat16.ensure(p->feat_floats * sizeof(uint16_t) + 64);
+        ring16 = c->s_feat16.p != feat16_before || c->feat16_ring_owner != (const void*)p;
+    }
+    if (ring32 || ring16) {
+        hipLaunchKernelGGL(feat_ring_zero_k, dim3(ml_grid(p->feat_blocks)), dim3(256), 0, c->det_stream, p->feat, p->d_lv, B,
+                           ring32 ? c->s_feat.as<float>() : nullptr, ring16 ? c->s_feat16.as<uint16_t>() : nullptr, oy, ox);
+        if (ring32) c->feat_ring_owner = (const void*)p;
+        if (ring16) c->feat16_ring_owner = (const void*)p;
     }
     static std::atomic<uint64_t> attr_set{0};
     const uint64_t bit = 1ull << (c->device & 63);
     if (!(attr_set.load() & bit)) {
-        HIP_CHECK(hipFuncSetAttribute(reinterpret_cast<const void*>(fhog_split_ml_k), hipFuncAttributeMaxDynamicSharedMemorySize, FS_LDS_BYTES));
+        HIP_CHECK(hipFuncSetAttribute(reinterpret_cast<const void*>(fhog_split_ml_k<false>), hipFuncAttributeMaxDynamicSharedMemorySize, FS_LDS_BYTES));
+        HIP_CHECK(hipFuncSetAttribute(reinterpret_cast<const void*>(fhog_split_ml_k<true>), hipFuncAttributeMaxDynamicSharedMemorySize, FS_LDS_BYTES));
         attr_set.fetch_or(bit);
     }
-    hipLaunchKernelGGL(fhog_split_ml_k, dim3(ml_grid(p->fused_blocks)), dim3(512), FS_LDS_BYTES, c->det_stream, p->fused, p->d_lv, B,
-                       c->s_pyr.as<uint8_t>(), c->s_feat.as<float>(), orientation_lut_wrapped(c), oy, ox);
+    if (with_f16)
+        hipLaunchKernelGGL(fhog_split_ml_k<true>, dim3(ml_grid(p->fused_blocks)), dim3(512), FS_LDS_BYTES, c->det_stream, p->fused, p->d_lv, B,
+                           c->s_pyr.as<uint8_t>(), c->s_feat.as<float>(), c->s_feat16.as<uint16_t>(), orientation_lut_wrapped(c), oy, ox);
+    else
+        hipLaunchKernelGGL(fhog_split_ml_k<false>, dim3(ml_grid(p->fused_blocks)), dim3(512), FS_LDS_BYTES, c->det_stream, p->fused, p->d_lv, B,
+                           c->s_pyr.as<uint8_t>(), c->s_feat.as<float>(), (uint16_t*)nullptr, orientation_lut_wrapped(c), oy, ox);
     return p;
 }
 
@@ -973,16 +1008,21 @@
 {
     const DetectorModel& m = c->det;
     const int B = (int)frames.size();
-    MlPlan* p = ml_features(c, frames, upsample);
+    bool screened = false;
+    if (c->det_screen && !c->det_screen_suspended) {
+        MlPlan* p0 = ml_plan(c, frames[0].h, frames[0].w, upsample, B);
+        if (p0->walk_blocks != 0) {
+            if (!p0->screen_built) { screen_plan_build(p0->screen, p0->lv, B); p0->screen_built = true; }
+            screened = p0->screen.usable;
+        }
+    }
+    MlPlan* p = ml_features(c, frames, upsample, screened);
     if (p->walk_blocks == 0) return;
-    if (c->det_screen && !c->det_screen_suspended) {
-        if (!p->screen_built) { screen_plan_build(p->screen, p->lv, B); p->screen_built = true; }
-        if (p->screen.usable) {
-            ProfScope ps(c, "score_screened", c->det_stream);
-            screen_launch(c, p->screen, p->d_lv, B, c->s_feat.as<float>(), sp0, d_counts, d_cands, d_counts + B);
-            ++c->screen_batches;
-            return;
-        }
+    if (screened) {
+        ProfScope ps(c, "score_screened", c->det_stream);
+        screen_launch(c, p->screen, p->d_lv, B, c->s_feat.as<float>(), c->s_feat16.as<uint16_t>(), sp0, d_counts, d_cands, d_counts + B);
+        ++c->screen_batches;
+        return;
     }
     ProfScope ps(c, "score", c->det_stream);
     const size_t lds = (size_t)2 * (((2 * 48 + 11) * 31 + 3) / 4 * 4) * sizeof(float);
@@ -1031,6 +1071,37 @@
             for (int j = 0; j < 8; ++j)
                 for (int x = 0; x < d.fw; ++x)
                     memcpy(out->data() + ((size_t)y * d.fw + x) * PVF_FHOG_STRIDE + 4 * j, dev.data() + feat_at(y, j, x, d.fwp), 4 * sizeof(float));
+    }
+    HIP_CHECK(hipStreamSynchronize(c->det_stream));
+}
+
+void det_level_features_f16(Ctx* c, const Frame& f, int upsample, int level, std::vector<uint16_t>* out, int* fh, int* fw, int pad_kq,
+                            std::vector<uint16_t>* pad_out, int* fwp)
+{
+    PVF_REQUIRE(c->det.loaded, "detector not loaded");
+    std::vector<Frame> fr{f};
+    MlPlan* p = ml_features(c, fr, upsample, true);
+    PVF_REQUIRE(level >= 0 && level < (int)p->lv.size(), "pyramid level out of range");
+    const LvDesc& d = p->lv[level];
+    *fh = d.fh; *fw = d.fw; *fwp = d.fwp;
+    if (out || pad_out) {
+        std::vector<uint16_t> dev((size_t)d.feat_stride);
+        if (!dev.empty())
+            HIP_CHECK(hipMemcpyAsync(dev.data(), c->s_feat16.as<uint16_t>() + d.feat_off, dev.size() * sizeof(uint16_t), hipMemcpyDeviceToHost, c->det_stream));
+        HIP_CHECK(hipStreamSynchronize(c->det_stream));
+        if (out) {
+            out->resize((size_t)d.fh * d.fw * PVF_FHOG_STRIDE);
+            for (int y = 0; y < d.fh; ++y)
+                for (int kq = 0; kq < 4; ++kq)
+                    for (int x = 0; x < d.fw; ++x)
+                        memcpy(out->data() + ((size_t)y * d.fw + x) * PVF_FHOG_STRIDE + 8 * kq, dev.data() + feat16_at(y, kq, x, d.fwp), 8 * sizeof(uint16_t));
+        }
+        if (pad_out) {
+            PVF_REQUIRE(pad_kq >= 0 && pad_kq < 4, "level features f16: plane octet out of range");
+            pad_out->resize((size_t)d.fh * d.fwp * 8);
+            for (int y = 0; y < d.fh; ++y)
+                memcpy(pad_out->data() + (size_t)y * d.fwp * 8, dev.data() + feat16_at(y, pad_kq, 0, d.fwp), (size_t)d.fwp * 8 * sizeof(uint16_t));
+        }
     }
     HIP_CHECK(hipStreamSynchronize(c->det_stream));
 }
diff --git a/pyannote-video_amd/csrc/detect_ml.h b/pyannote-video_amd/csrc/detect_ml.h
--- a/pyannote-video_amd/csrc/detect_ml.h
+++ b/pyannote-video_amd/csrc/detect_ml.h
@@ -19,6 +19,7 @@
 
 #define FEAT_PAD_COLS 52
 __host__ __device__ __forceinline__ size_t feat_at(int row, int j, int col, int fwp) { return (((size_t)row * 8 + j) * fwp + col) * 4; }
+__host__ __device__ __forceinline__ size_t feat16_at(int row, int kq, int col, int fwp) { return (((size_t)row * 4 + kq) * fwp + col) * 8; }
 
 struct ScoreParams { float thresh[8]; int n_filters; int level; int cap; };
 struct CandRec { float score; int32_t filter, level, r, c; };
@@ -42,6 +43,6 @@
     ScreenPlan& operator=(const ScreenPlan&) = delete;
 };
 void screen_plan_build(ScreenPlan& sp, const std::vector<LvDesc>& lv, int B);
-void screen_launch(Ctx* c, const ScreenPlan& sp, const LvDesc* d_lv, int B, const float* feat, const ScoreParams& thr, int* d_counts,
-                   CandRec* d_cands, int* ctl);
+void screen_launch(Ctx* c, const ScreenPlan& sp, const LvDesc* d_lv, int B, const float* feat, const uint16_t* feat16, const ScoreParams& thr,
+                   int* d_counts, CandRec* d_cands, int* ctl);
 void screen_prepare_model(DetectorModel& d, const float* w);
diff --git a/pyannote-video_amd/csrc/pvf_internal.h b/pyannote-video_amd/csrc/pvf_internal.h
--- a/pyannote-video_amd/csrc/pvf_internal.h
+++ b/pyannote-video_amd/csrc/pvf_internal.h
@@ -232,6 +232,8 @@
     bool det_screen = true, det_screen_suspended = false, screen_attr_set = false;
     int screen_list_cap = 1 << 20;
     DevBuf s_screen;
+    DevBuf s_feat16;
+    const void* feat16_ring_owner = nullptr;
     int64_t screen_batches = 0, screen_listed = 0, screen_retries = 0;
     double screen_pipe_err = -1;
     bool screen_pipe_flushes_subnormals = false;
@@ -334,6 +336,8 @@
 void det_nms(const DetectorModel& m, const std::vector<RawDet>& sorted, std::vector<RawDet>& out);
 void det_pyramid_level(Ctx* c, const Frame& f, int upsample, int level, std::vector<uint8_t>* out, int* h, int* w);
 void det_level_features(Ctx* c, const Frame& f, int upsample, int level, std::vector<float>* out, int* fh, int* fw);
+void det_level_features_f16(Ctx* c, const Frame& f, int upsample, int level, std::vector<uint16_t>* out, int* fh, int* fw, int pad_kq,
+                            std::vector<uint16_t>* pad_out, int* fwp);
 void det_level_plan(Ctx* c, const Frame& f, int upsample, int level, int32_t out[8]);
 void det_pyramid_batch(Ctx* c, const std::vector<Frame>& frames, int upsample);
 void fhog_debug(Ctx* c, const uint8_t* himg, int h, int w, int cell, int pad_r, int pad_c, std::vector<float>& out, int* fh, int* fw);
diff --git a/pyannote-video_amd/csrc/screen.hip b/pyannote-video_amd/csrc/screen.hip
--- a/pyannote-video_amd/csrc/screen.hip
+++ b/pyannote-video_amd/csrc/screen.hip
@@ -11,13 +11,8 @@
 #define SCR_B_BYTES (10 * 12 * 64 * 16)
 #define SCR_M_STRIDE (12 * 64 * 16)
 
-__device__ __forceinline__ uint32_t pk_f16(float a, float b)
-{
-    return __builtin_bit_cast(uint32_t, __builtin_amdgcn_cvt_pkrtz(a, b));
-}
-
 template <int NG>
-__device__ __forceinline__ void screen_walk(const ScreenItem t, const LvDesc* __restrict__ lv, const float* __restrict__ feat_base,
+__device__ __forceinline__ void screen_walk(const ScreenItem t, const LvDesc* __restrict__ lv, const uint16_t* __restrict__ feat_base,
                                             const uint8_t* s_b, const float th_lane, int* __restrict__ ctl, uint2* __restrict__ list,
                                             const int list_cap, u32x4& mx)
 {
@@ -28,13 +23,12 @@
     const int fw = lv[t.lv].fw;
     const long long feat_off = lv[t.lv].feat_off, feat_stride = lv[t.lv].feat_stride;
     const int fwp = lv[t.lv].fwp;
-    const float* fb = feat_base + feat_off + (size_t)t.b * feat_stride + feat_at(t.r_base, 0, t.c_base, fwp);
-    const int row_bytes = (8 * fwp - t.c_base) * 16;
+    const uint16_t* fb = feat_base + feat_off + (size_t)t.b * feat_stride + feat16_at(t.r_base, 0, t.c_base, fwp);
+    const int row_bytes = (4 * fwp - t.c_base) * 16;
     const int fh_in = t.out_rows + FR - 1;
     const int c1 = fw - (FC - FC / 2 - 1);
-    const int voff = i * 48 + kq * 2 * fwp * 16;
-    const int voff2 = voff + fwp * 16;
-    const int voff_t = i < 3 ? voff : 0x40000000, voff2_t = i < 3 ? voff2 : 0x40000000;
+    const int voff = i * 48 + kq * fwp * 16;
+    const int voff_t = i < 3 ? voff : 0x40000000;
     f32x4 acc[10][NG];
 #pragma unroll
     for (int q = 0; q < 10; ++q)
@@ -42,19 +36,14 @@
         for (int g = 0; g < NG; ++g) acc[q][g] = (f32x4){0.f, 0.f, 0.f, 0.f};
     const uint8_t* b_lo = s_b + lane * 16;
     const uint8_t* b_hi = s_b + lane * 16 + 5 * SCR_M_STRIDE;
-    auto load_cls = [&](int row, int cls, u32x4 (&raw)[NG + 1][2]) {
-        const __amdgpu_buffer_rsrc_t rs = __builtin_amdgcn_make_buffer_rsrc((void*)(fb + (size_t)row * 8 * fwp * 4), 0,
+    auto load_cls = [&](int row, int cls, u32x4 (&raw)[NG + 1]) {
+        const __amdgpu_buffer_rsrc_t rs = __builtin_amdgcn_make_buffer_rsrc((void*)(fb + (size_t)row * 4 * fwp * 8), 0,
                                                                             row < fh_in ? row_bytes : 0, RSRC_FLAGS);
 #pragma unroll
-        for (int g = 0; g <= NG; ++g) {
-            raw[g][0] = __builtin_amdgcn_raw_buffer_load_b128(rs, (g < NG ? voff : voff_t) + cls * 16 + g * 768, 0, 0);
-            raw[g][1] = __builtin_amdgcn_raw_buffer_load_b128(rs, (g < NG ? voff2 : voff2_t) + cls * 16 + g * 768, 0, 0);
-        }
-    };
-    auto cvt_frag = [&](const u32x4 (&r)[2]) -> u32x4 {
-        u32x4 o;
-        o.x = pk_f16(__uint_as_float(r[0].x), __uint_as_float(r[0].y)); o.y = pk_f16(__uint_as_float(r[0].z), __uint_as_float(r[0].w));
-        o.z = pk_f16(__uint_as_float(r[1].x), __uint_as_float(r[1].y)); o.w = pk_f16(__uint_as_float(r[1].z), __uint_as_float(r[1].w));
+        for (int g = 0; g <= NG; ++g)
+            raw[g] = __builtin_amdgcn_raw_buffer_load_b128(rs, (g < NG ? voff : voff_t) + cls * 16 + g * 768, 0, 0);
+    };
+    auto take_frag = [&](const u32x4& o) -> u32x4 {
 #pragma unroll
         for (int k = 0; k < 4; ++k) mx[k] = __builtin_bit_cast(uint32_t, __builtin_elementwise_max(__builtin_bit_cast(f16x2, mx[k]), __builtin_bit_cast(f16x2, o[k])));
         return o;
@@ -96,12 +85,12 @@
 
     u32x4 A[3][NG + 1];
     {
-        u32x4 raw[NG + 1][2];
+        u32x4 raw[NG + 1];
 #pragma unroll
         for (int cls = 0; cls < 3; ++cls) {
             load_cls(0, cls, raw);
 #pragma unroll
-            for (int g = 0; g <= NG; ++g) A[cls][g] = cvt_frag(raw[g]);
+            for (int g = 0; g <= NG; ++g) A[cls][g] = take_frag(raw[g]);
         }
     }
     auto b_frag = [&](int q, int j) -> u32x4 {
@@ -112,7 +101,7 @@
     for (int q = 0; q < 10; ++q) bn[q] = b_frag(q, 0);
     for (int s = 0; s < fh_in; ++s) {
         u32x4 An[3][NG + 1];
-        u32x4 raw[NG + 1][2];
+        u32x4 raw[NG + 1];
         f32x4 done[NG];
 #pragma unroll
         for (int j = 0; j < 12; ++j) {
@@ -139,7 +128,7 @@
             }
             if (j % 4 == 3) {
 #pragma unroll
-                for (int g = 0; g <= NG; ++g) An[j / 4][g] = cvt_frag(raw[g]);
+                for (int g = 0; g <= NG; ++g) An[j / 4][g] = take_frag(raw[g]);
             }
             __builtin_amdgcn_sched_barrier(0);
         }
@@ -154,7 +143,7 @@
 }
 
 __global__ void __launch_bounds__(256) __attribute__((amdgpu_waves_per_eu(1, 1)))
-score_screen_k(const ScreenItem* __restrict__ items, const LvDesc* __restrict__ lv, const float* __restrict__ feat_base,
+score_screen_k(const ScreenItem* __restrict__ items, const LvDesc* __restrict__ lv, const uint16_t* __restrict__ feat_base,
                const u32x4* __restrict__ Bh, ScreenParams sp, int* __restrict__ ctl, uint2* __restrict__ list)
 {
     extern __shared__ __attribute__((aligned(16))) uint8_t s_b[];
@@ -468,8 +457,8 @@
     PVF_REQUIRE(dpp_ok, "screening: v_mov_b32_dpp row_shl:1 / row_shr:15 do not move data as the screening kernel expects on this device");
 }
 
-void screen_launch(Ctx* c, const ScreenPlan& plan, const LvDesc* d_lv, int B, const float* feat, const ScoreParams& thr, int* d_counts,
-                   CandRec* d_cands, int* ctl)
+void screen_launch(Ctx* c, const ScreenPlan& plan, const LvDesc* d_lv, int B, const float* feat, const uint16_t* feat16, const ScoreParams& thr,
+                   int* d_counts, CandRec* d_cands, int* ctl)
 {
     const DetectorModel& m = c->det;
     if (plan.n_items == 0) return;
@@ -495,7 +484,7 @@
     c->s_screen.ensure((size_t)sp.list_cap * sizeof(uint2) + 64);
     uint2* list = c->s_screen.as<uint2>();
     const int grid = std::min(c->n_cu, (plan.n_items + 3) / 4);
-    hipLaunchKernelGGL(score_screen_k, dim3(grid), dim3(256), SCR_B_BYTES, c->det_stream, plan.d_items, d_lv, feat,
+    hipLaunchKernelGGL(score_screen_k, dim3(grid), dim3(256), SCR_B_BYTES, c->det_stream, plan.d_items, d_lv, feat16,
                        reinterpret_cast<const u32x4*>(m.d_bscreen), sp, ctl, list);
     hipLaunchKernelGGL(score_list_k, dim3(256), dim3(256), 0, c->det_stream, list, ctl, sp.list_cap, d_lv, feat, m.d_w, thr, d_counts, d_cands);
 }
diff --git a/pyannote-video_amd/pyannote_video_amd/_lib.py b/pyannote-video_amd/pyannote_video_amd/_lib.py
--- a/pyannote-video_amd/pyannote_video_amd/_lib.py
+++ b/pyannote-video_amd/pyannote_video_amd/_lib.py
@@ -114,6 +114,7 @@
     "pvf_debug_pyramid_level": (C.c_int32, [H, H, C.c_int32, C.c_int32, P, P, P]),
     "pvf_debug_pyramid_batch": (C.c_int32, [H, P, C.c_int32, C.c_int32]),
     "pvf_debug_level_features": (C.c_int32, [H, H, C.c_int32, C.c_int32, P, P, P]),
+    "pvf_debug_level_features_f16": (C.c_int32, [H, H, C.c_int32, C.c_int32, P, P, P, C.c_int32, P, P]),
     "pvf_debug_level_plan": (C.c_int32, [H, H, C.c_int32, C.c_int32, P]),
     "pvf_debug_fhog": (C.c_int32, [H, P, C.c_int32, C.c_int32, C.c_int32, C.c_int32, C.c_int32, P, P, P]),
     "pvf_debug_detect_raw": (C.c_int32, [H, H, C.c_int32, C.c_double, P, P, C.c_int32, P]),
diff --git a/pyannote-video_amd/pyannote_video_amd/runtime.py b/pyannote-video_amd/pyannote_video_amd/runtime.py
--- a/pyannote-video_amd/pyannote_video_amd/runtime.py
+++ b/pyannote-video_amd/pyannote_video_amd/runtime.py
@@ -532,6 +532,17 @@
         if out.size:
             check(self._l.pvf_debug_level_features(self._h, f.handle, upsample, level, ptr(out), C.byref(fh), C.byref(fw)))
         return out
+
+    def level_features_f16(self, frame, upsample, level, pad_kq=0):
+        f = self.stage(frame)
+        fh, fw, fwp = C.c_int32(0), C.c_int32(0), C.c_int32(0)
+        check(self._l.pvf_debug_level_features_f16(self._h, f.handle, upsample, level, None, C.byref(fh), C.byref(fw), 0, None, C.byref(fwp)))
+        out = np.zeros((fh.value, fw.value, 32), np.uint16)
+        pad = np.zeros((fh.value, fwp.value, 8), np.uint16)
+        if out.size:
+            check(self._l.pvf_debug_level_features_f16(self._h, f.handle, upsample, level, ptr(out), C.byref(fh), C.byref(fw),
+                                                       int(pad_kq), ptr(pad), C.byref(fwp)))
+        return out, pad
 
     def level_plan(self, frame, upsample, level):
         f = self.stage(frame)
```
